# zhiyuns/AFCM

Measured on AMD Instinct MI355X. Metric: generator fwd+bwd images/sec @256^2, higher is better.
Workload: dtype bf16; 1 GPU; AFCM --model stylegan3 generator training step (fwd + L1 loss + bwd + grad all-reduce + Adam), IXI T1->T2 shape: 256x256, 4->1 channels, full-width 58.5M-param generator, random init; global_batch=16, per_gpu_batch=16, resolution=256, parallelism=dp1, world_size=1, gradient_buckets=0, comm_dtype=fp32, homogeneous_dot=True

## Files before the change

afcm_amd/_lib.py:

```python
import ctypes as C
import os

import numpy as np
import torch

_HERE = os.path.dirname(os.path.abspath(__file__))
LIB_PATH = os.environ.get('AFCM_HIP_LIB') or os.path.join(_HERE, 'libafcm_hip.so')

F32, F16, BF16 = 0, 1, 2
E_NOKERNEL, E_INVALID = -1, -2
SIGNS_NONE, SIGNS_WRITE, SIGNS_READ = 0, 1, 2
SRC_U8, SRC_I16, SRC_F32, SRC_F64 = 0, 1, 2, 3
SCHEDULE_SLOTS = 8
EMA_LERP, EMA_COPY = 0, 1
GROUP_2B, GROUP_4B = 2, 4

_DTYPES = {torch.float32: F32, torch.float16: F16, torch.bfloat16: BF16}
OUT_DTYPES = tuple(_DTYPES)
SOURCE_DTYPES = {torch.uint8: SRC_U8, torch.int16: SRC_I16, torch.float32: SRC_F32, torch.float64: SRC_F64}
NUMPY_SOURCE_DTYPES = {np.dtype(np.uint8): SRC_U8, np.dtype(np.int16): SRC_I16, np.dtype(np.float32): SRC_F32, np.dtype(np.float64): SRC_F64}


class FilteredLReluArgs(C.Structure):
    _fields_ = [
        ('x', C.c_void_p), ('y', C.c_void_p), ('b', C.c_void_p), ('signs', C.c_void_p),
        ('fu', C.c_void_p), ('fd', C.c_void_p),
        ('dtype', C.c_int32),
        ('n', C.c_int32), ('c', C.c_int32), ('xh', C.c_int32), ('xw', C.c_int32), ('yh', C.c_int32), ('yw', C.c_int32),
        ('fuw', C.c_int32), ('fuh', C.c_int32), ('fdw', C.c_int32), ('fdh', C.c_int32),
        ('up', C.c_int32), ('down', C.c_int32),
        ('px0', C.c_int32), ('px1', C.c_int32), ('py0', C.c_int32), ('py1', C.c_int32),
        ('sx', C.c_int32), ('sy', C.c_int32), ('sh', C.c_int32), ('swb', C.c_int32),
        ('gain', C.c_float), ('slope', C.c_float), ('clamp', C.c_float),
        ('flip_filter', C.c_int32), ('sign_mode', C.c_int32),
        ('workspace', C.c_void_p), ('sign_layout', C.c_int32), ('plane_sum_slots', C.c_int32),
        ('plane_sum', C.c_void_p), ('oscale', C.c_void_p), ('skip', C.c_void_p), ('oscale2', C.c_void_p),
        ('x_pitch', C.c_int32), ('y_pitch', C.c_int32), ('skip_pitch', C.c_int32), ('row_pitch_ok', C.c_int32),
        ('clamp_flags', C.c_void_p),
    ]


AFFINE_MAX = 16


class AffineBank(C.Structure):
    _fields_ = [
        ('layers', C.c_int32), ('n', C.c_int32), ('kw', C.c_int32), ('kg', C.c_int32),
        ('w_stride_n', C.c_int64), ('w_stride_l', C.c_int64),
        ('w', C.c_void_p), ('g', C.c_void_p),
        ('weight', C.c_void_p * AFFINE_MAX), ('bias', C.c_void_p * AFFINE_MAX),
        ('cout', C.c_int32 * AFFINE_MAX), ('w_index', C.c_int32 * AFFINE_MAX),
        ('alpha', C.c_float * AFFINE_MAX), ('beta', C.c_float * AFFINE_MAX),
    ]


MODULATION_MAX = 16


class ModulationLayer(C.Structure):
    _fields_ = [('cout', C.c_int32), ('cin', C.c_int32), ('kk', C.c_int32), ('demodulate', C.c_int32)] + [
        (k, C.c_void_p) for k in ('w', 't', 'magnitude', 'w_hat', 'wsq', 'scale', 's_eff', 'd', 'r', 'g_hat', 'g_s', 'g_d', 'dw', 'dt', 'workspace')]


PACK_MAX = 32


class PackEntry(C.Structure):
    _fields_ = [('dst_fwd', C.c_void_p), ('dst_dgrad', C.c_void_p), ('w', C.c_void_p),
                ('cout', C.c_int32), ('cin', C.c_int32), ('rows_pad_fwd', C.c_int32), ('rows_pad_dgrad', C.c_int32)]


_lib = None
ABI_VERSION = 13

_i32, _i64, _f32, _f64, _vp = C.c_int32, C.c_int64, C.c_float, C.c_double, C.c_void_p
SIGNATURES = {
    'afcm_abi_version': (C.c_int, []),
    'afcm_last_error': (C.c_char_p, []),
    'afcm_noop': (C.c_int, [_vp]),
    'afcm_filtered_lrelu_shapes': (C.c_int, [C.POINTER(FilteredLReluArgs)]),
    'afcm_filtered_lrelu': (C.c_int, [C.POINTER(FilteredLReluArgs), _vp]),
    'afcm_filtered_lrelu_workspace_bytes': (C.c_int64, []),
    'afcm_filtered_lrelu_prepare': (C.c_int, [C.POINTER(FilteredLReluArgs), _vp]),
    'afcm_filtered_lrelu_act': (C.c_int, [_vp, _vp, _i32, _i32, _i32, _i32, _i32, _i32, _i32, _i32, _i32, _f32, _f32, _f32, _i32, _vp]),
    'afcm_upfirdn2d': (C.c_int, [_vp, _vp, _vp, _i32, _i32, _i32, _i32, _i32, _i32, _i32, _i32, _i32, _i32, _i32, _i32, _i32,
                                 _i32, _i32, _i32, _f32, _vp]),
    'afcm_bias_act': (C.c_int, [_vp, _vp, _vp, _vp, _vp, _vp, _i32, _i64, _i64, _i32, _i32, _i32, _f32, _f32, _f32, _vp]),
    'afcm_conv2d_block_k': (C.c_int, [_i32]),
    'afcm_conv2d_block_k_ks': (C.c_int, [_i32, _i32]),
    'afcm_conv2d_pack_weights_bk': (C.c_int, [_vp, _vp, _i32, _i32, _i32, _i32, _i32, _i32, _i32, _vp]),
    'afcm_conv2d_pack_weights': (C.c_int, [_vp, _vp, _i32, _i32, _i32, _i32, _i32, _i32, _vp]),
    'afcm_conv2d_pack_weights2': (C.c_int, [_vp, _vp, _vp, _i32, _i32, _i32, _i32, _i32, _i32, _vp]),
    'afcm_conv2d': (C.c_int, [_vp, _vp, _vp, _vp, _vp, _i32, _i32, _i32, _i32, _i32, _i32, _i32, _i32, _i32, _vp]),
    'afcm_conv2d_ld': (C.c_int, [_vp, _vp, _vp, _vp, _vp, _i32, _i32, _i32, _i32, _i32, _i32, _i32, _i32, _i32, _i32, _i32, _vp]),
    'afcm_conv2d_plan': (C.c_int, [_i32] * 11 + [C.POINTER(_i32)]),
    'afcm_conv2d_wgrad_plan': (C.c_int, [_i32] * 11 + [C.POINTER(_i32)]),
    'afcm_conv2d_wgrad_splits': (C.c_int, [_i32, _i32, _i32, _i32]),
    'afcm_conv2d_wgrad': (C.c_int, [_vp, _vp, _vp, _vp, _i32, _i32, _i32, _i32, _i32, _i32, _i32, _i32, _vp]),
    'afcm_conv2d_wgrad_ld': (C.c_int, [_vp, _vp, _vp, _vp, _i32, _i32, _i32, _i32, _i32, _i32, _i32, _i32, _i32, _i32, _vp]),
    'afcm_conv2d_wgrad_dots_ld': (C.c_int, [_vp, _vp, _vp, _vp, _vp, _vp, _i32, _i32, _i32, _i32, _i32, _i32, _i32, _i32, _i32, _i32, _vp]),
    'afcm_scale_planes': (C.c_int, [_vp, _vp, _vp, _i32, _i32, _i64, _i32, _vp]),
    'afcm_plane_dot': (C.c_int, [_vp, _vp, _vp, _i32, _i64, _i32, _vp]),
    'afcm_plane_dot_ld': (C.c_int, [_vp, _vp, _vp, _i32, _i64, _i32, _i32, _i32, _i32, _vp]),
    'afcm_split16': (C.c_int, [_vp, _vp, _vp, _vp, _i32, _i64, _i32, _i32, _i64, _vp]),
    'afcm_conv2d_split': (C.c_int, [_vp, _vp, _vp, _vp, _vp, _i32, _i32, _i32, _i32, _i32, _i32, _i32, _i32, _i32, C.c_uint32, _i64, _vp, _vp, _vp]),
    'afcm_amax_bits': (C.c_int, [_vp, _vp, _i64, _i32, _vp, _vp]),
    'afcm_unscale': (C.c_int, [_vp, _i64, _vp, _vp, _vp]),
    'afcm_plane_dot_parts': (C.c_int, [_vp, _vp, _i64, _i32, _vp, _i32, _i64, _i32, _vp, _vp]),
    'afcm_conv2d_pack_split': (C.c_int, [_vp, _vp, _vp, _i32, _i32, _i32, _i32, _i32, _i32, C.c_uint32, _vp]),
    'afcm_plane_dot_gated_ld': (C.c_int, [_vp, _vp, _vp, _i32, _i64, _i32, _i32, _i32, _i32, _vp, _i32, _vp, _vp, _vp, _vp, _vp]),
    'afcm_weight_norm_fwd': (C.c_int, [_vp, _vp, _vp, _vp, _i32, _i32, _i32, _vp]),
    'afcm_weight_norm_bwd': (C.c_int, [_vp, _vp, _vp, _vp, _vp, _i32, _i32, _i32, _vp]),
    'afcm_style_coefs_fwd': (C.c_int, [_vp, _vp, _vp, _vp, _vp, _vp, _i32, _i32, _i32, _i32, _vp]),
    'afcm_style_coefs_bwd': (C.c_int, [_vp, _vp, _vp, _vp, _vp, _vp, _vp, _vp, _vp, _vp, _i32, _i32, _i32, _i32, _vp]),
    'afcm_layer_bwd_coefs': (C.c_int, [_vp, _vp, _vp, _vp, _i32, _vp, _vp, _vp, _vp, _vp, _i32, _i32, _vp]),
    'afcm_affine_bank_workspace_bytes': (C.c_int64, [C.POINTER(AffineBank)]),
    'afcm_affine_bank_fwd': (C.c_int, [C.POINTER(AffineBank), C.POINTER(C.c_void_p), _vp]),
    'afcm_modulation_bank_workspace_floats': (C.c_int64, [_i32, _i32, _i32, _i32]),
    'afcm_modulation_bank_fwd': (C.c_int, [C.POINTER(ModulationLayer), _i32, _i32, _vp]),
    'afcm_modulation_bank_bwd': (C.c_int, [C.POINTER(ModulationLayer), _i32, _i32, _vp]),
    'afcm_conv2d_stride2': (C.c_int, [_vp, _vp, _vp, _i32, _i32, _i32, _i32, _i32, _i32, _i32, _i32, _vp]),
    'afcm_conv2d_pack_bank': (C.c_int, [C.POINTER(PackEntry), _i32, _i32, _i32, _vp]),
    'afcm_affine_bank_bwd': (C.c_int, [C.POINTER(AffineBank), C.POINTER(C.c_void_p), C.POINTER(C.c_void_p), C.POINTER(C.c_void_p), _vp, _vp, _vp, _vp]),
    'afcm_pool_blocks_fwd': (C.c_int, [_vp, _vp, _i32, _i64, _i32, _i32, _vp]),
    'afcm_pool_blocks_bwd': (C.c_int, [_vp, _vp, _i32, _i64, _i32, _i32, _vp]),
    'afcm_l1_partials': (C.c_int, [_vp, _vp, _vp, _i64, _i32, _f32, _vp]),
    'afcm_l1_grad': (C.c_int, [_vp, _vp, _vp, _vp, _i64, _f32, _vp]),
    'afcm_axpy_planes': (C.c_int, [_vp, _vp, _vp, _vp, _i32, _i64, _i32, _vp]),
    'afcm_fc_act_fwd': (C.c_int, [_vp, _vp, _vp, _vp, _i32, _i32, _i32, _f32, _f32, _i32, _vp]),
    'afcm_fc_act_bwd': (C.c_int, [_vp, _vp, _vp, _vp, _vp, _vp, _vp, _i32, _i32, _i32, _f32, _f32, _i32, _vp]),
    'afcm_mapping_input_fwd': (C.c_int, [_vp, _vp, _vp, _vp, _vp, _i32, _i32, _i32, _i32, _f32, _f32, _vp]),
    'afcm_mapping_input_bwd_workspace_bytes': (C.c_int64, [_i32, _i32]),
    'afcm_mapping_input_bwd': (C.c_int, [_vp, _vp, _vp, _vp, _vp, _vp, _i32, _i32, _i32, _i32, _f32, _f32, _vp, _vp]),
    'afcm_adam_chunk_elems': (C.c_int32, []),
    'afcm_adam_multi': (C.c_int, [_vp, _i32, _i64, _f32, _f32, _f32, _f32, _f32, _f32, _f32, _f32, _i32, _f32, _f32, _i32, _vp]),
    'afcm_adam_multi_capturable': (C.c_int, [_vp, _i32, _i64, _vp, _f32, _f32, _f32, _f32, _f32, _i32, _f32, _f32, _i32, _vp]),
    'afcm_adam_multi_capturable_d': (C.c_int, [_vp, _i32, _i64, _vp, C.c_double, C.c_double, C.c_double, _f32, _f32, _i32, _f32, _f32, _i32, _vp]),
    'afcm_adam_multi_capturable_lr': (C.c_int, [_vp, _i32, _i64, _vp, _vp, C.c_double, C.c_double, _f32, _f32, _i32, _f32, _f32, _i32, _vp]),
    'afcm_plane_metrics_workspace_bytes': (C.c_int64, [_i64, _i32, _i32]),
    'afcm_plane_metrics': (C.c_int, [_vp, _vp, _vp, _i32, _i32, _i64, _i32, _i32, _i64, _i64, _i64, _i64, _i64, _i64, _i32, _f64, _f64, _vp, _vp]),
    'afcm_volume_ssim_workspace_bytes': (C.c_int64, [_i64, _i32, _i32, _i32]),
    'afcm_volume_ssim': (C.c_int, [_vp, _vp, _vp, _i32, _i32, _i64, _i32, _i32, _i32] + [_i64] * 8 + [_i32, _f64, _f64, _vp, _vp]),
    'afcm_slice_assemble': (C.c_int, [_vp, _vp, _vp, _i32, _i32, _i32, _i32, _i32, _i64, _i32, _i32, _i32, _i32, _i32, _i32, _f64, _f64, _vp]),
    'afcm_halo_accumulate': (C.c_int, [_vp, _vp, _vp, _i32, _i64, _i64, _i64, _i64, _i64, _i32, _vp, _i32, _i32, _i32] + [_i32] * 17 + [_vp]),
    'afcm_batch_assemble': (C.c_int, [_vp, _vp, _vp, _vp, _i64, _i32, _vp, _i32, _vp, _i32, _vp] + [_i32] * 6 + [_f64, _f64, _vp]),
    'afcm_batch_assemble_aug': (C.c_int, [_vp, _vp, _vp, _vp, _i64, _i32, _vp, _i32, _vp, _i32, _vp, _vp] + [_i32] * 6 + [_f64, _f64, _vp]),
    'afcm_cursor_advance': (C.c_int, [_vp, _i64, _vp]),
    'afcm_schedule_advance': (C.c_int, [_vp, _i64, _f64, _f64, _f64, _f64, _vp]),
    'afcm_gauss_blur_rmax': (C.c_int32, []),
    'afcm_gauss_blur': (C.c_int, [_vp, _vp, _vp, _i64, _i32, _i32, _f64, _vp, _vp]),
    'afcm_ema_multi': (C.c_int, [_vp, _i32, _i64, _f64, _vp, _vp]),
    'afcm_rescale_plan': (C.c_int, [_i64, _i32, C.POINTER(_i32)]),
    'afcm_rescale_workspace_bytes': (C.c_int64, [_i64, _i32]),
    'afcm_rescale_intensity': (C.c_int, [_vp, _vp, _vp, _vp, _i32, _i32, _i32, _i32, _i64, _f64, _f64, _vp]),
    'afcm_percentile_plan': (C.c_int, [_i64, _i32, C.POINTER(_i32)]),
    'afcm_percentile_workspace_bytes': (C.c_int64, [_i64, _i32]),
    'afcm_percentile_bounds': (C.c_int, [_vp, _vp, _vp, _i32, _i32, _i32, _i32, _i64, _f64, _f64, _i32, _vp]),
    'afcm_clip_normalize': (C.c_int, [_vp, _vp, _vp, _i32, _i32, _i32, _i32, _i64, _vp]),
    'afcm_group_chunk_bytes': (C.c_int32, []),
    'afcm_group_expand': (C.c_int, [_vp, _vp, _i32, _i32, _vp, _vp]),
}


def load():
    global _lib
    if _lib is None:
        if not os.path.exists(LIB_PATH):
            raise RuntimeError(
                f'{LIB_PATH} is missing: the HIP kernels are not built.  Run `python -c "import __graft_entry__ as g; g.build()"` '
                f'or `make -C afcm_amd/csrc`.  afcm_amd has no CPU fallback.')
        lib = C.CDLL(LIB_PATH)
        for name, (res, args) in SIGNATURES.items():
            fn = getattr(lib, name)
            fn.restype = res
            fn.argtypes = args
        if lib.afcm_abi_version() != ABI_VERSION:
            raise RuntimeError(f'libafcm_hip.so ABI version {lib.afcm_abi_version()} does not match this package ({ABI_VERSION}); rebuild it')
        _lib = lib
    return _lib


def dtype_code(t):
    try:
        return _DTYPES[t.dtype]
    except KeyError:
        raise RuntimeError(f'afcm_amd kernels support float32/float16/bfloat16, got {t.dtype}') from None


def source_code(dtype, what):
    code = (SOURCE_DTYPES if isinstance(dtype, torch.dtype) else NUMPY_SOURCE_DTYPES).get(dtype)
    if code is None:
        raise RuntimeError(f'{what}: source volumes are uint8 / int16 / float32 / float64, got {dtype}')
    return code


def require_out_dtype(dtype, what):
    if dtype not in OUT_DTYPES:
        raise RuntimeError(f'{what}: output dtype float32 / float16 / bfloat16, got {dtype}')


def require_slice_num(slice_num, what):
    if slice_num not in (1, 4):
        raise RuntimeError(f'{what}: slice number {slice_num} not supported (1 or 4)')


def require_gpu(*tensors):
    for t in tensors:
        if t is not None and t.device.type != 'cuda':
            raise RuntimeError(
                f'afcm_amd ops need ROCm device tensors (got a tensor on {t.device}); there is no CPU path in this package '
                f'-- the aten reference lives in oracle/ and is test-only')


def stream_ptr(t):
    return torch.cuda.current_stream(t.device).cuda_stream


def ptr(t):
    return None if t is None else t.data_ptr()


def check(rc, what):
    if rc == 0 or rc == E_NOKERNEL:
        return rc
    if rc == E_INVALID:
        raise RuntimeError(f'{what}: {load().afcm_last_error().decode()}')
    raise RuntimeError(f'{what}: HIP error {rc - 1000} at kernel launch')


def launched(rc, what):
    if check(rc, what) == E_NOKERNEL:
        raise RuntimeError(f'{what}: no kernel for this shape (the Python gate and the C entry point disagree)')
    return rc
```

afcm_amd/csrc/common.h:

```cpp
#pragma once
#include <hip/hip_runtime.h>
#include <stdint.h>
#include <stdio.h>
#include <stdarg.h>

#include "../../include/afcm_hip.h"

namespace afcm {

typedef _Float16 f16_t;
typedef __bf16   bf16_t;

template <typename T> __device__ __forceinline__ float to_f32(T v) { return (float)v; }
template <typename T> __device__ __forceinline__ T from_f32(float v) { return (T)v; }

template <int DT> struct dtype_of;
template <> struct dtype_of<AFCM_F32>  { typedef float  type; };
template <> struct dtype_of<AFCM_F16>  { typedef f16_t  type; };
template <> struct dtype_of<AFCM_BF16> { typedef bf16_t type; };

static inline int dtype_size(int dt) { return dt == AFCM_F32 ? 4 : 2; }

void set_error(const char* fmt, ...);

#define AFCM_REQUIRE(cond, ...)                         \
    do {                                                \
        if (!(cond)) {                                  \
            ::afcm::set_error(__VA_ARGS__);             \
            return AFCM_E_INVALID;                      \
        }                                               \
    } while (0)

static inline int hip_status(hipError_t e) { return e == hipSuccess ? AFCM_OK : 1000 + (int)e; }

constexpr int kAdamChunk = 16384;

constexpr int cdiv(int a, int b) { return (a + b - 1) / b; }
constexpr int round_up(int a, int b) { return cdiv(a, b) * b; }

__device__ __forceinline__ int xcd_order(int bid, int total) {
    const int x = bid & 7, k = bid >> 3, q = total >> 3, r = total & 7;
    return x * q + (x < r ? x : r) + k;
}
constexpr int cmax(int a, int b) { return a > b ? a : b; }
constexpr int odd4(int a) { return ((a / 4) % 2 == 1) ? a : a + 4; }

__host__ __device__ __forceinline__ int floor_div(int a, int b) {
    int q = a / b;
    return (a % b != 0 && (a < 0)) ? q - 1 : q;
}
__host__ __device__ __forceinline__ int pos_mod(int a, int b) {
    int r = a % b;
    return r < 0 ? r + b : r;
}

}
```

afcm_amd/csrc/conv2d_planes.hip:

```cpp
#include "conv2d_common.h"

namespace afcm {

template <typename T> struct Vec4 { T v[4]; } __attribute__((aligned(sizeof(T) * 4)));

__device__ __forceinline__ float formed_f32(float v) { asm("" : "+v"(v)); return v; }

template <typename TI, typename TO>
__global__ __launch_bounds__(256) void scale_planes_kernel(TO* __restrict__ y, const TI* __restrict__ x, const float* __restrict__ scale,
                                                           long long planes, int hw) {
    const int per = (hw + 3) >> 2;
    const long long total = planes * per;
    const bool vec = (hw & 3) == 0 && ((uintptr_t)x & (sizeof(TI) * 4 - 1)) == 0 && ((uintptr_t)y & (sizeof(TO) * 4 - 1)) == 0;
    for (long long idx = (long long)blockIdx.x * blockDim.x + threadIdx.x; idx < total; idx += (long long)gridDim.x * blockDim.x) {
        const long long plane = idx / per;
        const int i0 = (int)(idx - plane * per) << 2;
        const float sc = scale ? scale[plane] : 1.f;
        const TI* xp = x + plane * hw + i0;
        TO* yp = y + plane * hw + i0;
        if (vec) {
            const Vec4<TI> in = *(const Vec4<TI>*)xp;
            Vec4<TO> out;
#pragma unroll
            for (int e = 0; e < 4; e++) out.v[e] = from_f32<TO>(formed_f32(to_f32(in.v[e]) * sc));
// ... 9 lines not shown
template <typename T>
__global__ __launch_bounds__(256) void axpy_planes_kernel(T* __restrict__ y, const T* __restrict__ a, const T* __restrict__ b, const float* __restrict__ scale,
                                                          long long planes, int hw) {
    union V16 { uint4 u; T v[8]; };
    const int per = hw >> 3;
    for (long long plane = blockIdx.y; plane < planes; plane += gridDim.y) {
        const float sc = scale ? scale[plane] : 1.f;
        const uint4* ap = (const uint4*)a + plane * per;
        const uint4* bp = (const uint4*)b + plane * per;
        uint4* yp = (uint4*)y + plane * per;
        for (int i = blockIdx.x * blockDim.x + threadIdx.x; i < per; i += gridDim.x * blockDim.x) {
            V16 av, bv, out;
            av.u = ap[i];
            bv.u = bp[i];
#pragma unroll
            for (int e = 0; e < 8; e++) out.v[e] = from_f32<T>(to_f32(av.v[e]) + sc * to_f32(bv.v[e]));
            yp[i] = out.u;
        }
    }
}

__global__ __launch_bounds__(256) void amax_bits_kernel(unsigned* __restrict__ out, const float* __restrict__ x, long long planes, int hw,
                                                        const float* __restrict__ scale) {
    __shared__ unsigned red[4];
    unsigned m = 0;
    const long long numel = planes * hw;
    const bool vec = (((uintptr_t)x & 15) == 0) && (hw & 3) == 0;
    const long long n4 = vec ? (numel >> 2) : 0;
    const int per = hw >> 2;
    const long long stride = (long long)gridDim.x * blockDim.x;
    long long i = (long long)blockIdx.x * blockDim.x + threadIdx.x;
    auto fold = [&](const uint4 v, long long g) {
        const unsigned ax = v.x & 0x7fffffffu, ay = v.y & 0x7fffffffu, az = v.z & 0x7fffffffu, aw = v.w & 0x7fffffffu;
        unsigned a = max(max(ax < 0x7f800000u ? ax : 0u, ay < 0x7f800000u ? ay : 0u), max(az < 0x7f800000u ? az : 0u, aw < 0x7f800000u ? aw : 0u));
        if (scale) {
            a = __float_as_uint(__uint_as_float(a) * __builtin_fabsf(scale[g / per]));
            if (a >= 0x7f800000u) a = 0u;
        }
        m = max(m, a);
    };
    for (; i + 3 * stride < n4; i += 4 * stride) {
        const uint4 v0 = ((const uint4*)x)[i], v1 = ((const uint4*)x)[i + stride], v2 = ((const uint4*)x)[i + 2 * stride], v3 = ((const uint4*)x)[i + 3 * stride];
        fold(v0, i); fold(v1, i + stride); fold(v2, i + 2 * stride); fold(v3, i + 3 * stride);
    }
    for (; i < n4; i += stride) fold(((const uint4*)x)[i], i);
    for (long long j = 4 * n4 + (long long)blockIdx.x * blockDim.x + threadIdx.x; j < numel; j += stride) {
        const float v = x[j] * (scale ? scale[j / hw] : 1.f);
        const unsigned a = __float_as_uint(v) & 0x7fffffffu;
        m = max(m, a < 0x7f800000u ? a : 0u);
    }
#pragma unroll
    for (int o = 32; o > 0; o >>= 1) m = max(m, (unsigned)__shfl_xor((int)m, o));
    if ((threadIdx.x & 63) == 0) red[threadIdx.x >> 6] = m;
    __syncthreads();
    if (threadIdx.x == 0) {
        m = max(max(red[0], red[1]), max(red[2], red[3]));
        if (m > __atomic_load_n(out, __ATOMIC_RELAXED)) atomicMax(out, m);
    }
}

template <typename TP>
__global__ __launch_bounds__(256) void plane_dot_parts_kernel(float* __restrict__ out, const TP* __restrict__ parts, long long part_stride, int nparts,
                                                              const float* __restrict__ b, long long planes, int hw, const unsigned* __restrict__ bound) {
    __shared__ float red[4];
    const long long plane = blockIdx.x;
    if (plane >= planes) return;
    const TP* ap = parts + plane * hw;
    const float* bp = b + plane * hw;
    float acc = 0.f;
    if ((hw & 3) == 0 && (part_stride & 3) == 0) {
        union V8 { uint2 u; TP v[4]; };
        for (int i = threadIdx.x * 4; i < hw; i += blockDim.x * 4) {
            const float4 b0 = *(const float4*)(bp + i);
            const float bv[4] = {b0.x, b0.y, b0.z, b0.w};
            for (int k = 0; k < nparts; k++) {
                V8 a; a.u = *(const uint2*)(ap + k * part_stride + i);
#pragma unroll
                for (int e = 0; e < 4; e++) acc += (float)a.v[e] * bv[e];
            }
        }
    } else {
        for (int i = threadIdx.x; i < hw; i += blockDim.x) {
            float a = 0.f;
            for (int k = 0; k < nparts; k++) a += (float)ap[k * part_stride + i];
            acc += a * bp[i];
        }
    }
#pragma unroll
    for (int o = 32; o > 0; o >>= 1) acc += __shfl_xor(acc, o);
    if ((threadIdx.x & 63) == 0) red[threadIdx.x >> 6] = acc;
    __syncthreads();
    if (threadIdx.x == 0) {
        float inv = 1.f;
        if (bound) pow2_factor(bound[0], &inv);
        out[plane] = (red[0] + red[1] + red[2] + red[3]) * inv;
    }
}

__global__ __launch_bounds__(256) void unscale_kernel(float* __restrict__ t, long long numel, const unsigned* __restrict__ bound_a, const unsigned* __restrict__ bound_b) {
    float ia = 1.f, ib = 1.f;
    if (bound_a) pow2_factor(bound_a[0], &ia);
    if (bound_b) pow2_factor(bound_b[0], &ib);
    const float inv = ia * ib;
    for (long long i = (long long)blockIdx.x * blockDim.x + threadIdx.x; i < numel; i += (long long)gridDim.x * blockDim.x) t[i] *= inv;
}

template <typename TP, int PARTS>
__global__ __launch_bounds__(256) void split16_kernel(TP* __restrict__ parts, const float* __restrict__ x, const float* __restrict__ scale,
                                                      const unsigned* __restrict__ bound, long long planes, int hw, long long part_stride) {
    const int per = (hw + 3) >> 2;
    const long long total = planes * per;
    const bool vec = (hw & 3) == 0;
    const float gs = bound ? pow2_factor(bound[0]) : 1.f;
    for (long long idx = (long long)blockIdx.x * blockDim.x + threadIdx.x; idx < total; idx += (long long)gridDim.x * blockDim.x) {
        const long long plane = idx / per;
        const int i0 = (int)(idx - plane * per) << 2;
        const float sc = (scale ? scale[plane] : 1.f) * gs;
        const float* xp = x + plane * hw + i0;
        TP* yp = parts + plane * hw + i0;
        float v[4];
        if (vec) {
            const Vec4<float> in = *(const Vec4<float>*)xp;
#pragma unroll
            for (int e = 0; e < 4; e++) v[e] = in.v[e] * sc;
        } else {
#pragma unroll
            for (int e = 0; e < 4; e++) v[e] = (i0 + e < hw) ? xp[e] * sc : 0.f;
        }
        Vec4<TP> out[PARTS];
#pragma unroll
        for (int e = 0; e < 4; e++) {
            float r = v[e];
#pragma unroll
            for (int k = 0; k < PARTS; k++) {
                const TP q = (TP)r;
                out[k].v[e] = q;
                const float qf = (float)q;
                r = (__builtin_fabsf(qf) <= 3.4028234664e38f) ? r - qf : 0.f;
            }
        }
#pragma unroll
        for (int k = 0; k < PARTS; k++) {
            if (vec) {
                *(Vec4<TP>*)(yp + k * part_stride) = out[k];
            } else {
#pragma unroll
                for (int e = 0; e < 4; e++)
                    if (i0 + e < hw) yp[k * part_stride + e] = out[k].v[e];
            }
        }
    }
}

template <typename T>
__global__ __launch_bounds__(256) void plane_dot_kernel(float* __restrict__ out, const T* __restrict__ a, const T* __restrict__ b,
                                                        long long planes, int hw) {
    constexpr int E = 16 / (int)sizeof(T);
    union V16 { uint4 u; T v[E]; };
    __shared__ float part[4];
    const long long plane = blockIdx.x;
    if (plane >= planes) return;
    const long long off = plane * hw;
    const T* ap = a + off;
    const T* bp = b ? b + off : nullptr;
    int head = (int)((E - (off % E)) % E);
    if (head > hw) head = hw;
    const int nv = (hw - head) / E;
    float s0 = 0.f, s1 = 0.f;
    {
        const int tail0 = head + nv * E;
        int i = -1;
        if ((int)threadIdx.x < head) i = threadIdx.x;
        else if ((int)threadIdx.x - head < hw - tail0) i = tail0 + (int)threadIdx.x - head;
        if (i >= 0) s0 = to_f32(ap[i]) * (bp ? to_f32(bp[i]) : 1.f);
    }
    const uint4* av = (const uint4*)(ap + head);
    const uint4* bv = bp ? (const uint4*)(bp + head) : nullptr;
    int i = threadIdx.x;
    if (bv) {
        for (; i + 768 < nv; i += 1024) {
            V16 a0, a1, a2, a3, b0, b1, b2, b3;
            a0.u = av[i]; a1.u = av[i + 256]; a2.u = av[i + 512]; a3.u = av[i + 768];
            b0.u = bv[i]; b1.u = bv[i + 256]; b2.u = bv[i + 512]; b3.u = bv[i + 768];
#pragma unroll
            for (int e = 0; e < E; e++) {
                s0 = fmaf(to_f32(a0.v[e]), to_f32(b0.v[e]), s0); s1 = fmaf(to_f32(a1.v[e]), to_f32(b1.v[e]), s1);
                s0 = fmaf(to_f32(a2.v[e]), to_f32(b2.v[e]), s0); s1 = fmaf(to_f32(a3.v[e]), to_f32(b3.v[e]), s1);
            }
        }
    }
    for (; i + 256 < nv; i += 512) {
        V16 a0, a1, b0, b1;
        a0.u = av[i]; a1.u = av[i + 256];
        if (bv) {
            b0.u = bv[i]; b1.u = bv[i + 256];
#pragma unroll
            for (int e = 0; e < E; e++) { s0 = fmaf(to_f32(a0.v[e]), to_f32(b0.v[e]), s0); s1 = fmaf(to_f32(a1.v[e]), to_f32(b1.v[e]), s1); }
        } else {
#pragma unroll
            for (int e = 0; e < E; e++) { s0 += to_f32(a0.v[e]); s1 += to_f32(a1.v[e]); }
        }
    }
    if (i < nv) {
        V16 a0, b0;
        a0.u = av[i];
        if (bv) {
            b0.u = bv[i];
#pragma unroll
            for (int e = 0; e < E; e++) s0 = fmaf(to_f32(a0.v[e]), to_f32(b0.v[e]), s0);
        } else {
#pragma unroll
            for (int e = 0; e < E; e++) s0 += to_f32(a0.v[e]);
        }
    }
    float s = s0 + s1;
#pragma unroll
    for (int off2 = 32; off2 > 0; off2 >>= 1) s += __shfl_down(s, off2, 64);
    if ((threadIdx.x & 63) == 0) part[threadIdx.x >> 6] = s;
    __syncthreads();
    if (threadIdx.x == 0) out[plane] = part[0] + part[1] + part[2] + part[3];
}

template <typename T>
__global__ __launch_bounds__(256) void plane_dot_wave_kernel(float* __restrict__ out, const T* __restrict__ a, const T* __restrict__ b,
                                                             long long planes, int hw) {
    constexpr int E = 16 / (int)sizeof(T);
    union V16 { uint4 u; T v[E]; };
    const int lane = threadIdx.x & 63;
    const long long plane = (long long)blockIdx.x * 4 + (threadIdx.x >> 6);
    if (plane >= planes) return;
    const long long off = plane * hw;
    const T* ap = a + off;
    const T* bp = b ? b + off : nullptr;
    int head = (int)((E - (off % E)) % E);
    if (head > hw) head = hw;
    const int nv = (hw - head) / E;
    float s0 = 0.f, s1 = 0.f;
    {
        const int tail0 = head + nv * E;
        int i = -1;
        if (lane < head) i = lane;
        else if (lane - head < hw - tail0) i = tail0 + lane - head;
        if (i >= 0) s0 = to_f32(ap[i]) * (bp ? to_f32(bp[i]) : 1.f);
    }
    const uint4* av = (const uint4*)(ap + head);
    const uint4* bv = bp ? (const uint4*)(bp + head) : nullptr;
    int i = lane;
    for (; i + 64 < nv; i += 128) {
        V16 a0, a1, b0, b1;
        a0.u = av[i]; a1.u = av[i + 64];
        if (bv) {
            b0.u = bv[i]; b1.u = bv[i + 64];
#pragma unroll
            for (int e = 0; e < E; e++) { s0 = fmaf(to_f32(a0.v[e]), to_f32(b0.v[e]), s0); s1 = fmaf(to_f32(a1.v[e]), to_f32(b1.v[e]), s1); }
        } else {
#pragma unroll
            for (int e = 0; e < E; e++) { s0 += to_f32(a0.v[e]); s1 += to_f32(a1.v[e]); }
        }
    }
    if (i < nv) {
        V16 a0, b0;
        a0.u = av[i];
        if (bv) {
            b0.u = bv[i];
#pragma unroll
            for (int e = 0; e < E; e++) s0 = fmaf(to_f32(a0.v[e]), to_f32(b0.v[e]), s0);
        } else {
#pragma unroll
            for (int e = 0; e < E; e++) s0 += to_f32(a0.v[e]);
        }
    }
    float s = s0 + s1;
#pragma unroll
    for (int off2 = 32; off2 > 0; off2 >>= 1) s += __shfl_down(s, off2, 64);
    if (lane == 0) out[plane] = s;
}

struct PlaneGate {
    const int* flags;
    int slots;
    const float *osc, *gz, *nsc, *gsk;
};
template <typename T, bool PER_WAVE>
__global__ __launch_bounds__(256) void plane_dot_rows_kernel(float* __restrict__ out, const T* __restrict__ a, const T* __restrict__ b,
                                                             long long planes, int h, int w, int lda, int ldb, PlaneGate gate) {
    constexpr int E = 16 / (int)sizeof(T);
    union V16 { uint4 u; T v[E]; };
    __shared__ float part[4];
    const int nthr = PER_WAVE ? 64 : 256;
    const int t = PER_WAVE ? (int)(threadIdx.x & 63) : (int)threadIdx.x;
    const long long plane = PER_WAVE ? (long long)blockIdx.x * 4 + (threadIdx.x >> 6) : (long long)blockIdx.x;
    if (plane >= planes) return;
    if (gate.flags != nullptr) {
        int any = 0;
        for (int i = 0; i < gate.slots; i++) any |= gate.flags[plane * gate.slots + i];
        if (!any) {
            const float zz = gate.gz[plane], kk = gate.gsk ? (gate.nsc ? gate.nsc[plane] : 1.f) * gate.gsk[plane] : 0.f;
            const float diff = zz - kk;
            if (!(gate.gsk != nullptr && fabsf(diff) * 8.f < fabsf(zz) + fabsf(kk))) {
                if (t == 0) out[plane] = gate.osc[plane] * diff;
                return;
            }
        }
    }
    const int nvec = (w + E - 1) / E, total = h * nvec;
    const unsigned magic = nvec > 1 ? (unsigned)((0x100000000ull + (unsigned)nvec - 1) / (unsigned)nvec) : 0u;
    const T* ap = a + plane * h * lda;
    const T* bp = b ? b + plane * h * ldb : nullptr;
    float s0 = 0.f, s1 = 0.f;
    for (int i0 = t; i0 < total; i0 += 4 * nthr) {
        V16 av[4], bv[4];
        int skip[4];
#pragma unroll
        for (int u = 0; u < 4; u++) {
            const int i = i0 + u * nthr;
            const int ic = i < total ? i : total - 1;
            int row = nvec > 1 ? (int)__umulhi((unsigned)ic, magic) : ic;
            row -= row * nvec > ic;
            const int col = (ic - row * nvec) * E;
            const int colc = col + E <= w ? col : w - E;
            skip[u] = i < total ? col - colc : E;
            av[u].u = *(const uint4*)(ap + (size_t)row * lda + colc);
            if (bp) bv[u].u = *(const uint4*)(bp + (size_t)row * ldb + colc);
        }
#pragma unroll
        for (int u = 0; u < 4; u++) {
#pragma unroll
            for (int e = 0; e < E; e++) {
                const float x = e >= skip[u] ? to_f32(av[u].v[e]) : 0.f;
                const float y = bp ? to_f32(bv[u].v[e]) : 1.f;
                if (u & 1) s1 = fmaf(x, e >= skip[u] ? y : 0.f, s1); else s0 = fmaf(x, e >= skip[u] ? y : 0.f, s0);
            }
        }
    }
    float s = s0 + s1;
#pragma unroll
    for (int off2 = 32; off2 > 0; off2 >>= 1) s += __shfl_down(s, off2, 64);
    if (PER_WAVE) {
        if ((threadIdx.x & 63) == 0) out[plane] = s;
    } else {
        if ((threadIdx.x & 63) == 0) part[threadIdx.x >> 6] = s;
        __syncthreads();
        if (threadIdx.x == 0) out[plane] = part[0] + part[1] + part[2] + part[3];
    }
}

}

using namespace afcm;

extern "C" int afcm_split16(void* parts, const float* x, const float* scale, const uint32_t* bound, int32_t dtype, int64_t planes, int32_t hw,
                            int32_t nparts, int64_t part_stride, void* stream) {
    AFCM_REQUIRE(parts != nullptr && x != nullptr && planes > 0 && hw > 0, "split16: empty input");
    AFCM_REQUIRE(dtype == AFCM_BF16 || dtype == AFCM_F16, "split16: parts are bfloat16 or float16");
    AFCM_REQUIRE(nparts == 2 || nparts == 3, "split16: 2 or 3 parts (got %d)", nparts);
    AFCM_REQUIRE(part_stride >= planes * (long long)hw && part_stride % 4 == 0, "split16: part stride %lld must cover the tensor and be a multiple of 4", (long long)part_stride);
    AFCM_REQUIRE(((uintptr_t)x & 15) == 0 && ((uintptr_t)parts & 7) == 0, "split16: x must be 16-byte, parts 8-byte aligned");
    long long blocks = (planes * ((hw + 3) >> 2) + 255) / 256;
    if (blocks > 4096) blocks = 4096;
    dim3 grid((unsigned)blocks), block(256);
    hipStream_t st = (hipStream_t)stream;
#define AFCM_SPLIT(T, K) hipLaunchKernelGGL((split16_kernel<T, K>), grid, block, 0, st, (T*)parts, x, scale, (const unsigned*)bound, (long long)planes, hw, (long long)part_stride)
    if (dtype == AFCM_BF16) { if (nparts == 2) AFCM_SPLIT(bf16_t, 2); else AFCM_SPLIT(bf16_t, 3); }
    else { if (nparts == 2) AFCM_SPLIT(f16_t, 2); else AFCM_SPLIT(f16_t, 3); }
#undef AFCM_SPLIT
    return hip_status(hipGetLastError());
}

extern "C" int afcm_amax_bits(uint32_t* out, const float* x, int64_t planes, int32_t hw, const float* scale, void* stream) {
    AFCM_REQUIRE(out != nullptr && x != nullptr && planes > 0 && hw > 0, "amax_bits: empty input");
    AFCM_REQUIRE(((uintptr_t)out & 3) == 0 && ((uintptr_t)x & 3) == 0, "amax_bits: misaligned pointer");
    long long blocks = (planes * hw / 16 + 255) / 256;
    blocks = blocks < 1 ? 1 : (blocks > 2048 ? 2048 : blocks);
    hipLaunchKernelGGL(amax_bits_kernel, dim3((unsigned)blocks), dim3(256), 0, (hipStream_t)stream, (unsigned*)out, x, (long long)planes, hw, scale);
    return hip_status(hipGetLastError());
}

extern "C" int afcm_plane_dot_parts(float* out, const void* parts, int64_t part_stride, int32_t nparts, const float* b, int32_t dtype, int64_t planes,
                                    int32_t hw, const uint32_t* bound, void* stream) {
    AFCM_REQUIRE(out != nullptr && parts != nullptr && b != nullptr && planes > 0 && hw > 0, "plane_dot_parts: empty input");
    AFCM_REQUIRE(dtype == AFCM_BF16 || dtype == AFCM_F16, "plane_dot_parts: parts are bfloat16 or float16");
    AFCM_REQUIRE(nparts >= 1 && nparts <= 3 && part_stride >= planes * (long long)hw, "plane_dot_parts: 1..3 parts, a stride covering the tensor");
    AFCM_REQUIRE(planes < (1ll << 31), "plane_dot_parts: too many planes");
    AFCM_REQUIRE(((uintptr_t)parts & 7) == 0 && ((uintptr_t)b & 15) == 0, "plane_dot_parts: parts must be 8-byte, b 16-byte aligned");
    hipStream_t st = (hipStream_t)stream;
    if (dtype == AFCM_BF16) hipLaunchKernelGGL((plane_dot_parts_kernel<bf16_t>), dim3((unsigned)planes), dim3(256), 0, st, out, (const bf16_t*)parts, (long long)part_stride, nparts, b, (long long)planes, hw, (const unsigned*)bound);
    else hipLaunchKernelGGL((plane_dot_parts_kernel<f16_t>), dim3((unsigned)planes), dim3(256), 0, st, out, (const f16_t*)parts, (long long)part_stride, nparts, b, (long long)planes, hw, (const unsigned*)bound);
    return hip_status(hipGetLastError());
}

extern "C" int afcm_unscale(float* t, int64_t numel, const uint32_t* bound_a, const uint32_t* bound_b, void* stream) {
    AFCM_REQUIRE(t != nullptr && numel > 0, "unscale: empty input");
    long long blocks = (numel + 255) / 256;
    if (blocks > 2048) blocks = 2048;
    hipLaunchKernelGGL(unscale_kernel, dim3((unsigned)blocks), dim3(256), 0, (hipStream_t)stream, t, (long long)numel, (const unsigned*)bound_a, (const unsigned*)bound_b);
    return hip_status(hipGetLastError());
}

extern "C" int afcm_scale_planes(void* y, const void* x, const float* scale, int32_t dtype_in, int32_t dtype_out, int64_t planes,
                                 int32_t hw, void* stream) {
    AFCM_REQUIRE(y != nullptr && x != nullptr && planes > 0 && hw > 0, "scale_planes: empty input");
    long long blocks = (planes * ((hw + 3) >> 2) + 255) / 256;
    if (blocks > 2048) blocks = 2048;
    dim3 grid((unsigned)blocks), block(256);
    hipStream_t st = (hipStream_t)stream;
#define AFCM_SP(TI, TO) hipLaunchKernelGGL((scale_planes_kernel<TI, TO>), grid, block, 0, st, (TO*)y, (const TI*)x, scale, (long long)planes, hw)
    if (dtype_in == AFCM_F32 && dtype_out == AFCM_F32) AFCM_SP(float, float);
    else if (dtype_in == AFCM_F32 && dtype_out == AFCM_BF16) AFCM_SP(float, bf16_t);
    else if (dtype_in == AFCM_F32 && dtype_out == AFCM_F16) AFCM_SP(float, f16_t);
    else if (dtype_in == AFCM_BF16 && dtype_out == AFCM_BF16) AFCM_SP(bf16_t, bf16_t);
    else if (dtype_in == AFCM_F16 && dtype_out == AFCM_F16) AFCM_SP(f16_t, f16_t);
    else if (dtype_in == AFCM_BF16 && dtype_out == AFCM_F32) AFCM_SP(bf16_t, float);
    else if (dtype_in == AFCM_F16 && dtype_out == AFCM_F32) AFCM_SP(f16_t, float);
    else { set_error("scale_planes: unsupported dtype pair %d -> %d", dtype_in, dtype_out); return AFCM_E_INVALID; }
#undef AFCM_SP
    return hip_status(hipGetLastError());
}

extern "C" int afcm_axpy_planes(void* y, const void* a, const void* b, const float* scale, int32_t dtype, int64_t planes, int32_t hw, void* stream) {
    AFCM_REQUIRE(y != nullptr && a != nullptr && b != nullptr && planes > 0 && hw > 0, "axpy_planes: empty input");
    AFCM_REQUIRE(dtype == AFCM_F16 || dtype == AFCM_BF16, "axpy_planes: 16-bit tensors only");
    if ((hw & 7) != 0 || ((((uintptr_t)y | (uintptr_t)a | (uintptr_t)b)) & 15) != 0) return AFCM_E_NOKERNEL;
    const int per = hw >> 3;
    const dim3 grid((unsigned)((per + 1023) / 1024), (unsigned)(planes < 65535 ? planes : 65535));
    hipStream_t st = (hipStream_t)stream;
    if (dtype == AFCM_BF16) hipLaunchKernelGGL((axpy_planes_kernel<bf16_t>), grid, dim3(256), 0, st, (bf16_t*)y, (const bf16_t*)a, (const bf16_t*)b, scale, (long long)planes, hw);
    else hipLaunchKernelGGL((axpy_planes_kernel<f16_t>), grid, dim3(256), 0, st, (f16_t*)y, (const f16_t*)a, (const f16_t*)b, scale, (long long)planes, hw);
    return hip_status(hipGetLastError());
}

extern "C" int afcm_plane_dot(float* out, const void* a, const void* b, int32_t dtype, int64_t planes, int32_t hw, void* stream) {
    AFCM_REQUIRE(out != nullptr && a != nullptr && planes > 0 && hw > 0, "plane_dot: empty input");
    AFCM_REQUIRE(planes < (1ll << 31), "plane_dot: too many planes");
    AFCM_REQUIRE((((uintptr_t)a | (uintptr_t)b) & 15) == 0, "plane_dot: operands must be 16-byte aligned");
    hipStream_t st = (hipStream_t)stream;
    const int esize = dtype == AFCM_F32 ? 4 : 2;
    const bool per_wave = (long long)hw * esize <= 16384;
    dim3 grid((unsigned)(per_wave ? (planes + 3) / 4 : planes)), block(256);
#define AFCM_PD(T) do { \
        if (per_wave) hipLaunchKernelGGL((plane_dot_wave_kernel<T>), grid, block, 0, st, out, (const T*)a, (const T*)b, (long long)planes, hw); \
        else hipLaunchKernelGGL((plane_dot_kernel<T>), grid, block, 0, st, out, (const T*)a, (const T*)b, (long long)planes, hw); } while (0)
    switch (dtype) {
        case AFCM_F32: AFCM_PD(float); break;
        case AFCM_F16: AFCM_PD(f16_t); break;
        case AFCM_BF16: AFCM_PD(bf16_t); break;
        default: set_error("plane_dot: bad dtype"); return AFCM_E_INVALID;
    }
#undef AFCM_PD
    return hip_status(hipGetLastError());
}

static int plane_dot_rows(float* out, const void* a, const void* b, int32_t dtype, int64_t planes, int32_t h, int32_t w,
                          int32_t a_pitch, int32_t b_pitch, const PlaneGate& gate, void* stream) {
    AFCM_REQUIRE(out != nullptr && a != nullptr && planes > 0 && h > 0 && w > 0, "plane_dot: empty input");
    AFCM_REQUIRE(planes < (1ll << 31), "plane_dot: too many planes");
    const int esize = dtype == AFCM_F32 ? 4 : 2;
    const int lda = a_pitch ? a_pitch : w, ldb = b_pitch ? b_pitch : w;
    AFCM_REQUIRE(lda >= w && ldb >= w, "plane_dot: row pitches %d / %d are below the width %d", lda, ldb, w);
    AFCM_REQUIRE(w >= 16 / esize, "plane_dot: rows of %d elements are shorter than one 16-byte vector", w);
    AFCM_REQUIRE((((uintptr_t)a | (uintptr_t)b) & 3) == 0 && (esize == 4 || ((w | lda | ldb) & 1) == 0), "plane_dot: rows must start on 4-byte boundaries");
    AFCM_REQUIRE((long long)h * (lda > ldb ? lda : ldb) < (1ll << 31) / 16, "plane_dot: plane is out of range");
    hipStream_t st = (hipStream_t)stream;
    const bool per_wave = (long long)h * w * esize <= 16384;
    dim3 grid((unsigned)(per_wave ? (planes + 3) / 4 : planes)), block(256);
#define AFCM_PDR(T) do { \
        if (per_wave) hipLaunchKernelGGL((plane_dot_rows_kernel<T, true>), grid, block, 0, st, out, (const T*)a, (const T*)b, (long long)planes, h, w, lda, ldb, gate); \
        else hipLaunchKernelGGL((plane_dot_rows_kernel<T, false>), grid, block, 0, st, out, (const T*)a, (const T*)b, (long long)planes, h, w, lda, ldb, gate); } while (0)
    switch (dtype) {
        case AFCM_F32: AFCM_PDR(float); break;
        case AFCM_F16: AFCM_PDR(f16_t); break;
        case AFCM_BF16: AFCM_PDR(bf16_t); break;
        default: set_error("plane_dot: bad dtype"); return AFCM_E_INVALID;
    }
#undef AFCM_PDR
    return hip_status(hipGetLastError());
}

extern "C" int afcm_plane_dot_ld(float* out, const void* a, const void* b, int32_t dtype, int64_t planes, int32_t h, int32_t w,
                                 int32_t a_pitch, int32_t b_pitch, void* stream) {
    return plane_dot_rows(out, a, b, dtype, planes, h, w, a_pitch, b_pitch, PlaneGate{nullptr, 0, nullptr, nullptr, nullptr, nullptr}, stream);
}

extern "C" int afcm_plane_dot_gated_ld(float* out, const void* a, const void* b, int32_t dtype, int64_t planes, int32_t h, int32_t w,
                                       int32_t a_pitch, int32_t b_pitch, const int32_t* flags, int32_t slots, const float* out_scale,
                                       const float* gz, const float* next_scale, const float* gskip, void* stream) {
    AFCM_REQUIRE(flags != nullptr && slots > 0 && out_scale != nullptr && gz != nullptr && b != nullptr, "plane_dot_gated: null pointer");
    return plane_dot_rows(out, a, b, dtype, planes, h, w, a_pitch, b_pitch, PlaneGate{flags, slots, out_scale, gz, next_scale, gskip}, stream);
}
```

afcm_amd/csrc/conv2d_wgrad.hip:

```cpp
#include <type_traits>

#include "conv2d_common.h"

namespace afcm {

constexpr int kWgKQ = 64;

struct WgradParams {
    const void* dy;
    const void* x;
    float* part;
    int N, O, I, H, W, P, Q, pad;
    int lddy, ldx;
    int splits, steps_per_split;
    int splits_img;
    int qchunks;
    int rowgroups;
};

template <int KS, int XOFF>
__global__ __launch_bounds__(512, 1) void conv2d_wgrad_kernel(WgradParams p) {
    constexpr int R = 1, KK = KS * KS;
    constexpr int PDY = kWgKQ + 8;
    constexpr int PX = kWgKQ + 24;
// ... 685 lines not shown
                    const frag_t bv = *(const frag_t*)(buf + x0_off[ib2] + xr * (64 * ROWB));
#pragma unroll
                    for (int ob2 = 0; ob2 < 2; ob2++) mma(a[ob2][xr], bv, 0, 2 * ob2 + ib2);
                });
            } else {
                frag_t a[2][R];
#pragma unroll
                for (int ob2 = 0; ob2 < 2; ob2++)
#pragma unroll
                    for (int rr = 0; rr < R; rr++) a[ob2][rr] = *(const frag_t*)(buf + a_off[ob2] + rr * (64 * ROWB));
                uint4 lo_n = *(const uint4*)(buf + x0_off[0]);
                uint4 hi_n = *(const uint4*)(buf + x1_off[0][0]);
                static_for<0, 2 * XR>([&](auto itc) __attribute__((always_inline)) {
                    constexpr int it = decltype(itc)::value, xr = it >> 1, ib2 = it & 1, NIT = 2 * XR;
                    const uint4 lo = lo_n, hi = hi_n;
                    if constexpr (it + 1 < NIT) {
                        constexpr int xr1 = (it + 1) >> 1, ib1 = (it + 1) & 1;
                        lo_n = *(const uint4*)(buf + x0_off[ib1] + xr1 * (64 * ROWB));
                        hi_n = *(const uint4*)(buf + x1_off[ib1][xr1]);
                    }
                    __builtin_amdgcn_sched_barrier(0);
                    if constexpr (LATE) {
                        static_assert(!LATE || NPIECE == NIT - 1, "one piece per iteration after the first");
                        if constexpr (it > 0) issue_piece(std::integral_constant<int, it - 1>{});
                    } else
                        issue_range(std::integral_constant<int, (it * NPIECE) / NIT>{}, std::integral_constant<int, ((it + 1) * NPIECE) / NIT>{});
                    asm volatile("" : : "v"(lo.x), "v"(lo.y), "v"(lo.z));
                    const unsigned d[5] = {lo.w, hi.x, hi.y, hi.z, hi.w};
#pragma unroll
                    for (int sft = 0; sft < KS; sft++) {
                        union { unsigned u[4]; frag_t f; } bw;
#pragma unroll
                        for (int w = 0; w < 4; w++)
                            bw.u[w] = (sft == 0) ? d[w] : (sft == 1) ? __builtin_amdgcn_alignbyte(d[w + 1], d[w], 2) : d[w + 1];
#pragma unroll
                        for (int rr = 0; rr < R; rr++) {
                            const int r = xr - rr;
                            if (r >= 0 && r < KS) {
#pragma unroll
                                for (int ob2 = 0; ob2 < 2; ob2++) mma(a[ob2][rr], bw.f, r * KS + sft, 2 * ob2 + ib2);
                            }
                        }
                    }
                    if constexpr (LATE && it == 0) begin_loads(step + NBUF - 1 < s1);
                    __builtin_amdgcn_sched_barrier(0);
                });
            }
        } else if constexpr (!TAIL) {
            static_for<0, 2>([&](auto kqc) __attribute__((always_inline)) {
                constexpr int kq = decltype(kqc)::value;
                if ((kq * 2 + th) * 16 >= vq) {
                    issue_range(std::integral_constant<int, (kq * XR * NPIECE) / (2 * XR)>{}, std::integral_constant<int, ((kq + 1) * XR * NPIECE) / (2 * XR)>{});
                    return;
                }
                frag_t a[R];
#pragma unroll
                for (int rr = 0; rr < R; rr++) a[rr] = *(const frag_t*)(buf + a_off[kq] + rr * (64 * ROWB));
                static_for<0, XR>([&](auto xrc) __attribute__((always_inline)) {
                    constexpr int xr = decltype(xrc)::value;
                    constexpr int it = kq * XR + xr, NIT = 2 * XR;
                    issue_range(std::integral_constant<int, (it * NPIECE) / NIT>{}, std::integral_constant<int, ((it + 1) * NPIECE) / NIT>{});
                    const frag_t b = *(const frag_t*)(buf + x0_off[kq] + xr * (64 * ROWB));
                    constexpr int rr = xr;
                    if constexpr (std::is_same<T, bf16_t>::value) acc[0] = __builtin_amdgcn_mfma_f32_32x32x16_bf16(a[rr], b, acc[0], 0, 0, 0);
                    else acc[0] = __builtin_amdgcn_mfma_f32_32x32x16_f16(a[rr], b, acc[0], 0, 0, 0);
                });
            });
        } else {
            frag_t a[2][R];
#pragma unroll
            for (int rr = 0; rr < R; rr++) a[0][rr] = *(const frag_t*)(buf + a_off[0] + rr * (64 * ROWB));
            uint4 lo_n = *(const uint4*)(buf + x0_off[0]);
            uint4 hi_n = *(const uint4*)(buf + x1_off[0][0]);
            static_for<0, 2>([&](auto kqc) __attribute__((always_inline)) {
                constexpr int kq = decltype(kqc)::value;
                if ((kq * 2 + th) * 16 >= vq) {
                    issue_range(std::integral_constant<int, (kq * XR * NPIECE) / (2 * XR)>{}, std::integral_constant<int, ((kq + 1) * XR * NPIECE) / (2 * XR)>{});
                    if constexpr (kq == 0) {
#pragma unroll
                        for (int rr = 0; rr < R; rr++) a[1][rr] = *(const frag_t*)(buf + a_off[1] + rr * (64 * ROWB));
                        lo_n = *(const uint4*)(buf + x0_off[1]);
                        hi_n = *(const uint4*)(buf + x1_off[1][0]);
                    }
                    return;
                }
                static_for<0, XR>([&](auto xrc) __attribute__((always_inline)) {
                    constexpr int xr = decltype(xrc)::value;
                    const uint4 lo = lo_n, hi = hi_n;
                    if constexpr (xr + 1 < XR) {
                        lo_n = *(const uint4*)(buf + x0_off[kq] + (xr + 1) * (64 * ROWB));
                        hi_n = *(const uint4*)(buf + x1_off[kq][xr + 1 < XR ? xr + 1 : xr]);
                    } else if constexpr (kq == 0) {
                        lo_n = *(const uint4*)(buf + x0_off[1]);
                        hi_n = *(const uint4*)(buf + x1_off[1][0]);
                    }
                    if constexpr (kq == 0 && xr == 1) {
#pragma unroll
                        for (int rr = 0; rr < R; rr++) a[1][rr] = *(const frag_t*)(buf + a_off[1] + rr * (64 * ROWB));
                    }
                    __builtin_amdgcn_sched_barrier(0);
                    row_mfmas(kqc, xrc, lo, hi, a[kq]);
                    __builtin_amdgcn_sched_barrier(0);
                });
            });
        }
        if (NBUF == 3) asm volatile("s_waitcnt vmcnt(%0)" : : "n"(NPIECE));
        else { asm volatile("s_waitcnt vmcnt(0)"); f_q0 = c_q0; f_live = c_live; f_bufa = c_bufa; }
        fix_edge();
        __syncthreads();
        if (++cbuf == NBUF) cbuf = 0;
    }
    asm volatile("s_waitcnt vmcnt(0)");
    __syncthreads();
    {
        float* red = (float*)lds;
        constexpr int TPR_CAP = (NBUF * BUF) / (4 * 16 * 64 * (int)sizeof(float));
        constexpr int TPR = TPR_CAP < KK ? TPR_CAP : KK;
        static_assert(TPR >= 1, "LDS too small for the half-sum");
        const int wv4 = wo + 2 * wi;
#pragma unroll
        for (int t0 = 0; t0 < KK; t0 += TPR) {
            if (t0 > 0) __syncthreads();
            if (th == 1) {
#pragma unroll
                for (int t = t0; t < t0 + TPR && t < KK; t++)
#pragma unroll
                    for (int reg = 0; reg < 16; reg++) red[((wv4 * TPR + (t - t0)) * 16 + reg) * 64 + lane] = acc[t][reg];
            }
            __syncthreads();
            if (th == 0) {
#pragma unroll
                for (int t = t0; t < t0 + TPR && t < KK; t++)
#pragma unroll
                    for (int reg = 0; reg < 16; reg++) acc[t][reg] += red[((wv4 * TPR + (t - t0)) * 16 + reg) * 64 + lane];
            }
        }
    }
    if (th == 0) {
        float* out = p.part + (size_t)split * p.O * p.I * KK;
#pragma unroll
        for (int reg = 0; reg < 16; reg++) {
            const int o = o0 + wo * 32 + (X16 ? 16 * (reg >> 3) + 4 * g4 + (reg & 3) : (reg & 3) + 8 * (reg >> 2) + 4 * h);
            const int i = i0 + wi * 32 + (X16 ? 16 * ((reg >> 2) & 1) + c16 : r32);
            if (o < p.O && i < p.I) {
                float* dst = out + ((size_t)o * p.I + i) * KK;
#pragma unroll
                for (int t = 0; t < KK; t++) dst[t] = acc[t][reg];
            }
        }
    }
}

struct WgradSlabs { int splits; };
__global__ __launch_bounds__(256) void wgrad_reduce_kernel(float* __restrict__ dw, const float* __restrict__ part, long long numel, WgradSlabs w) {
    for (long long idx = (long long)blockIdx.x * blockDim.x + threadIdx.x; idx < numel; idx += (long long)gridDim.x * blockDim.x) {
        float s = 0.f;
        for (int k = 0; k < w.splits; k++) s += part[(size_t)k * numel + idx];
        dw[idx] = s;
    }
}

template <int COLS>
__global__ __launch_bounds__(256) void wgrad_reduce4_kernel(float* __restrict__ dw, const float* __restrict__ part, long long numel4, WgradSlabs w) {
    constexpr int GROUPS = 256 / COLS;
    typedef __attribute__((ext_vector_type(4))) float f32x4v;
    __shared__ f32x4v red[GROUPS][COLS];
    const int col = threadIdx.x % COLS, grp = threadIdx.x / COLS;
    const long long c4 = (long long)blockIdx.x * COLS + col;
    f32x4v s0 = {0.f, 0.f, 0.f, 0.f}, s1 = s0;
    if (c4 < numel4) {
        const f32x4v* src = (const f32x4v*)part + c4;
        const int splits = w.splits;
        int k = grp;
        for (; k + 3 * GROUPS < splits; k += 4 * GROUPS) {
            const f32x4v v0 = src[(size_t)k * numel4], v1 = src[(size_t)(k + GROUPS) * numel4];
            const f32x4v v2 = src[(size_t)(k + 2 * GROUPS) * numel4], v3 = src[(size_t)(k + 3 * GROUPS) * numel4];
            s0 += v0; s1 += v1; s0 += v2; s1 += v3;
        }
        for (; k < splits; k += GROUPS) s0 += src[(size_t)k * numel4];
    }
    s0 += s1;
    if (GROUPS > 1) {
        red[grp][col] = s0;
        __syncthreads();
        if (grp == 0 && c4 < numel4) {
#pragma unroll
            for (int g = 1; g < GROUPS; g++) s0 += red[g][col];
            ((f32x4v*)dw)[c4] = s0;
        }
    } else if (c4 < numel4) {
        ((f32x4v*)dw)[c4] = s0;
    }
}


template <typename T, int KK>
__global__ __launch_bounds__(1024) void wgrad_reduce_dots_kernel(float* __restrict__ dw, float* __restrict__ dots, const float* __restrict__ part,
                                                                 const float* __restrict__ w, int N, int O, int I, int splits_img) {
    constexpr int NW = 16;
    __shared__ float red[NW - 1][64][KK];
    const int i = blockIdx.x, lane = threadIdx.x & 63, q = threadIdx.x >> 6;
    const size_t slab = (size_t)O * I * KK;
    float dotp[4];
#pragma unroll
    for (int k = 0; k < 4; k++) dotp[k] = 0.f;
    for (int ob = 0; ob < O; ob += 64) {
        const int o = ob + lane;
        const bool live = o < O;
        const size_t e0 = ((size_t)(live ? o : O - 1) * I + i) * KK;
        float wq[KK], tot[KK];
#pragma unroll
        for (int t = 0; t < KK; t++) { wq[t] = live ? to_f32(from_f32<T>(w[e0 + t])) : 0.f; tot[t] = 0.f; }
#pragma unroll
        for (int k = 0; k < 4; k++) {
            const int n = q + NW * k;
            if (n >= N) break;
            float acc[KK];
#pragma unroll
            for (int t = 0; t < KK; t++) acc[t] = 0.f;
            for (int sp = 0; sp < splits_img; sp++) {
                const float* src = part + (size_t)(n * splits_img + sp) * slab + e0;
#pragma unroll
                for (int t = 0; t < KK; t++) acc[t] += src[t];
            }
            float d = 0.f;
#pragma unroll
            for (int t = 0; t < KK; t++) { tot[t] += acc[t]; d = fmaf(wq[t], acc[t], d); }
            dotp[k] += d;
        }
        if (ob > 0) __syncthreads();
        if (q > 0) {
#pragma unroll
            for (int t = 0; t < KK; t++) red[q - 1][lane][t] = tot[t];
        }
        __syncthreads();
        if (q == 0 && live) {
#pragma unroll
            for (int t = 0; t < KK; t++) {
                float s = tot[t];
#pragma unroll
                for (int k = 0; k < NW - 1; k++) s += red[k][lane][t];
                dw[e0 + t] = s;
            }
        }
    }
#pragma unroll
    for (int k = 0; k < 4; k++) {
        const int n = q + NW * k;
        if (n >= N) break;
        float d = dotp[k];
#pragma unroll
        for (int off = 32; off > 0; off >>= 1) d += __shfl_xor(d, off);
        if (lane == 0) dots[(size_t)n * I + i] = d;
    }
}
}

using namespace afcm;


static int wgrad_rows_per_step(int dtype) { return dtype == AFCM_F32 ? 1 : 2; }

static int wgrad_splits(int n, int cout, int cin, int p_rows) {
    const int tiles = cdiv(cout, 64) * cdiv(cin, 64);
    const long long ksteps = (long long)n * p_rows;
    int s = 256 / tiles;
    if (s > ksteps) s = (int)ksteps;
    return s < 1 ? 1 : s;
}

extern "C" int afcm_conv2d_wgrad_splits(int32_t n, int32_t cout, int32_t cin, int32_t p_rows) {
    return wgrad_splits(n, cout, cin, p_rows);
}

extern "C" int afcm_conv2d_wgrad(float* dw, float* workspace, const void* dy, const void* x, int32_t dtype, int32_t n, int32_t cin,
                                 int32_t cout, int32_t h, int32_t w, int32_t ks, int32_t pad, void* stream) {
    return afcm_conv2d_wgrad_ld(dw, workspace, dy, x, dtype, n, cin, cout, h, w, ks, pad, 0, 0, stream);
}

enum { kWgF32 = 0, kWgDword = 1, kWgGranule = 2 };
enum { kWgReduceScalar = 0, kWgReduce4x256 = 1, kWgReduce4x64 = 2, kWgReduce4x16 = 3, kWgReduceDots = 4 };
struct WgradPlan {
    int kernel;
    int pad_odd;
    bool x16;
    bool small;
    int qchunks, rowgroups;
    int splits, steps_per_split, splits_img;
    int reduce;
};

static int wgrad_plan(WgradPlan* pl, int dtype, int n, int cin, int cout, int h, int ldx, int ks, int pad, int P, int Q, int lddy, bool dots) {
    const int R = wgrad_rows_per_step(dtype);
    pl->qchunks = cdiv(Q, kWgKQ);
    pl->rowgroups = cdiv(P, R);
    const long long ksteps = (long long)n * pl->rowgroups * pl->qchunks;
    const bool granule = (ks == 3 && pad == 2) || (ks == 1 && pad == 0);
    pl->kernel = dtype == AFCM_F32 ? kWgF32 : granule ? kWgGranule : kWgDword;
    pl->pad_odd = (ks == 3) ? (pad & 1) : 0;
    pl->splits = wgrad_splits(n, cout, cin, P);
    if (pl->splits > ksteps) pl->splits = (int)ksteps;
    pl->steps_per_split = (int)((ksteps + pl->splits - 1) / pl->splits);
    pl->splits_img = 0;
    if (dots) {
        if (pl->kernel != kWgGranule || n > 64 || pl->splits % n != 0 || pl->splits / n < 1) return AFCM_E_NOKERNEL;
        pl->splits_img = pl->splits / n;
        const long long per_img = (long long)pl->rowgroups * pl->qchunks;
        pl->steps_per_split = (int)((per_img + pl->splits_img - 1) / pl->splits_img);
    }
    const int q_last = Q % 64;
    pl->x16 = !(q_last > 32 && q_last <= 48);
    pl->small = (long long)n * cout * P * lddy * 2 < (1ll << 31) - 65536 &&
                (long long)n * cin * h * ldx * 2 < (1ll << 31) - 65536;
    const long long numel = (long long)cout * cin * ks * ks;
    if (pl->splits_img > 0) pl->reduce = kWgReduceDots;
    else if ((numel & 3) != 0) pl->reduce = kWgReduceScalar;
    else pl->reduce = pl->splits >= 64 ? kWgReduce4x16 : pl->splits >= 8 ? kWgReduce4x64 : kWgReduce4x256;
    return AFCM_OK;
}

static int wgrad_impl(float* dw, float* workspace, const void* dy, const void* x, int32_t dtype, int32_t n, int32_t cin,
                      int32_t cout, int32_t h, int32_t w, int32_t ks, int32_t pad, int32_t dy_pitch, int32_t x_pitch, float* dots, const float* wref, void* stream) {
    AFCM_REQUIRE(dw != nullptr && workspace != nullptr && dy != nullptr && x != nullptr, "conv2d_wgrad: null pointer");
    AFCM_REQUIRE(dtype == AFCM_F32 || dtype == AFCM_F16 || dtype == AFCM_BF16, "x must be float32, float16 or bfloat16");
    AFCM_REQUIRE(ks == 1 || ks == 3, "only 1x1 and 3x3 kernels are supported");
    AFCM_REQUIRE(pad >= 0 && pad <= ks - 1, "padding must be in [0, k-1]");
    WgradParams p;
    p.dy = dy; p.x = x; p.part = workspace;
    p.N = n; p.O = cout; p.I = cin; p.H = h; p.W = w; p.pad = pad;
    p.P = h + 2 * pad - ks + 1; p.Q = w + 2 * pad - ks + 1;
    AFCM_REQUIRE(p.P >= 1 && p.Q >= 1, "output must be at least 1x1");
    AFCM_REQUIRE(dtype == AFCM_F32 || (w % 2 == 0 && p.Q % 2 == 0), "16-bit conv2d_wgrad needs even widths (got %d, %d)", w, p.Q);
    p.lddy = dy_pitch ? dy_pitch : p.Q; p.ldx = x_pitch ? x_pitch : w;
    const bool pitched = p.lddy != p.Q || p.ldx != w;
    AFCM_REQUIRE(!pitched || (p.lddy >= p.Q && p.ldx >= w && ((p.lddy | p.ldx) & 1) == 0), "conv2d_wgrad: row pitches %d / %d must be even and cover the widths %d / %d", p.lddy, p.ldx, p.Q, w);
    WgradPlan pl;
    if (wgrad_plan(&pl, dtype, n, cin, cout, h, p.ldx, ks, pad, p.P, p.Q, p.lddy, dots != nullptr) != AFCM_OK) return AFCM_E_NOKERNEL;
    AFCM_REQUIRE(dots == nullptr || wref != nullptr, "conv2d_wgrad_dots: the weight tensor the dot products are taken with is missing");
    p.qchunks = pl.qchunks; p.rowgroups = pl.rowgroups;
    p.splits = pl.splits; p.steps_per_split = pl.steps_per_split; p.splits_img = pl.splits_img;
    const bool granule = pl.kernel == kWgGranule;
    const bool wg_x16 = pl.x16, small = pl.small;
    const long long blocks = (long long)cdiv(cout, 64) * cdiv(cin, 64) * p.splits;
    dim3 grid((unsigned)blocks), block(512);
    hipStream_t st = (hipStream_t)stream;
#define AFCM_WG16(T) do { constexpr int NB = 3; \
                           if (pl.pad_odd == 0) hipLaunchKernelGGL((conv2d_wgrad16_kernel<T, 3, 0, NB>), grid, block, 0, st, p); \
                           else hipLaunchKernelGGL((conv2d_wgrad16_kernel<T, 3, 1, NB>), grid, block, 0, st, p); } while (0)
#define AFCM_WG16G_(T, X) do { constexpr int NB = kWgradRing; \
                            if (small && ks == 3) hipLaunchKernelGGL((conv2d_wgrad16g_kernel<T, 3, NB, true, X>), grid, block, 0, st, p); \
                            else if (small) hipLaunchKernelGGL((conv2d_wgrad16g_kernel<T, 1, NB, true, X>), grid, block, 0, st, p); \
                            else if (ks == 3) hipLaunchKernelGGL((conv2d_wgrad16g_kernel<T, 3, NB, false, X>), grid, block, 0, st, p); \
                            else hipLaunchKernelGGL((conv2d_wgrad16g_kernel<T, 1, NB, false, X>), grid, block, 0, st, p); } while (0)
#define AFCM_WG16G(T) do { if (wg_x16) AFCM_WG16G_(T, true); else AFCM_WG16G_(T, false); } while (0)
    AFCM_REQUIRE(!pitched || (dtype != AFCM_F32 && granule), "conv2d_wgrad: row pitches need the 16-bit granule kernel (3x3 pad 2 or 1x1 pad 0)");
    switch (dtype) {
        case AFCM_F32:
            if (ks == 3 && pl.pad_odd == 0) hipLaunchKernelGGL((conv2d_wgrad_kernel<3, 0>), grid, block, 0, st, p);
            else if (ks == 3) hipLaunchKernelGGL((conv2d_wgrad_kernel<3, 1>), grid, block, 0, st, p);
            else hipLaunchKernelGGL((conv2d_wgrad_kernel<1, 0>), grid, block, 0, st, p);
            break;
        case AFCM_F16: if (granule) AFCM_WG16G(f16_t); else AFCM_WG16(f16_t); break;
        default: if (granule) AFCM_WG16G(bf16_t); else AFCM_WG16(bf16_t); break;
    }
#undef AFCM_WG16G
#undef AFCM_WG16G_
#undef AFCM_WG16
    int rc = hip_status(hipGetLastError());
    if (rc != AFCM_OK) return rc;
    const long long numel = (long long)cout * cin * ks * ks;
    if (p.splits_img > 0) {
        const dim3 rgrid((unsigned)cin), rblock(1024);
#define AFCM_RD(T) do { if (ks == 3) hipLaunchKernelGGL((wgrad_reduce_dots_kernel<T, 9>), rgrid, rblock, 0, st, dw, dots, (const float*)workspace, wref, n, cout, cin, p.splits_img); \
                        else hipLaunchKernelGGL((wgrad_reduce_dots_kernel<T, 1>), rgrid, rblock, 0, st, dw, dots, (const float*)workspace, wref, n, cout, cin, p.splits_img); } while (0)
        if (dtype == AFCM_F16) AFCM_RD(f16_t); else AFCM_RD(bf16_t);
#undef AFCM_RD
        return hip_status(hipGetLastError());
    }
    const WgradSlabs slabs{p.splits};
    long long rb = (numel + 255) / 256;
    if (rb > 2048) rb = 2048;
    if (pl.reduce != kWgReduceScalar && (((uintptr_t)dw | (uintptr_t)workspace) & 15) == 0) {
        const long long n4 = numel / 4;
        if (pl.reduce == kWgReduce4x16) hipLaunchKernelGGL(wgrad_reduce4_kernel<16>, dim3((unsigned)cdiv(n4, 16)), dim3(256), 0, st, dw, (const float*)workspace, n4, slabs);
        else if (pl.reduce == kWgReduce4x64) hipLaunchKernelGGL(wgrad_reduce4_kernel<64>, dim3((unsigned)cdiv(n4, 64)), dim3(256), 0, st, dw, (const float*)workspace, n4, slabs);
        else hipLaunchKernelGGL(wgrad_reduce4_kernel<256>, dim3((unsigned)cdiv(n4, 256)), dim3(256), 0, st, dw, (const float*)workspace, n4, slabs);
    } else {
        hipLaunchKernelGGL(wgrad_reduce_kernel, dim3((unsigned)rb), dim3(256), 0, st, dw, (const float*)workspace, numel, slabs);
    }
    return hip_status(hipGetLastError());
}

extern "C" int afcm_conv2d_wgrad_ld(float* dw, float* workspace, const void* dy, const void* x, int32_t dtype, int32_t n, int32_t cin,
                                    int32_t cout, int32_t h, int32_t w, int32_t ks, int32_t pad, int32_t dy_pitch, int32_t x_pitch, void* stream) {
    return wgrad_impl(dw, workspace, dy, x, dtype, n, cin, cout, h, w, ks, pad, dy_pitch, x_pitch, nullptr, nullptr, stream);
}

extern "C" int afcm_conv2d_wgrad_dots_ld(float* dw, float* dots, float* workspace, const void* dy, const void* x, const float* wref, int32_t dtype,
                                         int32_t n, int32_t cin, int32_t cout, int32_t h, int32_t w, int32_t ks, int32_t pad, int32_t dy_pitch,
                                         int32_t x_pitch, void* stream) {
    AFCM_REQUIRE(dots != nullptr, "conv2d_wgrad_dots: dots must be non-null");
    return wgrad_impl(dw, workspace, dy, x, dtype, n, cin, cout, h, w, ks, pad, dy_pitch, x_pitch, dots, wref, stream);
}

extern "C" int afcm_conv2d_wgrad_plan(int32_t dtype, int32_t n, int32_t cin, int32_t cout, int32_t h, int32_t w, int32_t ks, int32_t pad,
                                      int32_t dy_pitch, int32_t x_pitch, int32_t dots, int32_t out[8]) {
    AFCM_REQUIRE(out != nullptr, "conv2d_wgrad_plan: null pointer");
    AFCM_REQUIRE(dtype == AFCM_F32 || dtype == AFCM_F16 || dtype == AFCM_BF16, "x must be float32, float16 or bfloat16");
    AFCM_REQUIRE(n > 0 && cin > 0 && cout > 0 && h > 0 && w > 0, "x is empty");
    AFCM_REQUIRE(ks == 1 || ks == 3, "only 1x1 and 3x3 kernels are supported");
    AFCM_REQUIRE(pad >= 0 && pad <= ks - 1, "padding must be in [0, k-1]");
    const int P = h + 2 * pad - ks + 1, Q = w + 2 * pad - ks + 1;
    AFCM_REQUIRE(P >= 1 && Q >= 1, "output must be at least 1x1");
    WgradPlan pl;
    const int rc = wgrad_plan(&pl, dtype, n, cin, cout, h, x_pitch ? x_pitch : w, ks, pad, P, Q, dy_pitch ? dy_pitch : Q, dots != 0);
    if (rc != AFCM_OK) return rc;
    out[0] = pl.kernel; out[1] = pl.pad_odd; out[2] = pl.x16 ? 1 : 0; out[3] = pl.small ? 1 : 0; out[4] = pl.splits; out[5] = pl.steps_per_split;
    out[6] = pl.reduce; out[7] = pl.splits_img;
    return AFCM_OK;
}
```

afcm_amd/csrc/modulation.hip:

```cpp
#include "common.h"

namespace afcm {

__device__ __forceinline__ float block_sum(float v, float* red) {
#pragma unroll
    for (int off = 32; off > 0; off >>= 1) v += __shfl_xor(v, off, 64);
    __syncthreads();
    if ((threadIdx.x & 63) == 0) red[threadIdx.x >> 6] = v;
    __syncthreads();
    return red[0] + red[1] + red[2] + red[3];
}

template <int PT>
__device__ __forceinline__ void weight_norm_fwd_body(float* red, float* row, int o, float* __restrict__ w_hat, float* __restrict__ wsq,
                                                     float* __restrict__ scale, const float* __restrict__ w, int I, int KK) {
    const int n = I * KK;
    const float* wo = w + (size_t)o * n;
    float ss = 0.f;
    if constexpr (PT > 0) {
        float v[PT];
#pragma unroll
        for (int k = 0; k < PT; k++) { const int j = threadIdx.x + 256 * k; v[k] = j < n ? wo[j] : 0.f; }
#pragma unroll
        for (int k = 0; k < PT; k++) ss += v[k] * v[k];
// ... 71 lines not shown
        dot = block_sum(dot, red);
        const float m = dot / (float)n, sc = scale[o];
        for (int j = threadIdx.x; j < n; j += 256) {
            const float wh = w_hat[base + j];
            float g = g_hat ? g_hat[base + j] : 0.f;
            if (g_wsq) g += 2.f * wh * g_wsq[(size_t)o * I + j / KK];
            dw[base + j] = sc * (g - wh * m);
        }
    }
}

template <int PT>
__global__ __launch_bounds__(256) void weight_norm_bwd_kernel(float* __restrict__ dw, const float* __restrict__ g_hat, const float* __restrict__ g_wsq,
                                                              const float* __restrict__ w_hat, const float* __restrict__ scale, int I, int KK) {
    __shared__ float red[4];
    weight_norm_bwd_body<PT>(red, blockIdx.x, dw, g_hat, g_wsq, w_hat, scale, I, KK);
}

__device__ __forceinline__ void style_coefs_fwd_body(float* red, float* s2, int n, int oc, float* __restrict__ s_eff, float* __restrict__ d,
                                                     float* __restrict__ r_out, const float* __restrict__ t, const float* __restrict__ wsq,
                                                     const float* __restrict__ magnitude, int N, int I, int O, int demod) {
    float r = 1.f;
    if (demod) {
        float ss = 0.f;
        float s4[4] = {0.f, 0.f, 0.f, 0.f};
        int j = threadIdx.x;
        for (; j + 768 < N * I; j += 1024) {
            const float a0 = t[j], a1 = t[j + 256], a2 = t[j + 512], a3 = t[j + 768];
            s4[0] += a0 * a0; s4[1] += a1 * a1; s4[2] += a2 * a2; s4[3] += a3 * a3;
        }
        for (; j < N * I; j += 256) s4[0] += t[j] * t[j];
        ss = block_sum((s4[0] + s4[1]) + (s4[2] + s4[3]), red);
        r = rsqrtf(ss / (float)(N * I));
    }
    if (n == 0 && oc == 0 && threadIdx.x == 0) r_out[0] = r;
    const float g = magnitude ? rsqrtf(magnitude[0]) : 1.f;
    for (int i = threadIdx.x; i < I; i += 256) {
        const float sh = t[(size_t)n * I + i] * r;
        if (oc == 0) s_eff[(size_t)n * I + i] = sh * g;
        s2[i] = sh * sh;
    }
    if (!demod) return;
    __syncthreads();
    const int wave = threadIdx.x >> 6, lane = threadIdx.x & 63;
    const int ob = oc * 32 + wave * 8;
    float q[8];
#pragma unroll
    for (int j = 0; j < 8; j++) q[j] = 0.f;
    for (int i = lane; i < I; i += 64) {
        const float sv = s2[i];
#pragma unroll
        for (int j = 0; j < 8; j++) {
            const int o = ob + j < O ? ob + j : O - 1;
            q[j] = fmaf(sv, wsq[(size_t)o * I + i], q[j]);
        }
    }
#pragma unroll
    for (int j = 0; j < 8; j++) {
#pragma unroll
        for (int off = 32; off > 0; off >>= 1) q[j] += __shfl_xor(q[j], off, 64);
        if (lane == 0 && ob + j < O) d[(size_t)n * O + ob + j] = rsqrtf(q[j] + 1e-8f);
    }
}

__global__ __launch_bounds__(256) void style_coefs_fwd_kernel(float* __restrict__ s_eff, float* __restrict__ d, float* __restrict__ r_out,
                                                              const float* __restrict__ t, const float* __restrict__ wsq,
                                                              const float* __restrict__ magnitude, int N, int I, int O, int demod) {
    __shared__ float red[4];
    extern __shared__ float s2[];
    style_coefs_fwd_body(red, s2, blockIdx.x, blockIdx.y, s_eff, d, r_out, t, wsq, magnitude, N, I, O, demod);
}

__device__ __forceinline__ void style_coefs_bwd1_body(float (*us)[64], float* q_s, int n, int ib, int IB, float* __restrict__ G,
                                                      float* __restrict__ Q, float* __restrict__ partial, const float* __restrict__ g_s,
                                                      const float* __restrict__ g_d, const float* __restrict__ t, const float* __restrict__ d,
                                                      const float* __restrict__ wsq, const float* __restrict__ magnitude,
                                                      const float* __restrict__ r_in, int I, int O, int demod) {
    const int tx = threadIdx.x & 63, ty = threadIdx.x >> 6;
    const int i = ib * 64 + tx;
    const float r = r_in[0], g = magnitude ? rsqrtf(magnitude[0]) : 1.f;
    if (demod) {
        for (int o = threadIdx.x; o < O; o += 256) {
            const float dd = d[(size_t)n * O + o];
            const float q = g_d ? -0.5f * g_d[(size_t)n * O + o] * dd * dd * dd : 0.f;
            q_s[o] = q;
            if (ib == 0) Q[(size_t)n * O + o] = q;
        }
        __syncthreads();
        float u = 0.f;
        if (i < I) {
#pragma unroll 8
            for (int o = ty; o < O; o += 4) u = fmaf(q_s[o], wsq[(size_t)o * I + i], u);
        }
        us[ty][tx] = u;
        __syncthreads();
    }
    if (ty != 0) return;
    float dot = 0.f;
    if (i < I) {
        const float sh = t[(size_t)n * I + i] * r;
        float gg = g_s ? g * g_s[(size_t)n * I + i] : 0.f;
        if (demod) gg += 2.f * sh * (us[0][tx] + us[1][tx] + us[2][tx] + us[3][tx]);
        G[(size_t)n * I + i] = gg;
        dot = gg * sh;
    }
#pragma unroll
    for (int off = 32; off > 0; off >>= 1) dot += __shfl_xor(dot, off, 64);
    if (tx == 0) partial[(size_t)n * IB + ib] = dot;
}

__global__ __launch_bounds__(256) void style_coefs_bwd1_kernel(float* __restrict__ G, float* __restrict__ Q, float* __restrict__ partial,
                                                               const float* __restrict__ g_s, const float* __restrict__ g_d,
                                                               const float* __restrict__ t, const float* __restrict__ d, const float* __restrict__ wsq,
                                                               const float* __restrict__ magnitude, const float* __restrict__ r_in, int I, int O, int demod) {
    __shared__ float us[4][64];
    extern __shared__ float q_s[];
    style_coefs_bwd1_body(us, q_s, blockIdx.x, blockIdx.y, gridDim.y, G, Q, partial, g_s, g_d, t, d, wsq, magnitude, r_in, I, O, demod);
}

__device__ __forceinline__ void style_coefs_bwd2_body(int bx, float* __restrict__ dt, float* __restrict__ g_wsq, const float* __restrict__ G,
                                                      const float* __restrict__ Q, const float* __restrict__ partial, const float* __restrict__ t,
                                                      const float* __restrict__ r_in, int N, int I, int O, int demod, int NP) {
    const float r = r_in[0];
    if (bx < N) {
        const int n = bx;
        float m = 0.f;
        if (demod) {
            for (int k = 0; k < NP; k++) m += partial[k];
            m /= (float)(N * I);
        }
        for (int i = threadIdx.x; i < I; i += 256) {
            const float gg = G[(size_t)n * I + i];
            dt[(size_t)n * I + i] = demod ? r * (gg - t[(size_t)n * I + i] * r * m) : gg;
        }
    } else if (demod && g_wsq != nullptr) {
        const int o = bx - N;
        for (int i = threadIdx.x; i < I; i += 256) {
            float acc = 0.f;
            for (int n = 0; n < N; n++) {
                const float sh = t[(size_t)n * I + i] * r;
                acc += Q[(size_t)n * O + o] * sh * sh;
            }
            g_wsq[(size_t)o * I + i] = acc;
        }
    }
}

__global__ __launch_bounds__(256) void style_coefs_bwd2_kernel(float* __restrict__ dt, float* __restrict__ g_wsq, const float* __restrict__ G,
                                                               const float* __restrict__ Q, const float* __restrict__ partial,
                                                               const float* __restrict__ t, const float* __restrict__ r_in, int N, int I, int O, int demod, int NP) {
    style_coefs_bwd2_body((int)blockIdx.x, dt, g_wsq, G, Q, partial, t, r_in, N, I, O, demod, NP);
}

__global__ __launch_bounds__(64) void layer_bwd_coefs_kernel(float* __restrict__ db, float* __restrict__ d_next, float* __restrict__ d_out,
                                                             const float* __restrict__ psum, int slots, const float* __restrict__ out_scale,
                                                             const float* __restrict__ next_scale, const float* __restrict__ bias,
                                                             const float* __restrict__ gz, const float* __restrict__ dysy, int N, int O) {
    const int o = blockIdx.x;
    const float b = bias ? bias[o] : 0.f;
    float acc = 0.f;
    for (int n = threadIdx.x; n < N; n += 64) {
        const size_t idx = (size_t)n * O + o;
        float ps = 0.f;
        for (int k = 0; k < slots; k++) ps += psum[idx * slots + k];
        const float d = out_scale ? out_scale[idx] : 1.f;
        acc += ps / d;
        if (d_next) {
            const float ns = next_scale[idx];
            d_next[idx] = ns != 0.f ? gz[idx] / ns : 0.f;
        }
        if (d_out) d_out[idx] = (dysy[idx] - b * ps) / (d * d);
    }
#pragma unroll
    for (int off = 32; off > 0; off >>= 1) acc += __shfl_xor(acc, off, 64);
    if (db && threadIdx.x == 0) db[o] = acc;
}

struct ModBank {
    int count, n;
    int blk[AFCM_MODULATION_MAX + 1];
    afcm_modulation_layer L[AFCM_MODULATION_MAX];
};

__device__ __forceinline__ int bank_layer(const ModBank& b, int bid) {
    int l = 0;
    while (l + 1 < b.count && bid >= b.blk[l + 1]) l++;
    return l;
}

__global__ __launch_bounds__(256) void modulation_bank_norm_fwd_kernel(const ModBank b) {
    __shared__ float red[4];
    __shared__ float row[256 * 18];
    const int l = bank_layer(b, blockIdx.x), o = blockIdx.x - b.blk[l];
    const afcm_modulation_layer& L = b.L[l];
    const int n = L.cin * L.kk;
    if (n <= 256 * 4) weight_norm_fwd_body<4>(red, row, o, L.w_hat, L.wsq, L.scale, L.w, L.cin, L.kk);
    else if (n <= 256 * 18) weight_norm_fwd_body<18>(red, row, o, L.w_hat, L.wsq, L.scale, L.w, L.cin, L.kk);
    else weight_norm_fwd_body<0>(red, row, o, L.w_hat, L.wsq, L.scale, L.w, L.cin, L.kk);
}

__global__ __launch_bounds__(256) void modulation_bank_coefs_fwd_kernel(const ModBank b) {
    __shared__ float red[4];
    extern __shared__ float dyn[];
    const int l = bank_layer(b, blockIdx.x), loc = blockIdx.x - b.blk[l];
    const afcm_modulation_layer& L = b.L[l];
    const int ocs = L.demodulate ? (L.cout + 31) / 32 : 1;
    style_coefs_fwd_body(red, dyn, loc / ocs, loc % ocs, L.s_eff, L.d, L.r, L.t, L.wsq, L.magnitude, b.n, L.cin, L.cout, L.demodulate);
}

__device__ __forceinline__ void bank_workspace(const afcm_modulation_layer& L, int n, float*& G, float*& Q, float*& partial, float*& g_wsq) {
    G = L.workspace;
    Q = G + (size_t)n * L.cin;
    partial = Q + (size_t)n * (L.demodulate ? L.cout : 0);
    g_wsq = partial + (size_t)n * ((L.cin + 63) / 64);
}

__global__ __launch_bounds__(256) void modulation_bank_coefs_bwd1_kernel(const ModBank b) {
    __shared__ float us[4][64];
    extern __shared__ float dyn[];
    const int l = bank_layer(b, blockIdx.x), loc = blockIdx.x - b.blk[l];
    const afcm_modulation_layer& L = b.L[l];
    const int IB = (L.cin + 63) / 64;
    float *G, *Q, *partial, *g_wsq;
    bank_workspace(L, b.n, G, Q, partial, g_wsq);
    style_coefs_bwd1_body(us, dyn, loc / IB, loc % IB, IB, G, Q, partial, L.g_s, L.g_d, L.t, L.d, L.wsq, L.magnitude, L.r, L.cin, L.cout, L.demodulate);
}

__global__ __launch_bounds__(256) void modulation_bank_coefs_bwd2_kernel(const ModBank b) {
    const int l = bank_layer(b, blockIdx.x), loc = blockIdx.x - b.blk[l];
    const afcm_modulation_layer& L = b.L[l];
    float *G, *Q, *partial, *g_wsq;
    bank_workspace(L, b.n, G, Q, partial, g_wsq);
    style_coefs_bwd2_body(loc, L.dt, g_wsq, G, Q, partial, L.t, L.r, b.n, L.cin, L.cout, L.demodulate, b.n * ((L.cin + 63) / 64));
}

__global__ __launch_bounds__(256) void modulation_bank_norm_bwd_kernel(const ModBank b) {
    __shared__ float red[4];
    const int l = bank_layer(b, blockIdx.x), o = blockIdx.x - b.blk[l];
    const afcm_modulation_layer& L = b.L[l];
    float *G, *Q, *partial, *g_wsq;
    bank_workspace(L, b.n, G, Q, partial, g_wsq);
    const int n = L.cin * L.kk;
    if (n <= 256 * 4) weight_norm_bwd_body<4>(red, o, L.dw, L.g_hat, g_wsq, L.w_hat, L.scale, L.cin, L.kk);
    else if (n <= 256 * 18) weight_norm_bwd_body<18>(red, o, L.dw, L.g_hat, g_wsq, L.w_hat, L.scale, L.cin, L.kk);
    else weight_norm_bwd_body<0>(red, o, L.dw, L.g_hat, g_wsq, L.w_hat, L.scale, L.cin, L.kk);
}

}

using namespace afcm;

extern "C" int afcm_layer_bwd_coefs(float* db, float* d_next, float* d_out, const float* psum, int32_t slots, const float* out_scale,
                                    const float* next_scale, const float* bias, const float* gz, const float* dysy, int32_t n, int32_t cout,
                                    void* stream) {
    AFCM_REQUIRE(psum && slots > 0 && n > 0 && cout > 0, "layer_bwd_coefs: bad arguments");
    AFCM_REQUIRE(!d_next || (next_scale && gz), "layer_bwd_coefs: d_next needs next_scale and <g, z>");
    AFCM_REQUIRE(!d_out || (out_scale && dysy), "layer_bwd_coefs: d_out needs out_scale and <dys, y>");
    hipLaunchKernelGGL(layer_bwd_coefs_kernel, dim3(cout), dim3(64), 0, (hipStream_t)stream, db, d_next, d_out, psum, slots, out_scale, next_scale,
                       bias, gz, dysy, n, cout);
    return hip_status(hipGetLastError());
}

extern "C" int afcm_weight_norm_fwd(float* w_hat, float* wsq, float* scale, const float* w, int32_t cout, int32_t cin, int32_t kk, void* stream) {
    AFCM_REQUIRE(w_hat && wsq && scale && w && cout > 0 && cin > 0 && kk > 0, "weight_norm_fwd: bad arguments");
    const int n = cin * kk;
    if (n <= 256 * 4) hipLaunchKernelGGL(weight_norm_fwd_kernel<4>, dim3(cout), dim3(256), 0, (hipStream_t)stream, w_hat, wsq, scale, w, cin, kk);
    else if (n <= 256 * 18) hipLaunchKernelGGL(weight_norm_fwd_kernel<18>, dim3(cout), dim3(256), 0, (hipStream_t)stream, w_hat, wsq, scale, w, cin, kk);
    else hipLaunchKernelGGL(weight_norm_fwd_kernel<0>, dim3(cout), dim3(256), 0, (hipStream_t)stream, w_hat, wsq, scale, w, cin, kk);
    return hip_status(hipGetLastError());
}

extern "C" int afcm_weight_norm_bwd(float* dw, const float* g_hat, const float* g_wsq, const float* w_hat, const float* scale, int32_t cout,
                                    int32_t cin, int32_t kk, void* stream) {
    AFCM_REQUIRE(dw && w_hat && scale && cout > 0 && cin > 0 && kk > 0, "weight_norm_bwd: bad arguments");
    const int n = cin * kk;
    if (n <= 256 * 4) hipLaunchKernelGGL(weight_norm_bwd_kernel<4>, dim3(cout), dim3(256), 0, (hipStream_t)stream, dw, g_hat, g_wsq, w_hat, scale, cin, kk);
    else if (n <= 256 * 18) hipLaunchKernelGGL(weight_norm_bwd_kernel<18>, dim3(cout), dim3(256), 0, (hipStream_t)stream, dw, g_hat, g_wsq, w_hat, scale, cin, kk);
    else hipLaunchKernelGGL(weight_norm_bwd_kernel<0>, dim3(cout), dim3(256), 0, (hipStream_t)stream, dw, g_hat, g_wsq, w_hat, scale, cin, kk);
    return hip_status(hipGetLastError());
}

extern "C" int afcm_style_coefs_fwd(float* s_eff, float* d, float* r, const float* t, const float* wsq, const float* magnitude, int32_t n, int32_t cin,
                                    int32_t cout, int32_t demodulate, void* stream) {
    AFCM_REQUIRE(s_eff && r && t && n > 0 && cin > 0 && (!demodulate || (d && wsq && cout > 0)), "style_coefs_fwd: bad arguments");
    AFCM_REQUIRE(cin <= 16384, "style_coefs_fwd: %d input channels exceed the LDS row", cin);
    hipLaunchKernelGGL(style_coefs_fwd_kernel, dim3(n, demodulate ? (cout + 31) / 32 : 1), dim3(256), cin * sizeof(float), (hipStream_t)stream, s_eff,
                       d, r, t, wsq, magnitude, n, cin, cout, demodulate);
    return hip_status(hipGetLastError());
}

extern "C" int afcm_style_coefs_bwd(float* dt, float* g_wsq, float* workspace, const float* g_s, const float* g_d, const float* t, const float* d,
                                    const float* wsq, const float* magnitude, const float* r, int32_t n, int32_t cin, int32_t cout, int32_t demodulate,
                                    void* stream) {
    AFCM_REQUIRE(dt && workspace && t && r && n > 0 && cin > 0 && (!demodulate || (d && wsq && cout > 0)), "style_coefs_bwd: bad arguments");
    AFCM_REQUIRE(cout <= 16384, "style_coefs_bwd: %d output channels exceed the LDS row", cout);
    float* G = workspace;
    float* Q = G + (size_t)n * cin;
    float* partial = Q + (size_t)n * (demodulate ? cout : 0);
    hipStream_t st = (hipStream_t)stream;
    const int ib = (cin + 63) / 64;
    hipLaunchKernelGGL(style_coefs_bwd1_kernel, dim3(n, ib), dim3(256), (demodulate ? cout : 1) * sizeof(float), st, G, Q, partial, g_s, g_d, t, d, wsq,
                       magnitude, r, cin, cout, demodulate);
    hipLaunchKernelGGL(style_coefs_bwd2_kernel, dim3(n + ((demodulate && g_wsq) ? cout : 0)), dim3(256), 0, st, dt, g_wsq, G, Q, partial, t, r, n, cin,
                       cout, demodulate, n * ib);
    return hip_status(hipGetLastError());
}

static int bank_check(const afcm_modulation_layer* layers, int32_t count, int32_t n, bool bwd) {
    AFCM_REQUIRE(layers && count > 0 && count <= AFCM_MODULATION_MAX && n > 0, "modulation_bank: bad arguments (1..%d layers)", AFCM_MODULATION_MAX);
    for (int l = 0; l < count; l++) {
        const afcm_modulation_layer& L = layers[l];
        AFCM_REQUIRE(L.cin > 0 && L.cin <= 16384 && L.t && L.r, "modulation_bank: layer %d: styles / r missing or cin outside 1..16384", l);
        if (L.demodulate)
            AFCM_REQUIRE(L.cout > 0 && L.cout <= 16384 && L.kk > 0 && L.w_hat && L.wsq && L.scale && L.d,
                         "modulation_bank: layer %d demodulates: w_hat / wsq / scale / d needed, cout in 1..16384", l);
        if (bwd) AFCM_REQUIRE(L.dt && L.workspace, "modulation_bank: layer %d: dt / workspace missing", l);
        else AFCM_REQUIRE(L.s_eff && (!L.demodulate || L.w), "modulation_bank: layer %d: s_eff / w missing", l);
    }
    return AFCM_OK;
}

extern "C" int64_t afcm_modulation_bank_workspace_floats(int32_t n, int32_t cin, int32_t cout, int32_t demodulate) {
    if (n <= 0 || cin <= 0 || (demodulate && cout <= 0)) return -1;
    return (int64_t)n * cin + (int64_t)n * ((cin + 63) / 64) + (demodulate ? (int64_t)n * cout + (int64_t)cout * cin : 0);
}

extern "C" int afcm_modulation_bank_fwd(const afcm_modulation_layer* layers, int32_t count, int32_t n, void* stream) {
    if (int rc = bank_check(layers, count, n, false)) return rc;
    hipStream_t st = (hipStream_t)stream;
    ModBank b;
    b.count = count;
    b.n = n;
    int max_cin = 1;
    for (int l = 0; l < count; l++) { b.L[l] = layers[l]; max_cin = layers[l].cin > max_cin ? layers[l].cin : max_cin; }
    int tot = 0;
    for (int l = 0; l < count; l++) { b.blk[l] = tot; tot += layers[l].demodulate ? layers[l].cout : 0; }
    b.blk[count] = tot;
    if (tot > 0) hipLaunchKernelGGL(modulation_bank_norm_fwd_kernel, dim3(tot), dim3(256), 0, st, b);
    tot = 0;
    for (int l = 0; l < count; l++) { b.blk[l] = tot; tot += n * (layers[l].demodulate ? (layers[l].cout + 31) / 32 : 1); }
    b.blk[count] = tot;
    hipLaunchKernelGGL(modulation_bank_coefs_fwd_kernel, dim3(tot), dim3(256), max_cin * sizeof(float), st, b);
    return hip_status(hipGetLastError());
}

extern "C" int afcm_modulation_bank_bwd(const afcm_modulation_layer* layers, int32_t count, int32_t n, void* stream) {
    if (int rc = bank_check(layers, count, n, true)) return rc;
    hipStream_t st = (hipStream_t)stream;
    ModBank b;
    b.count = count;
    b.n = n;
    int max_cout = 1;
    for (int l = 0; l < count; l++) { b.L[l] = layers[l]; if (layers[l].demodulate && layers[l].cout > max_cout) max_cout = layers[l].cout; }
    int tot = 0;
    for (int l = 0; l < count; l++) { b.blk[l] = tot; tot += n * ((layers[l].cin + 63) / 64); }
    b.blk[count] = tot;
    hipLaunchKernelGGL(modulation_bank_coefs_bwd1_kernel, dim3(tot), dim3(256), max_cout * sizeof(float), st, b);
    tot = 0;
    for (int l = 0; l < count; l++) { b.blk[l] = tot; tot += n + ((layers[l].demodulate && layers[l].dw) ? layers[l].cout : 0); }
    b.blk[count] = tot;
    hipLaunchKernelGGL(modulation_bank_coefs_bwd2_kernel, dim3(tot), dim3(256), 0, st, b);
    tot = 0;
    for (int l = 0; l < count; l++) { b.blk[l] = tot; tot += (layers[l].demodulate && layers[l].dw) ? layers[l].cout : 0; }
    b.blk[count] = tot;
    if (tot > 0) hipLaunchKernelGGL(modulation_bank_norm_bwd_kernel, dim3(tot), dim3(256), 0, st, b);
    return hip_status(hipGetLastError());
}
```

afcm_amd/torch_utils/ops/conv2d.py:

```python
import torch

from ... import _lib
from ... import profiling
from . import _rows


def _pad64(n):
    return (n + 63) // 64 * 64


def pack_weights(w, dtype, mode):
    lib = _lib.load()
    o, i, kh, kw = w.shape
    assert kh == kw and kh in (1, 3), 'only 1x1 and 3x3 kernels are supported'
    w = w.detach().to(torch.float32).contiguous()
    code = _lib._DTYPES[dtype]
    bk = lib.afcm_conv2d_block_k_ks(code, kh)
    rows, cols = (o, i) if mode == 0 else (i, o)
    rows_pad = _pad64(rows)
    nkc = (cols + bk - 1) // bk
    dst = torch.empty([nkc, kh * kw, rows_pad, bk], dtype=dtype, device=w.device)
    _lib.launched(lib.afcm_conv2d_pack_weights(dst.data_ptr(), w.data_ptr(), code, o, i, kh, mode, rows_pad, _lib.stream_ptr(w)),
                  'conv2d_pack_weights')
    return dst, rows_pad


def pack_weights_both(w, dtype):
    lib = _lib.load()
    o, i, kh, kw = w.shape
    assert kh == kw and kh in (1, 3), 'only 1x1 and 3x3 kernels are supported'
    w = w.detach().to(torch.float32).contiguous()
    code = _lib._DTYPES[dtype]
    bk = lib.afcm_conv2d_block_k_ks(code, kh)
    rp0, rp1 = _pad64(o), _pad64(i)
    d0 = torch.empty([(i + bk - 1) // bk, kh * kw, rp0, bk], dtype=dtype, device=w.device)
    d1 = torch.empty([(o + bk - 1) // bk, kh * kw, rp1, bk], dtype=dtype, device=w.device)
    _lib.launched(lib.afcm_conv2d_pack_weights2(d0.data_ptr(), d1.data_ptr(), w.data_ptr(), code, o, i, kh, rp0, rp1, _lib.stream_ptr(w)),
                  'conv2d_pack_weights2')
    return (d0, rp0), (d1, rp1)


PACK_MAX = _lib.PACK_MAX


def pack_weights_bank(ws, dtype, need_dgrad=True):
    lib = _lib.load()
    assert 0 < len(ws) <= _lib.PACK_MAX
    ks = int(ws[0].shape[2])
    assert ks in (1, 3) and all(tuple(w.shape[2:]) == (ks, ks) for w in ws), 'one kernel size (1x1 or 3x3) per bank'
    code = _lib._DTYPES[dtype]
    bk = lib.afcm_conv2d_block_k_ks(code, ks)
    table = (_lib.PackEntry * len(ws))()
    out, keep = [], []
    for e, w in zip(table, ws):
        o, i = int(w.shape[0]), int(w.shape[1])
        w32 = w.detach().to(torch.float32).contiguous()
        keep.append(w32)
        rp0, rp1 = _pad64(o), _pad64(i)
        d0 = torch.empty([(i + bk - 1) // bk, ks * ks, rp0, bk], dtype=dtype, device=w.device)
        d1 = torch.empty([(o + bk - 1) // bk, ks * ks, rp1, bk], dtype=dtype, device=w.device) if need_dgrad else None
        e.dst_fwd, e.dst_dgrad, e.w = d0.data_ptr(), (d1.data_ptr() if need_dgrad else 0), w32.data_ptr()
        e.cout, e.cin, e.rows_pad_fwd, e.rows_pad_dgrad = o, i, rp0, rp1
        out.append(((d0, rp0), ((d1, rp1) if need_dgrad else None)))
    _lib.launched(lib.afcm_conv2d_pack_bank(table, len(ws), code, ks, _lib.stream_ptr(ws[0])), 'conv2d_pack_bank')
    return out


def scale_planes(x, scale, out_dtype=None):
    lib = _lib.load()
    out_dtype = out_dtype or x.dtype
    full = _rows.whole_buffer(x) if out_dtype == x.dtype else None
    if full is not None:
        return scale_planes(full, scale, out_dtype)[..., :x.shape[3]]
    x = x.contiguous()
    y = torch.empty(x.shape, dtype=out_dtype, device=x.device)
    n, c, h, w = x.shape
    if scale is not None:
        scale = scale.to(torch.float32).contiguous()
        assert scale.numel() == n * c
    _lib.launched(lib.afcm_scale_planes(y.data_ptr(), x.data_ptr(), _lib.ptr(scale), _lib.dtype_code(x), _lib._DTYPES[out_dtype],
                                        n * c, h * w, _lib.stream_ptr(x)), 'scale_planes')
    return y


def plane_dot(a, b=None):
    lib = _lib.load()
    if b is not None:
        assert b.shape == a.shape and b.dtype == a.dtype
    lda = _rows.pitch_of(a)
    ldb = _rows.pitch_of(b) if b is not None else 0
    if (not (a.is_contiguous() and (b is None or b.is_contiguous())) and lda is not None and ldb is not None
            and a.shape[3] * a.element_size() >= 16 and (a.element_size() == 4 or a.shape[3] % 2 == 0)
            and a.data_ptr() % 4 == 0 and (b is None or b.data_ptr() % 4 == 0)):
        n, c, h, w = a.shape
        out = torch.empty([n, c], dtype=torch.float32, device=a.device)
        _lib.launched(lib.afcm_plane_dot_ld(out.data_ptr(), a.data_ptr(), _lib.ptr(b), _lib.dtype_code(a), n * c, h, w, lda, ldb, _lib.stream_ptr(a)),
                      'plane_dot')
        return out
    a = a.contiguous()
    if a.data_ptr() % 16:
        a = a.clone()
    n, c, h, w = a.shape
    if b is not None:
        b = b.contiguous()
        assert b.shape == a.shape and b.dtype == a.dtype
        if b.data_ptr() % 16:
            b = b.clone()
    out = torch.empty([n, c], dtype=torch.float32, device=a.device)
    _lib.launched(lib.afcm_plane_dot(out.data_ptr(), a.data_ptr(), _lib.ptr(b), _lib.dtype_code(a), n * c, h * w, _lib.stream_ptr(a)),
                  'plane_dot')
    return out


def plane_dot_gated(a, b, flags, out_scale, gz, next_scale=None, gskip=None):
    lib = _lib.load()
    assert b.shape == a.shape and b.dtype == a.dtype
    lda, ldb = _rows.pitch_of(a), _rows.pitch_of(b)
    n, c, h, w = a.shape
    ok = (lda is not None and ldb is not None and w * a.element_size() >= 16 and (a.element_size() == 4 or w % 2 == 0)
          and a.data_ptr() % 4 == 0 and b.data_ptr() % 4 == 0 and flags.dtype == torch.int32 and flags.is_contiguous()
          and tuple(flags.shape[:2]) == (n, c))
    if not ok:
        return plane_dot(a, b)
    f32 = torch.float32
    for t in (out_scale, gz, next_scale, gskip):
        assert t is None or (t.dtype == f32 and t.is_contiguous() and t.numel() == n * c)
    out = torch.empty([n, c], dtype=f32, device=a.device)
    _lib.launched(lib.afcm_plane_dot_gated_ld(out.data_ptr(), a.data_ptr(), b.data_ptr(), _lib.dtype_code(a), n * c, h, w, lda, ldb,
                                              flags.data_ptr(), int(flags.shape[2]), out_scale.data_ptr(), gz.data_ptr(), _lib.ptr(next_scale),
                                              _lib.ptr(gskip), _lib.stream_ptr(a)), 'plane_dot_gated')
    return out


FP32_SPLIT = (torch.float16, 3, 3, 3)
_SPLIT_TERMS = {
    3: ((1, 0), (0, 1), (0, 0)),
    6: ((2, 0), (0, 2), (1, 1), (1, 0), (0, 1), (0, 0)),
}


def _parts_fit(shape):
    n, c, h, w = [int(v) for v in shape]
    numel = n * c * h * w
    return (numel + 3) // 4 * 4 * 2 * 2 + c * h * w * 2 < (1 << 31)


def _split_plan(x, ks, cout=None, padding=None):
    if FP32_SPLIT is None or x.dtype != torch.float32 or ks != 3 or x.device.type != 'cuda' or x.ndim != 4 or x.shape[3] % 2:
        return None
    if not _parts_fit(x.shape):
        return None
    if cout is not None and padding is not None:
        p, q = x.shape[2] + 2 * padding - 2, x.shape[3] + 2 * padding - 2
        if q % 2 or not _parts_fit((x.shape[0], cout, p, q)):
            return None
    return FP32_SPLIT


_BOUND_POOL = {}


def _bound_word(device):
    slot = _BOUND_POOL.get(device)
    if slot is None or slot[1] >= slot[0].numel():
        slot = _BOUND_POOL[device] = [torch.zeros([1024], dtype=torch.int32, device=device), 0]
    word = slot[0][slot[1]:slot[1] + 1]
    slot[1] += 1
    return word


def amax_bits(x, scale=None, out=None):
    lib = _lib.load()
    assert x.dtype == torch.float32 and x.is_contiguous()
    word = _bound_word(x.device) if out is None else out
    if x.ndim == 4:
        planes, hw = x.shape[0] * x.shape[1], x.shape[2] * x.shape[3]
    else:
        planes, hw = 1, x.numel()
    if scale is not None:
        scale = scale.detach().to(torch.float32).contiguous()
        assert scale.numel() == planes
    _lib.launched(lib.afcm_amax_bits(word.data_ptr(), x.data_ptr(), planes, hw, _lib.ptr(scale), _lib.stream_ptr(x)), 'amax_bits')
    return word


def pow2_factor(word):
    b = word.view(torch.float32).double().cpu()
    if not bool(torch.isfinite(b).all()):
        return 1.0
    return float(2.0 ** (15 - torch.frexp(b.clamp_min(1e-30))[1].item()))


def split16(x, scale=None, nparts=2, dtype=torch.float16, bound=None):
    lib = _lib.load()
    x = x.contiguous()
    assert x.dtype == torch.float32 and x.ndim == 4 and nparts in (2, 3) and dtype in (torch.float16, torch.bfloat16)
    n, c, h, w = x.shape
    total = x.numel()
    stride = (total + 3) // 4 * 4
    buf = torch.empty([nparts, stride], dtype=dtype, device=x.device)
    if scale is not None:
        scale = scale.to(torch.float32).contiguous()
        assert scale.numel() == n * c
    if bound is not None:
        assert bound.dtype == torch.int32 and bound.numel() == 1 and bound.device == x.device
    _lib.launched(lib.afcm_split16(buf.data_ptr(), x.data_ptr(), _lib.ptr(scale), _lib.ptr(bound), _lib._DTYPES[dtype], n * c, h * w, nparts, stride,
                                   _lib.stream_ptr(x)), 'split16')
    return buf[:, :total].view(nparts, n, c, h, w)


def plane_dot_parts(parts, b, bound=None):
    lib = _lib.load()
    nparts, n, c, h, w = parts.shape
    b = b.contiguous()
    assert b.dtype == torch.float32 and tuple(b.shape) == (n, c, h, w) and parts.stride(1) == c * h * w
    out = torch.empty([n, c], dtype=torch.float32, device=b.device)
    _lib.launched(lib.afcm_plane_dot_parts(out.data_ptr(), parts.data_ptr(), parts.stride(0), nparts, b.data_ptr(), _lib._DTYPES[parts.dtype], n * c, h * w,
                                           _lib.ptr(bound), _lib.stream_ptr(b)), 'plane_dot_parts')
    return out


def _split_operand(x, scale, terms, dtype, bound=None):
    x = x.contiguous()
    if dtype == torch.float16 and bound is None:
        bound = amax_bits(x, scale)
    return split16(x, scale, _nparts(terms), dtype, bound if dtype == torch.float16 else None), (bound if dtype == torch.float16 else None)


def _nparts(*term_counts):
    return 1 + max(max(a, b) for t in term_counts for a, b in _SPLIT_TERMS[t])


def pack_weights_split(w, terms, dtype, transposed=False):
    lib = _lib.load()
    w = w.detach().to(torch.float32).contiguous()
    o, i = int(w.shape[0]), int(w.shape[1])
    assert tuple(w.shape[2:]) == (3, 3)
    rows, cols = (i, o) if transposed else (o, i)
    rows_pad = _pad64(rows)
    bound = amax_bits(w) if dtype == torch.float16 else None
    table = _SPLIT_TERMS[terms]
    bk = lib.afcm_conv2d_block_k_ks(_lib._DTYPES[dtype], 3)
    dst = torch.empty([terms * ((cols + bk - 1) // bk), 9, rows_pad, bk], dtype=dtype, device=w.device)
    code = sum(b << (4 * t) for t, (_, b) in enumerate(table))
    _lib.launched(lib.afcm_conv2d_pack_split(dst.data_ptr(), w.data_ptr(), _lib.ptr(bound), _lib._DTYPES[dtype], o, i, 1 if transposed else 0, rows_pad,
                                             terms, code, _lib.stream_ptr(w)), 'conv2d_pack_split')
    return dst, rows_pad, bound


def _conv_split(parts, wp, rows_pad, terms, oscale, cout, pad, obias=None, bounds=(None, None)):
    lib = _lib.load()
    nparts, n, cin, h, w = parts.shape
    table = _SPLIT_TERMS[terms]
    assert nparts > max(a for a, _ in table) and parts.dtype == wp.dtype and parts.stride(1) == cin * h * w
    bk = lib.afcm_conv2d_block_k_ks(_lib._DTYPES[parts.dtype], 3)
    assert tuple(wp.shape) == (terms * ((cin + bk - 1) // bk), 9, rows_pad, bk), 'the weight image does not belong to this split'
    p, q = h + 2 * pad - 2, w + 2 * pad - 2
    y = torch.empty([n, cout, p, q], dtype=torch.float32, device=parts.device)
    if oscale is not None:
        oscale = oscale.to(torch.float32).contiguous()
        assert oscale.numel() == n * cout
    if obias is not None:
        obias = obias.to(torch.float32).contiguous()
        assert obias.numel() == cout
    code = sum(a << (4 * t) for t, (a, _) in enumerate(table))
    span = profiling.span('conv2d', 2.0 * n * cout * cin * 9 * p * q)
    _lib.launched(lib.afcm_conv2d_split(y.data_ptr(), parts.data_ptr(), wp.data_ptr(), _lib.ptr(oscale), _lib.ptr(obias), _lib._DTYPES[parts.dtype], n, cin,
                                        cout, h, w, pad, rows_pad, terms, code, parts.stride(0), _lib.ptr(bounds[0]), _lib.ptr(bounds[1]),
                                        _lib.stream_ptr(parts)), 'conv2d_split')
    if span is not None:
        span.end()
    return y


def _wgrad_split(dy_parts, x_parts, cout, cin, pad, terms, bounds=(None, None)):
    dw = None
    framed = {}
    for a, b in _SPLIT_TERMS[terms]:
        if b not in framed:
            framed[b] = _frame_dy(dy_parts[b], 3, pad)
        dyb, padb = framed[b]
        d = _wgrad_raw(dyb, x_parts[a], cout, cin, 3, padb, work_share=1.0 / terms)
        dw = d if dw is None else dw.add_(d)
    if bounds[0] is not None or bounds[1] is not None:
        _lib.launched(_lib.load().afcm_unscale(dw.data_ptr(), dw.numel(), _lib.ptr(bounds[0]), _lib.ptr(bounds[1]), _lib.stream_ptr(dw)), 'unscale')
    return dw


def _pitch_conv(dtype, ks):
    return dtype in (torch.bfloat16, torch.float16) and ks == 3


def _pitch_wgrad(dtype, ks, pad):
    return dtype in (torch.bfloat16, torch.float16) and ((ks == 3 and pad == 2) or (ks == 1 and pad == 0))


def _conv_raw(x, wp, rows_pad, oscale, cout, ks, pad, obias=None, pitched_out=False):
    lib = _lib.load()
    n, cin, h, w = x.shape
    p, q = h + 2 * pad - ks + 1, w + 2 * pad - ks + 1
    if _pitch_conv(x.dtype, ks):
        x, xld = _rows.rows(x)
        y = _rows.empty([n, cout, p, q], x.dtype, x.device, pitched=pitched_out)
    else:
        x, xld = _rows.dense(x), w
        y = torch.empty([n, cout, p, q], dtype=x.dtype, device=x.device)
    yld = q if y.is_contiguous() else y.stride(2)
    if oscale is not None:
        oscale = oscale.to(torch.float32).contiguous()
    span = profiling.span('conv2d', 2.0 * n * cout * cin * ks * ks * p * q)
    if obias is not None:
        obias = obias.to(torch.float32).contiguous()
        assert obias.numel() == cout
    _lib.launched(lib.afcm_conv2d_ld(y.data_ptr(), x.data_ptr(), wp.data_ptr(), _lib.ptr(oscale), _lib.ptr(obias), _lib.dtype_code(x), n, cin, cout, h, w,
                                     ks, pad, rows_pad, 0 if xld == w else xld, 0 if yld == q else yld, _lib.stream_ptr(x)), 'conv2d')
    if span is not None:
        span.end()
    return y


_FRAME_WGRAD_MAX = 12 << 20


def _frame_dy(dy, ks, pad):
    if ks == 3 and pad == 1 and dy.dtype in (torch.bfloat16, torch.float16) and dy.numel() <= _FRAME_WGRAD_MAX:
        return torch.nn.functional.pad(dy, [1, 1, 1, 1]), 2
    return dy, pad


def _wgrad_raw(dy, x, cout, cin, ks, pad, work_share=1.0, dots_with=None):
    lib = _lib.load()
    n, _, h, w = x.shape
    work = work_share * 2.0 * n * cout * cin * ks * ks * (h + 2 * pad - ks + 1) * (w + 2 * pad - ks + 1)
    dy, pad = _frame_dy(dy, ks, pad)
    p = h + 2 * pad - ks + 1
    if _pitch_wgrad(x.dtype, ks, pad):
        (dy, lddy), (x, ldx) = _rows.rows(dy), _rows.rows(x)
    else:
        (dy, lddy), (x, ldx) = (_rows.dense(dy), dy.shape[3]), (_rows.dense(x), w)
    splits = lib.afcm_conv2d_wgrad_splits(n, cout, cin, p)
    dw = torch.empty([cout, cin, ks, ks], dtype=torch.float32, device=x.device)
    ws = torch.empty([splits, cout, cin, ks, ks], dtype=torch.float32, device=x.device)
    span = profiling.span('conv2d_wgrad', work)
    dots = None
    if dots_with is not None and x.dtype in (torch.bfloat16, torch.float16):
        wref = dots_with.detach().to(torch.float32).contiguous()
        dots = torch.empty([n, cin], dtype=torch.float32, device=x.device)
        rc = _lib.check(lib.afcm_conv2d_wgrad_dots_ld(dw.data_ptr(), dots.data_ptr(), ws.data_ptr(), dy.data_ptr(), x.data_ptr(), wref.data_ptr(),
                                                      _lib.dtype_code(x), n, cin, cout, h, w, ks, pad, 0 if lddy == dy.shape[3] else lddy,
                                                      0 if ldx == w else ldx, _lib.stream_ptr(x)), 'conv2d_wgrad_dots')
        if rc != 0:
            dots = None
    if dots is None:
        _lib.launched(lib.afcm_conv2d_wgrad_ld(dw.data_ptr(), ws.data_ptr(), dy.data_ptr(), x.data_ptr(), _lib.dtype_code(x), n, cin, cout,
                                               h, w, ks, pad, 0 if lddy == dy.shape[3] else lddy, 0 if ldx == w else ldx, _lib.stream_ptr(x)), 'conv2d_wgrad')
    if span is not None:
        span.end()
    return dw if dots_with is None else (dw, dots)


class _ScaledConv2d(torch.autograd.Function):

    @staticmethod
    def forward(ctx, x, w, in_scale, out_scale, padding, prescaled=False, link=None):
        ctx.link = link if (link is not None and prescaled) else None
        _lib.require_gpu(x, w, in_scale, out_scale)
        if x.ndim != 4 or w.ndim != 4 or x.shape[1] != w.shape[1]:
            raise RuntimeError(f'conv2d: incompatible shapes x{tuple(x.shape)} w{tuple(w.shape)}')
        if x.numel() == 0:
            raise RuntimeError('x is empty')
        _lib.dtype_code(x)
        cout, cin, ks, _ = w.shape
        x = x.contiguous()
        ctx.wpt = None
        plan = _split_plan(x, ks, cout, padding)
        if plan is not None:
            dt, tf = plan[0], plan[1]
            eff_in = in_scale if (in_scale is not None and not prescaled) else None
            parts, gsx = _split_operand(x, eff_in, tf, dt)
            wp, rows_pad, gsw = pack_weights_split(w, tf, dt)
            y = _conv_split(parts, wp, rows_pad, tf, out_scale, cout, padding, bounds=(gsx, gsw))
            keep_parts = (in_scale is not None or out_scale is not None) and _nparts(plan[3]) <= parts.shape[0]
            ctx.save_for_backward(parts if keep_parts else x, w, in_scale, out_scale, y if (out_scale is not None and ctx.needs_input_grad[3]) else None)
            ctx.padding = padding
            ctx.prescaled = bool(prescaled)
            ctx.split = plan
            ctx.kept_parts = keep_parts
            ctx.x_bound = gsx
            return y
        ctx.split = None
        xs = scale_planes(x, in_scale) if (in_scale is not None and not prescaled) else x
        if ctx.needs_input_grad[0] or ctx.needs_input_grad[2]:
            (wp, rows_pad), ctx.wpt = pack_weights_both(w, x.dtype)
        else:
            wp, rows_pad = pack_weights(w, x.dtype, 0)
        y = _conv_raw(xs, wp, rows_pad, out_scale, cout, ks, padding)
        ctx.save_for_backward(xs, w, in_scale, out_scale, y if (out_scale is not None and ctx.needs_input_grad[3]) else None)
        ctx.padding = padding
        ctx.prescaled = bool(prescaled)
        return y

    @staticmethod
    def backward(ctx, dy):
        xs, w, in_scale, out_scale, y = ctx.saved_tensors
        pad = ctx.padding
        if torch.is_grad_enabled() and (dy.requires_grad or xs.requires_grad or w.requires_grad):
            if in_scale is not None or out_scale is not None:
                raise RuntimeError('conv2d: second-order gradients are only built for the unscaled convolution')
            ks = int(w.shape[2])
            dx = dw = None
            if ctx.needs_input_grad[0]:
                dx = _ScaledConv2d.apply(dy, w.transpose(0, 1).flip([2, 3]), None, None, ks - 1 - pad, False)
            if ctx.needs_input_grad[1]:
                dw = _ConvWgrad.apply(dy, xs, ks, pad).to(w.dtype)
            return dx, dw, None, None, None, None, None
        dy = dy.detach()
        if ctx.prescaled:
            in_scale = None
        cout, cin, ks, _ = w.shape
        dy = dy.contiguous()
        dx = dw = d_in = d_out = None
        if ctx.split is not None:
            dt, td, tw = ctx.split[0], ctx.split[2], ctx.split[3]
            need_dx = ctx.needs_input_grad[0] or ctx.needs_input_grad[2]
            terms = [td] * bool(need_dx) + [tw] * bool(ctx.needs_input_grad[1])
            if terms:
                dparts, gsd = _split_operand(dy, out_scale, max(terms), dt)
            if need_dx:
                wpt, rows_pad, gsw = pack_weights_split(w, td, dt, transposed=True)
                dx = _conv_split(dparts, wpt, rows_pad, td, in_scale, cin, ks - 1 - pad, bounds=(gsd, gsw))
                if ctx.needs_input_grad[2] and in_scale is not None:
                    s1 = in_scale.to(torch.float32)
                    if ctx.kept_parts:
                        s2 = s1.square()
                        d_in = torch.where(s2 > 0, plane_dot_parts(xs, dx, ctx.x_bound) / s2.clamp_min(1e-30), torch.zeros_like(s2)).to(in_scale.dtype)
                    else:
                        d_in = torch.where(s1 != 0, plane_dot(xs, dx) / torch.where(s1 != 0, s1, torch.ones_like(s1)), torch.zeros_like(s1)).to(in_scale.dtype)
            if ctx.needs_input_grad[1]:
                if ctx.kept_parts:
                    xparts, gsx = xs, ctx.x_bound
                else:
                    xparts, gsx = _split_operand(xs, in_scale, tw, dt, bound=ctx.x_bound)
                dw = _wgrad_split(dparts, xparts, cout, cin, pad, tw, bounds=(gsd, gsx)).to(w.dtype)
            if ctx.needs_input_grad[3]:
                d_out = (plane_dot(dy, y) / out_scale.to(torch.float32)).to(out_scale.dtype)
            return dx, dw, d_in, d_out, None, None, None
        dys = scale_planes(dy, out_scale) if out_scale is not None else dy
        if ctx.needs_input_grad[0] or ctx.needs_input_grad[2]:
            wpt, rows_pad = ctx.wpt if (ctx.wpt is not None and ctx.wpt[0].dtype == dy.dtype) else pack_weights(w, dy.dtype, 1)
            dx = _conv_raw(dys, wpt, rows_pad, in_scale, cin, ks, ks - 1 - pad)
            if ctx.needs_input_grad[2] and in_scale is not None:
                s2 = in_scale.to(torch.float32).square()
                d_in = torch.where(s2 > 0, plane_dot(xs, dx) / s2.clamp_min(1e-30), torch.zeros_like(s2)).to(in_scale.dtype)
        if ctx.needs_input_grad[1]:
            if ctx.link is not None and ctx.link.want:
                dw, ctx.link.gz = _wgrad_raw(dys, xs, cout, cin, ks, pad, dots_with=w)
                dw = dw.to(w.dtype)
            else:
                dw = _wgrad_raw(dys, xs, cout, cin, ks, pad).to(w.dtype)
        if ctx.needs_input_grad[3]:
            d_out = (plane_dot(dy, y) / out_scale.to(torch.float32)).to(out_scale.dtype)
        return dx, dw, d_in, d_out, None, None, None


class _ConvWgrad(torch.autograd.Function):

    @staticmethod
    def forward(ctx, dy, x, ks, pad):
        dy, x = dy.contiguous(), x.contiguous()
        cout, cin = int(dy.shape[1]), int(x.shape[1])
        ctx.save_for_backward(dy, x)
        ctx.cfg = (ks, pad)
        plan = _split_plan(dy, ks) if _split_plan(x, ks) is not None else None
        if plan is not None:
            (dparts, gsd), (xparts, gsx) = _split_operand(dy, None, plan[3], plan[0]), _split_operand(x, None, plan[3], plan[0])
            return _wgrad_split(dparts, xparts, cout, cin, pad, plan[3], bounds=(gsd, gsx))
        return _wgrad_raw(dy, x, cout, cin, ks, pad)

    @staticmethod
    def backward(ctx, g):
        dy, x = ctx.saved_tensors
        ks, pad = ctx.cfg
        g_dy = g_x = None
        if ctx.needs_input_grad[0]:
            g_dy = _ScaledConv2d.apply(x, g, None, None, pad, False)
        if ctx.needs_input_grad[1]:
            g_x = _ScaledConv2d.apply(dy, g.transpose(0, 1).flip([2, 3]), None, None, ks - 1 - pad, False)
        return g_dy, g_x, None, None


_ONE_TAP = {}


def _one_tap(device):
    f = _ONE_TAP.get(device)
    if f is None:
        f = _ONE_TAP[device] = torch.ones([1, 1], dtype=torch.float32, device=device)
    return f


class _StridedConv2d(torch.autograd.Function):

    @staticmethod
    def forward(ctx, x, w, padding):
        _lib.require_gpu(x, w)
        lib = _lib.load()
# ... 160 lines not shown
```

afcm_amd/torch_utils/ops/fused_layer.py:

```python
import torch

from ... import _lib
from . import _rows
from . import conv2d as _conv
from . import filtered_lrelu as _flr


class _ConvFilteredLRelu(torch.autograd.Function):
    @staticmethod
    def forward(ctx, x, w, in_scale, out_scale, bias, fu, fd, skip, next_scale, conv_pad, cfg, prescaled, packed=None, fork=None, link_in=None, link_out=None):
        _lib.require_gpu(x, w, in_scale, out_scale, bias, fu, fd, skip, next_scale)
        cout, cin, ks, _ = w.shape
        xs = _conv.scale_planes(x, in_scale) if (in_scale is not None and not prescaled) else x
        ctx.wpt = None
        need_wpt = ctx.needs_input_grad[0] or (ctx.needs_input_grad[2] and not prescaled)
        if packed is not None and packed[0][0].dtype == x.dtype and (packed[1] is not None or not need_wpt):
            (wp, rows_pad), ctx.wpt = packed
            bk = wp.shape[3]
            assert tuple(wp.shape) == ((cin + bk - 1) // bk, ks * ks, rows_pad, bk) and rows_pad == (cout + 63) // 64 * 64, \
                f'packed weight image {tuple(wp.shape)} does not belong to a {tuple(w.shape)} weight'
        elif need_wpt:
            (wp, rows_pad), ctx.wpt = _conv.pack_weights_both(w, x.dtype)
        else:
            wp, rows_pad = _conv.pack_weights(w, x.dtype, 0)
        y = _conv._conv_raw(xs, wp, rows_pad, out_scale, cout, ks, conv_pad, obias=bias, pitched_out=True)
        need_grad = any(ctx.needs_input_grad[:5]) or ctx.needs_input_grad[7] or ctx.needs_input_grad[8]
        keep_y = out_scale is not None and ctx.needs_input_grad[3]
        flags = [] if (keep_y and need_grad and HOMOGENEOUS_DOT) else None
        z, signs, layout, _ = _flr._run(y, fu, fd, None, None, cfg, need_grad, oscale=next_scale, skip=skip, pitched_out=True, clamp_flags_out=flags)
        flags = flags[0] if flags else None
        keep_z = (next_scale is not None and ctx.needs_input_grad[8]) or flags is not None
        ctx.save_for_backward(xs, w, in_scale, out_scale, bias, fu, fd, signs, next_scale, y if keep_y else None, z if keep_z else None,
                              flags, skip if (flags is not None and skip is not None) else None)
        ctx.skip_by_fork = False
        if fork is not None and skip is not None and next_scale is not None and ctx.needs_input_grad[7]:
            fork.scale = next_scale.detach()
            ctx.skip_by_fork = True
        ctx.link_out = link_out if (link_out is not None and next_scale is not None) else None
        if ctx.link_out is not None:
            ctx.link_out.want, ctx.link_out.gz = True, None
        ctx.link_in = link_in if (link_in is not None and prescaled) else None
        ctx.meta = (conv_pad, cfg, bool(prescaled), layout, tuple(y.shape), tuple(z.shape), skip is not None)
        return z

    @staticmethod
    @torch.autograd.function.once_differentiable
    def backward(ctx, g):
        xs, w, in_scale, out_scale, bias, fu, fd, signs, next_scale, y, z, flags, skip = ctx.saved_tensors
        conv_pad, cfg, prescaled, layout, y_shape, z_shape, has_skip = ctx.meta
        cout, cin, ks, _ = w.shape
        f32 = torch.float32
        assert g.dtype in (torch.bfloat16, torch.float16)
        bcfg = _flr._backward_cfg(cfg, fu, fd, y_shape, z_shape, layout)
        dys, _, _, psum = _flr._run(g, fd, fu, None, signs, bcfg, False, want_plane_sum=True, oscale=out_scale, oscale2=next_scale, pitched_out=True)
        dx = dw = d_in = d_out = db = d_skip = d_next = None
        n, o = int(g.shape[0]), int(g.shape[1])
        want_db, want_next, want_out = ctx.needs_input_grad[4], ctx.needs_input_grad[8], ctx.needs_input_grad[3]
        if want_db or want_next or want_out:
            lib = _lib.load()
            gz = None
            if want_next or (want_out and flags is not None):
                if ctx.link_out is not None and ctx.link_out.gz is not None and tuple(ctx.link_out.gz.shape) == (n, o):
                    gz, ctx.link_out.gz = ctx.link_out.gz, None
                else:
                    gz = _conv.plane_dot(g, z)
            osc = None if out_scale is None else out_scale.to(f32).contiguous()
            nsc = None if next_scale is None else next_scale.to(f32).contiguous()
            if want_out and flags is not None:
                gsk = _conv.plane_dot(g, skip) if skip is not None else None
                dysy = _conv.plane_dot_gated(dys, y, flags, osc, gz, nsc, gsk)
            else:
                dysy = _conv.plane_dot(dys, y) if want_out else None
            db32 = torch.empty([o], dtype=f32, device=g.device) if want_db else None
            dn32 = torch.empty([n, o], dtype=f32, device=g.device) if want_next else None
            do32 = torch.empty([n, o], dtype=f32, device=g.device) if want_out else None
            b32 = None if bias is None else bias.to(f32).contiguous()
            _lib.launched(lib.afcm_layer_bwd_coefs(_lib.ptr(db32), _lib.ptr(dn32), _lib.ptr(do32), psum.data_ptr(), int(psum.shape[2]), _lib.ptr(osc),
                                                   _lib.ptr(nsc), _lib.ptr(b32), _lib.ptr(gz if want_next else None), _lib.ptr(dysy), n, o, _lib.stream_ptr(g)),
                          'layer_bwd_coefs')
            db = None if db32 is None else db32.to(bias.dtype)
            d_next = None if dn32 is None else dn32.to(next_scale.dtype)
            d_out = None if do32 is None else do32.to(out_scale.dtype)
        if has_skip and ctx.needs_input_grad[7]:
            d_skip = _conv.scale_planes(g, next_scale) if (next_scale is not None and not ctx.skip_by_fork) else g
        if ctx.needs_input_grad[0] or (ctx.needs_input_grad[2] and not prescaled):
            wpt, rows_pad = ctx.wpt if (ctx.wpt is not None and ctx.wpt[0].dtype == g.dtype) else _conv.pack_weights(w, g.dtype, 1)
            eff_in = None if prescaled else in_scale
            dx = _conv._conv_raw(dys, wpt, rows_pad, eff_in, cin, ks, ks - 1 - conv_pad, pitched_out=True)
            if ctx.needs_input_grad[2] and eff_in is not None:
                s2 = in_scale.to(f32).square()
                d_in = torch.where(s2 > 0, _conv.plane_dot(xs, dx) / s2.clamp_min(1e-30), torch.zeros_like(s2)).to(in_scale.dtype)
        if ctx.needs_input_grad[1]:
            if ctx.link_in is not None and ctx.link_in.want:
                dw, ctx.link_in.gz = _conv._wgrad_raw(dys, xs, cout, cin, ks, conv_pad, dots_with=w)
                dw = dw.to(w.dtype)
            else:
                dw = _conv._wgrad_raw(dys, xs, cout, cin, ks, conv_pad).to(w.dtype)
        return dx, dw, d_in, d_out, db, None, None, d_skip, d_next, None, None, None, None, None, None, None


HOMOGENEOUS_DOT = True



def _cfg(up, down, padding, gain, slope, clamp):
    px0, px1, py0, py1 = _flr._parse_padding(padding)
    return (int(up), int(down), px0, px1, py0, py1, float(gain), float(slope), float(clamp if clamp is not None else 'inf'), False, 0, 0, 0)


def available(x, w, fu, fd, up, down, padding, gain, slope, clamp, conv_pad):
    if w.shape[2] != 3 or x.dtype not in (torch.bfloat16, torch.float16) or x.device.type != 'cuda':
        return False
    yshape = [x.shape[0], w.shape[0], x.shape[2] + 2 * conv_pad - 2, x.shape[3] + 2 * conv_pad - 2]
    return _flr.matrix_core_available(yshape, x.dtype, x.device, fu, fd, _cfg(up, down, padding, gain, slope, clamp))


class LayerLink:
    __slots__ = ('want', 'gz')

    def __init__(self):
        self.want, self.gz = False, None


def conv_filtered_lrelu(x, w, in_scale, out_scale, bias, fu, fd, up, down, padding, gain, slope, clamp, conv_pad, skip=None,
                        next_scale=None, prescaled=False, packed=None, link_in=None, link_out=None):
    cfg = _cfg(up, down, padding, gain, slope, clamp)
    fork = getattr(skip, '_afcm_fork', None) if skip is not None else None
    return _ConvFilteredLRelu.apply(x, w, in_scale, out_scale, bias, fu, fd, skip, next_scale, int(conv_pad), cfg, bool(prescaled), packed, fork,
                                    link_in, link_out)


class _ForkState:
    __slots__ = ('scale', 'spent')

    def __init__(self):
        self.scale, self.spent = None, False


class _SkipFork(torch.autograd.Function):

    @staticmethod
    def forward(ctx, x, state):
        ctx.state = state
        return x.view_as(x), x.view_as(x)

    @staticmethod
    @torch.autograd.function.once_differentiable
    def backward(ctx, ga, gb):
        if ctx.state.spent:
            raise RuntimeError('skip_fork: the skip arm\'s style factor was consumed by an earlier backward over this graph; a second '
                               'backward (retain_graph=True) through the fused generator layers is not supported -- run the forward again')
        scale = ctx.state.scale
        ctx.state.scale, ctx.state.spent = None, scale is not None
        if gb is None:
            return ga, None
        if ga is None:
            return (gb if scale is None else _conv.scale_planes(gb, scale)), None
        out = None
        if ga.is_cuda and ga.dtype in (torch.bfloat16, torch.float16) and ga.dtype == gb.dtype and ga.shape == gb.shape:
            fa, fb = (_rows.whole_buffer(ga), _rows.whole_buffer(gb)) if not ga.is_contiguous() else (ga, gb if gb.is_contiguous() else None)
            if fa is not None and fb is not None and fa.shape == fb.shape:
                n, c, h, ld = fa.shape
                y = torch.empty_like(fa)
                sc = None if scale is None else scale.to(torch.float32).contiguous()
                rc = _lib.check(_lib.load().afcm_axpy_planes(y.data_ptr(), fa.data_ptr(), fb.data_ptr(), _lib.ptr(sc), _lib.dtype_code(fa), n * c, h * ld,
                                                            _lib.stream_ptr(fa)), 'axpy_planes')
                if rc == 0:
                    out = y[..., :ga.shape[3]]
        if out is None:
            out = ga + (gb if scale is None else _conv.scale_planes(gb, scale))
        return out, None


def skip_fork(x):
    if not (x.requires_grad and torch.is_grad_enabled()):
        return x, x
    state = _ForkState()
    a, b = _SkipFork.apply(x, state)
    b._afcm_fork = state
    return a, b
```

include/afcm_hip.h:

```cpp
#ifndef AFCM_HIP_H
#define AFCM_HIP_H

#include <stdint.h>

#ifdef __cplusplus
extern "C" {
#endif

#define AFCM_ABI_VERSION 13

enum { AFCM_F32 = 0, AFCM_F16 = 1, AFCM_BF16 = 2 };
enum { AFCM_OK = 0, AFCM_E_NOKERNEL = -1, AFCM_E_INVALID = -2 };
enum { AFCM_SIGNS_NONE = 0, AFCM_SIGNS_WRITE = 1, AFCM_SIGNS_READ = 2 };

int afcm_abi_version(void);
const char* afcm_last_error(void);
int afcm_noop(void* stream);

typedef struct afcm_filtered_lrelu_args {
    const void* x;
    void*       y;
    const void* b;
    uint8_t*    signs;
    const float* fu;
    const float* fd;
    int32_t dtype;
    int32_t n, c, xh, xw, yh, yw;
    int32_t fuw, fuh, fdw, fdh;
    int32_t up, down;
    int32_t px0, px1, py0, py1;
    int32_t sx, sy;
    int32_t sh, swb;
    float   gain, slope, clamp;
    int32_t flip_filter;
    int32_t sign_mode;
    void*   workspace;
    int32_t sign_layout;
    int32_t plane_sum_slots;
    float*  plane_sum;
    const float* oscale;
    const void*  skip;
    const float* oscale2;
    int32_t x_pitch, y_pitch, skip_pitch;
    int32_t row_pitch_ok;
    int32_t* clamp_flags;
} afcm_filtered_lrelu_args;

int afcm_filtered_lrelu_shapes(afcm_filtered_lrelu_args* a);
int afcm_filtered_lrelu(const afcm_filtered_lrelu_args* a, void* stream);

int64_t afcm_filtered_lrelu_workspace_bytes(void);
int afcm_filtered_lrelu_prepare(const afcm_filtered_lrelu_args* a, void* stream);

int afcm_filtered_lrelu_act(void* x, uint8_t* signs, int32_t dtype, int32_t n, int32_t c, int32_t h, int32_t w,
                            int32_t sh, int32_t swb, int32_t sx, int32_t sy, float gain, float slope, float clamp,
                            int32_t sign_mode, void* stream);

int afcm_upfirdn2d(void* y, const void* x, const float* f, int32_t dtype, int32_t n, int32_t c, int32_t xh, int32_t xw,
                   int32_t yh, int32_t yw, int32_t fh, int32_t fw, int32_t upx, int32_t upy, int32_t downx, int32_t downy,
                   int32_t padx0, int32_t pady0, int32_t flip, float gain, void* stream);

int afcm_bias_act(void* y, const void* x, const void* b, const void* xref, const void* yref, const void* dy,
                  int32_t dtype, int64_t numel, int64_t inner, int32_t nb, int32_t grad, int32_t act, float alpha,
                  float gain, float clamp, void* stream);



int afcm_conv2d_block_k(int32_t dtype);
int afcm_conv2d_block_k_ks(int32_t dtype, int32_t ks);

int afcm_conv2d_pack_weights(void* dst, const float* w, int32_t dtype, int32_t cout, int32_t cin, int32_t ks,
                             int32_t mode, int32_t rows_pad, void* stream);

int afcm_conv2d_pack_weights2(void* dst_fwd, void* dst_dgrad, const float* w, int32_t dtype, int32_t cout, int32_t cin, int32_t ks,
                              int32_t rows_pad_fwd, int32_t rows_pad_dgrad, void* stream);
int afcm_conv2d_pack_weights_bk(void* dst, const float* w, int32_t dtype, int32_t cout, int32_t cin, int32_t ks, int32_t mode,
                                int32_t rows_pad, int32_t block_k, void* stream);

int afcm_conv2d(void* y, const void* x, const void* wpacked, const float* oscale, const float* obias, int32_t dtype, int32_t n,
                int32_t cin, int32_t cout, int32_t h, int32_t w, int32_t ks, int32_t pad, int32_t rows_pad, void* stream);
int afcm_conv2d_ld(void* y, const void* x, const void* wpacked, const float* oscale, const float* obias, int32_t dtype, int32_t n,
                   int32_t cin, int32_t cout, int32_t h, int32_t w, int32_t ks, int32_t pad, int32_t rows_pad, int32_t x_pitch,
                   int32_t y_pitch, void* stream);

int afcm_conv2d_plan(int32_t dtype, int32_t n, int32_t cin, int32_t cout, int32_t h, int32_t w, int32_t ks, int32_t pad, int32_t x_pitch,
                     int32_t y_pitch, int32_t split, int32_t out[8]);

int afcm_conv2d_wgrad_splits(int32_t n, int32_t cout, int32_t cin, int32_t p_rows);
int afcm_conv2d_wgrad(float* dw, float* workspace, const void* dy, const void* x, int32_t dtype, int32_t n, int32_t cin,
                      int32_t cout, int32_t h, int32_t w, int32_t ks, int32_t pad, void* stream);
int afcm_conv2d_wgrad_ld(float* dw, float* workspace, const void* dy, const void* x, int32_t dtype, int32_t n, int32_t cin,
                         int32_t cout, int32_t h, int32_t w, int32_t ks, int32_t pad, int32_t dy_pitch, int32_t x_pitch, void* stream);
int afcm_conv2d_wgrad_dots_ld(float* dw, float* dots, float* workspace, const void* dy, const void* x, const float* wref, int32_t dtype, int32_t n,
                              int32_t cin, int32_t cout, int32_t h, int32_t w, int32_t ks, int32_t pad, int32_t dy_pitch, int32_t x_pitch,
                              void* stream);

int afcm_conv2d_wgrad_plan(int32_t dtype, int32_t n, int32_t cin, int32_t cout, int32_t h, int32_t w, int32_t ks, int32_t pad,
                           int32_t dy_pitch, int32_t x_pitch, int32_t dots, int32_t out[8]);

int afcm_scale_planes(void* y, const void* x, const float* scale, int32_t dtype_in, int32_t dtype_out, int64_t planes,
                      int32_t hw, void* stream);

int afcm_plane_dot(float* out, const void* a, const void* b, int32_t dtype, int64_t planes, int32_t hw, void* stream);
int afcm_plane_dot_ld(float* out, const void* a, const void* b, int32_t dtype, int64_t planes, int32_t h, int32_t w,
                      int32_t a_pitch, int32_t b_pitch, void* stream);
int afcm_plane_dot_gated_ld(float* out, const void* a, const void* b, int32_t dtype, int64_t planes, int32_t h, int32_t w,
                            int32_t a_pitch, int32_t b_pitch, const int32_t* flags, int32_t slots, const float* out_scale,
                            const float* gz, const float* next_scale, const float* gskip, void* stream);

int afcm_weight_norm_fwd(float* w_hat, float* wsq, float* scale, const float* w, int32_t cout, int32_t cin, int32_t kk, void* stream);
int afcm_weight_norm_bwd(float* dw, const float* g_hat, const float* g_wsq, const float* w_hat, const float* scale, int32_t cout,
                         int32_t cin, int32_t kk, void* stream);
int afcm_style_coefs_fwd(float* s_eff, float* d, float* r, const float* t, const float* wsq, const float* magnitude, int32_t n, int32_t cin,
                         int32_t cout, int32_t demodulate, void* stream);
int afcm_style_coefs_bwd(float* dt, float* g_wsq, float* workspace, const float* g_s, const float* g_d, const float* t, const float* d,
                         const float* wsq, const float* magnitude, const float* r, int32_t n, int32_t cin, int32_t cout, int32_t demodulate,
                         void* stream);

int afcm_layer_bwd_coefs(float* db, float* d_next, float* d_out, const float* psum, int32_t slots, const float* out_scale,
                         const float* next_scale, const float* bias, const float* gz, const float* dysy, int32_t n, int32_t cout,
                         void* stream);

typedef struct afcm_adam_entry {
    void*   p;
    void*   g;
    void*   m;
    void*   v;
    int64_t numel;
    int64_t chunk0;
} afcm_adam_entry;
int32_t afcm_adam_chunk_elems(void);
int afcm_adam_multi(const afcm_adam_entry* table, int32_t n, int64_t total_chunks, float step_size, float beta1, float beta2,
                    float one_minus_beta1, float one_minus_beta2, float bias_correction2_sqrt, float eps, float grad_scale, int32_t scrub, float posinf, float neginf,
                    int32_t write_grad, void* stream);
int afcm_adam_multi_capturable(const afcm_adam_entry* table_dev, int32_t n, int64_t total_chunks, float* step_dev, float lr, float beta1, float beta2,
                               float eps, float grad_scale, int32_t scrub, float posinf, float neginf, int32_t write_grad, void* stream);
int afcm_adam_multi_capturable_d(const afcm_adam_entry* table_dev, int32_t n, int64_t total_chunks, float* step_dev, double lr, double beta1, double beta2,
                                 float eps, float grad_scale, int32_t scrub, float posinf, float neginf, int32_t write_grad, void* stream);
int afcm_adam_multi_capturable_lr(const afcm_adam_entry* table_dev, int32_t n, int64_t total_chunks, float* step_dev, const double* lr_dev, double beta1,
                                  double beta2, float eps, float grad_scale, int32_t scrub, float posinf, float neginf, int32_t write_grad, void* stream);

#define AFCM_AFFINE_MAX 16
typedef struct afcm_affine_bank {
    int32_t layers, n, kw, kg;
    int64_t w_stride_n, w_stride_l;
    const float* w;
    const float* g;
    const float* weight[AFCM_AFFINE_MAX];
    const float* bias[AFCM_AFFINE_MAX];
    int32_t cout[AFCM_AFFINE_MAX];
    int32_t w_index[AFCM_AFFINE_MAX];
    float alpha[AFCM_AFFINE_MAX], beta[AFCM_AFFINE_MAX];
} afcm_affine_bank;
int64_t afcm_affine_bank_workspace_bytes(const afcm_affine_bank* a);
int afcm_affine_bank_fwd(const afcm_affine_bank* a, float* const* y, void* stream);
int afcm_affine_bank_bwd(const afcm_affine_bank* a, const float* const* dy, float* const* dweight, float* const* dbias, float* dws, float* dg,
                         void* workspace, void* stream);

#define AFCM_MODULATION_MAX 16
typedef struct afcm_modulation_layer {
    int32_t cout, cin, kk, demodulate;
    const float* w;
    const float* t;
    const float* magnitude;
    float* w_hat;
    float* wsq;
    float* scale;
    float* s_eff;
    float* d;
    float* r;
    const float* g_hat;
    const float* g_s;
    const float* g_d;
    float* dw;
    float* dt;
    float* workspace;
} afcm_modulation_layer;
int64_t afcm_modulation_bank_workspace_floats(int32_t n, int32_t cin, int32_t cout, int32_t demodulate);
int afcm_modulation_bank_fwd(const afcm_modulation_layer* layers, int32_t count, int32_t n, void* stream);
int afcm_modulation_bank_bwd(const afcm_modulation_layer* layers, int32_t count, int32_t n, void* stream);

#define AFCM_PACK_MAX 32
typedef struct afcm_pack_entry {
    void* dst_fwd;
    void* dst_dgrad;
    const float* w;
    int32_t cout, cin, rows_pad_fwd, rows_pad_dgrad;
} afcm_pack_entry;
int afcm_conv2d_pack_bank(const afcm_pack_entry* entries, int32_t count, int32_t dtype, int32_t ks, void* stream);

int afcm_amax_bits(uint32_t* out, const float* x, int64_t planes, int32_t hw, const float* scale, void* stream);
int afcm_split16(void* parts, const float* x, const float* scale, const uint32_t* bound, int32_t dtype, int64_t planes, int32_t hw,
                 int32_t nparts, int64_t part_stride, void* stream);
int afcm_unscale(float* t, int64_t numel, const uint32_t* bound_a, const uint32_t* bound_b, void* stream);
int afcm_plane_dot_parts(float* out, const void* parts, int64_t part_stride, int32_t nparts, const float* b, int32_t dtype, int64_t planes,
                         int32_t hw, const uint32_t* bound, void* stream);
int afcm_conv2d_pack_split(void* dst, const float* w, const uint32_t* bound, int32_t dtype, int32_t cout, int32_t cin, int32_t mode,
                           int32_t rows_pad, int32_t terms, uint32_t term_wparts, void* stream);
int afcm_conv2d_split(float* y, const void* x_parts, const void* wpacked, const float* oscale, const float* obias, int32_t dtype, int32_t n,
                      int32_t cin, int32_t cout, int32_t h, int32_t w, int32_t pad, int32_t rows_pad, int32_t terms, uint32_t term_parts,
                      int64_t part_stride, const uint32_t* bound_a, const uint32_t* bound_b, void* stream);

int afcm_conv2d_stride2(void* y, const void* x, const void* wpacked, int32_t dtype, int32_t n, int32_t cin, int32_t cout, int32_t h, int32_t w,
                        int32_t pad, int32_t rows_pad, void* stream);

int afcm_pool_blocks_fwd(float* y, const void* x, int32_t dtype, int64_t planes, int32_t h, int32_t w, void* stream);
int afcm_pool_blocks_bwd(void* dx, const float* gy, int32_t dtype, int64_t planes, int32_t h, int32_t w, void* stream);

int afcm_l1_partials(float* partials, const float* a, const float* b, int64_t numel, int32_t blocks, float weight, void* stream);
int afcm_l1_grad(float* ga, const float* a, const float* b, const float* gout, int64_t numel, float weight, void* stream);

int afcm_axpy_planes(void* y, const void* a, const void* b, const float* scale, int32_t dtype, int64_t planes, int32_t hw, void* stream);

int afcm_fc_act_fwd(float* y, const float* x, const float* w, const float* b, int32_t n, int32_t cin, int32_t cout, float alpha, float beta,
                    int32_t act, void* stream);
int afcm_fc_act_bwd(float* dx, float* dw, float* db, const float* gy, const float* y, const float* x, const float* w, int32_t n, int32_t cin,
                    int32_t cout, float alpha, float beta, int32_t act, void* stream);
int afcm_mapping_input_fwd(float* x0, const float* z, const float* c, const float* ew, const float* eb, int32_t n, int32_t zdim, int32_t cdim,
                           int32_t wdim, float alpha, float beta, void* stream);
int64_t afcm_mapping_input_bwd_workspace_bytes(int32_t n, int32_t wdim);
int afcm_mapping_input_bwd(float* dew, float* deb, const float* gx0, const float* c, const float* ew, const float* eb, int32_t n, int32_t zdim,
                           int32_t cdim, int32_t wdim, float alpha, float beta, void* workspace, void* stream);

int64_t afcm_plane_metrics_workspace_bytes(int64_t planes, int32_t h, int32_t w);
int afcm_plane_metrics(double* table, const void* ref, const void* test, int32_t dtype_ref, int32_t dtype_test, int64_t planes, int32_t h, int32_t w,
                       int64_t ref_stride_plane, int64_t ref_stride_row, int64_t ref_stride_col, int64_t test_stride_plane, int64_t test_stride_row,
                       int64_t test_stride_col, int32_t unit_map, double c1, double c2, void* workspace, void* stream);

enum { AFCM_SRC_U8 = 0, AFCM_SRC_I16 = 1, AFCM_SRC_F32 = 2, AFCM_SRC_F64 = 3 };

int afcm_slice_assemble(void* a, float* slice_idx, const void* src, int32_t src_dtype, int32_t out_dtype, int32_t depth, int32_t hs, int32_t ws,
                        int64_t src_stride_z, int32_t first, int32_t count, int32_t k, int32_t thickness, int32_t h, int32_t w, double min_value,
                        double max_value, void* stream);

int afcm_halo_accumulate(float* map, uint8_t* mask, const void* pred, int32_t dtype, int64_t stride_b, int64_t stride_c, int64_t stride_d,
                         int64_t stride_h, int64_t stride_w, int32_t channels, const int32_t* origins, int32_t table_len, int32_t first, int32_t count,
                         int32_t pd, int32_t ph, int32_t pw, int32_t halo_z, int32_t halo_y, int32_t halo_x, int32_t D, int32_t H, int32_t W,
                         int32_t map_channels, int32_t prediction_channel, int32_t z0, int32_t z1, int32_t y0, int32_t y1, int32_t x0, int32_t x1,
                         void* stream);

int64_t afcm_volume_ssim_workspace_bytes(int64_t volumes, int32_t d, int32_t h, int32_t w);
int afcm_volume_ssim(double* layers, const void* ref, const void* test, int32_t dtype_ref, int32_t dtype_test, int64_t volumes, int32_t d, int32_t h,
                     int32_t w, int64_t ref_stride_volume, int64_t ref_stride_z, int64_t ref_stride_y, int64_t ref_stride_x,
                     int64_t test_stride_volume, int64_t test_stride_z, int64_t test_stride_y, int64_t test_stride_x, int32_t unit_map, double c1,
                     double c2, void* workspace, void* stream);

int afcm_batch_assemble(void* a, void* b, float* slice_idx, const void* pool, int64_t pool_elems, int32_t src_dtype, const int64_t* vols,
                        int32_t n_vols, const int32_t* items, int32_t n_items, const int64_t* cursor, int32_t first, int32_t count, int32_t k, int32_t h,
                        int32_t w, int32_t out_dtype, double min_value, double max_value, void* stream);
int afcm_cursor_advance(int64_t* cursor, int64_t by, void* stream);

int afcm_batch_assemble_aug(void* a, void* b, float* slice_idx, const void* pool, int64_t pool_elems, int32_t src_dtype, const int64_t* vols,
                            int32_t n_vols, const int32_t* items, int32_t n_items, const double* augment, const int64_t* cursor, int32_t first,
                            int32_t count, int32_t k, int32_t h, int32_t w, int32_t out_dtype, double min_value, double max_value, void* stream);

#define AFCM_SCHEDULE_SLOTS 8
#define AFCM_EMA_LERP 0
#define AFCM_EMA_COPY 1
typedef struct afcm_ema_entry {
    void*       dst;
    const void* src;
    int64_t     numel;
    int64_t     chunk0;
    int32_t     kind;
    int32_t     reserved;
} afcm_ema_entry;
int afcm_schedule_advance(double* block, int64_t batch, double blur_init_sigma, double blur_fade_kimg, double ema_kimgs, double ema_ramp, void* stream);
int32_t afcm_gauss_blur_rmax(void);
int afcm_gauss_blur(float* y, const float* x, float* scratch, int64_t planes, int32_t h, int32_t w, double sigma, const double* block, void* stream);
int afcm_ema_multi(const afcm_ema_entry* table, int32_t n, int64_t total_chunks, double beta, const double* block, void* stream);

int afcm_rescale_plan(int64_t n, int32_t src_dtype, int32_t* plan);
int64_t afcm_rescale_workspace_bytes(int64_t n, int32_t src_dtype);
int afcm_rescale_intensity(uint8_t* out, double* stats, void* workspace, const void* volume, int32_t src_dtype, int32_t depth, int32_t h, int32_t w,
// ... 28 lines not shown
```

Measured before the change: 484.1 images/sec.

## Fuse layer backward coefficients into wgrad tail and dual plane dots

Adds a dual plane-dot kernel that computes <g,z> and <g,skip> in one pass over g. It also folds the per-layer backward coefficient computation (db, d_next, d_out) into the tail of the weight-gradient kernel, reading and writing native dtypes directly. This removes a separate coefficient launch, several fp32 staging casts and allocations, and one extra read of the gradient planes. In exchange the wgrad kernel grows more complex and gains extra parameters.

```diff
diff --git a/afcm_amd/_lib.py b/afcm_amd/_lib.py
--- a/afcm_amd/_lib.py
+++ b/afcm_amd/_lib.py
@@ -68,6 +68,11 @@
 class PackEntry(C.Structure):
     _fields_ = [('dst_fwd', C.c_void_p), ('dst_dgrad', C.c_void_p), ('w', C.c_void_p),
                 ('cout', C.c_int32), ('cin', C.c_int32), ('rows_pad_fwd', C.c_int32), ('rows_pad_dgrad', C.c_int32)]
+
+
+class LayerCoefs(C.Structure):
+    _fields_ = [(k, C.c_void_p) for k in ('db', 'd_next', 'd_out', 'psum', 'out_scale', 'next_scale', 'bias', 'gz', 'dysy')] + [
+        (k, C.c_int32) for k in ('slots', 'n', 'cout', 'out_scale_dtype', 'next_scale_dtype', 'bias_dtype', 'db_dtype', 'd_next_dtype', 'd_out_dtype')]
 
 
 _lib = None
@@ -99,9 +104,12 @@
     'afcm_conv2d_wgrad': (C.c_int, [_vp, _vp, _vp, _vp, _i32, _i32, _i32, _i32, _i32, _i32, _i32, _i32, _vp]),
     'afcm_conv2d_wgrad_ld': (C.c_int, [_vp, _vp, _vp, _vp, _i32, _i32, _i32, _i32, _i32, _i32, _i32, _i32, _i32, _i32, _vp]),
     'afcm_conv2d_wgrad_dots_ld': (C.c_int, [_vp, _vp, _vp, _vp, _vp, _vp, _i32, _i32, _i32, _i32, _i32, _i32, _i32, _i32, _i32, _i32, _vp]),
+    'afcm_conv2d_wgrad_tail_ld': (C.c_int, [_vp, _vp, _vp, _vp, _vp, _vp, _i32, _i32, _i32, _i32, _i32, _i32, _i32, _i32, _i32, _i32, C.POINTER(LayerCoefs), _vp]),
     'afcm_scale_planes': (C.c_int, [_vp, _vp, _vp, _i32, _i32, _i64, _i32, _vp]),
     'afcm_plane_dot': (C.c_int, [_vp, _vp, _vp, _i32, _i64, _i32, _vp]),
     'afcm_plane_dot_ld': (C.c_int, [_vp, _vp, _vp, _i32, _i64, _i32, _i32, _i32, _i32, _vp]),
+    'afcm_plane_dot2': (C.c_int, [_vp, _vp, _vp, _vp, _vp, _i32, _i64, _i32, _vp]),
+    'afcm_plane_dot2_ld': (C.c_int, [_vp, _vp, _vp, _vp, _vp, _i32, _i64, _i32, _i32, _i32, _i32, _i32, _vp]),
     'afcm_split16': (C.c_int, [_vp, _vp, _vp, _vp, _i32, _i64, _i32, _i32, _i64, _vp]),
     'afcm_conv2d_split': (C.c_int, [_vp, _vp, _vp, _vp, _vp, _i32, _i32, _i32, _i32, _i32, _i32, _i32, _i32, _i32, C.c_uint32, _i64, _vp, _vp, _vp]),
     'afcm_amax_bits': (C.c_int, [_vp, _vp, _i64, _i32, _vp, _vp]),
diff --git a/afcm_amd/csrc/common.h b/afcm_amd/csrc/common.h
--- a/afcm_amd/csrc/common.h
+++ b/afcm_amd/csrc/common.h
@@ -45,6 +45,44 @@
 constexpr int cmax(int a, int b) { return a > b ? a : b; }
 constexpr int odd4(int a) { return ((a / 4) % 2 == 1) ? a : a + 4; }
 
+__device__ __forceinline__ float coef_load(const void* p, int dt, size_t i) {
+    return dt == AFCM_F32 ? ((const float*)p)[i] : dt == AFCM_F16 ? to_f32(((const f16_t*)p)[i]) : to_f32(((const bf16_t*)p)[i]);
+}
+__device__ __forceinline__ void coef_store(void* p, int dt, size_t i, float v) {
+    asm volatile("" : "+v"(v));
+    if (dt == AFCM_F32) ((float*)p)[i] = v;
+    else if (dt == AFCM_F16) ((f16_t*)p)[i] = from_f32<f16_t>(v);
+    else ((bf16_t*)p)[i] = from_f32<bf16_t>(v);
+}
+__device__ __forceinline__ void layer_bwd_coefs_wave(const afcm_layer_coefs& c, int o, int lane) {
+    const float b = c.bias ? coef_load(c.bias, c.bias_dtype, o) : 0.f;
+    float acc = 0.f;
+    for (int n = lane; n < c.n; n += 64) {
+        const size_t idx = (size_t)n * c.cout + o;
+        float ps = 0.f;
+        for (int k = 0; k < c.slots; k++) ps += c.psum[idx * c.slots + k];
+        const float d = c.out_scale ? coef_load(c.out_scale, c.out_scale_dtype, idx) : 1.f;
+        acc += ps / d;
+        if (c.d_next) {
+            const float ns = coef_load(c.next_scale, c.next_scale_dtype, idx);
+            coef_store(c.d_next, c.d_next_dtype, idx, ns != 0.f ? c.gz[idx] / ns : 0.f);
+        }
+        if (c.d_out) coef_store(c.d_out, c.d_out_dtype, idx, (c.dysy[idx] - b * ps) / (d * d));
+    }
+#pragma unroll
+    for (int off = 32; off > 0; off >>= 1) acc += __shfl_xor(acc, off, 64);
+    if (c.db && lane == 0) coef_store(c.db, c.db_dtype, o, acc);
+}
+
+static inline int layer_coefs_check(const afcm_layer_coefs& c) {
+    AFCM_REQUIRE(c.psum && c.slots > 0 && c.n > 0 && c.cout > 0, "layer_bwd_coefs: bad arguments");
+    AFCM_REQUIRE(!c.d_next || (c.next_scale && c.gz), "layer_bwd_coefs: d_next needs next_scale and <g, z>");
+    AFCM_REQUIRE(!c.d_out || (c.out_scale && c.dysy), "layer_bwd_coefs: d_out needs out_scale and <dys, y>");
+    for (int dt : {c.out_scale_dtype, c.next_scale_dtype, c.bias_dtype, c.db_dtype, c.d_next_dtype, c.d_out_dtype})
+        AFCM_REQUIRE(dt == AFCM_F32 || dt == AFCM_F16 || dt == AFCM_BF16, "layer_bwd_coefs: bad dtype code %d", dt);
+    return AFCM_OK;
+}
+
 __host__ __device__ __forceinline__ int floor_div(int a, int b) {
     int q = a / b;
     return (a % b != 0 && (a < 0)) ? q - 1 : q;
diff --git a/afcm_amd/csrc/conv2d_planes.hip b/afcm_amd/csrc/conv2d_planes.hip
--- a/afcm_amd/csrc/conv2d_planes.hip
+++ b/afcm_amd/csrc/conv2d_planes.hip
@@ -185,30 +185,34 @@
     }
 }
 
-template <typename T>
+template <typename T, bool DUAL = false>
 __global__ __launch_bounds__(256) void plane_dot_kernel(float* __restrict__ out, const T* __restrict__ a, const T* __restrict__ b,
-                                                        long long planes, int hw) {
+                                                        long long planes, int hw, float* __restrict__ out2, const T* __restrict__ c) {
     constexpr int E = 16 / (int)sizeof(T);
     union V16 { uint4 u; T v[E]; };
     __shared__ float part[4];
+    __shared__ float part2[DUAL ? 4 : 1];
     const long long plane = blockIdx.x;
     if (plane >= planes) return;
     const long long off = plane * hw;
     const T* ap = a + off;
     const T* bp = b ? b + off : nullptr;
+    const T* cp = DUAL ? c + off : nullptr;
     int head = (int)((E - (off % E)) % E);
     if (head > hw) head = hw;
     const int nv = (hw - head) / E;
-    float s0 = 0.f, s1 = 0.f;
+    float s0 = 0.f, s1 = 0.f, t0 = 0.f, t1 = 0.f;
     {
         const int tail0 = head + nv * E;
         int i = -1;
         if ((int)threadIdx.x < head) i = threadIdx.x;
         else if ((int)threadIdx.x - head < hw - tail0) i = tail0 + (int)threadIdx.x - head;
         if (i >= 0) s0 = to_f32(ap[i]) * (bp ? to_f32(bp[i]) : 1.f);
+        if (DUAL && i >= 0) t0 = to_f32(ap[i]) * to_f32(cp[i]);
     }
     const uint4* av = (const uint4*)(ap + head);
     const uint4* bv = bp ? (const uint4*)(bp + head) : nullptr;
+    const uint4* cv = DUAL ? (const uint4*)(cp + head) : nullptr;
     int i = threadIdx.x;
     if (bv) {
         for (; i + 768 < nv; i += 1024) {
@@ -220,6 +224,15 @@
                 s0 = fmaf(to_f32(a0.v[e]), to_f32(b0.v[e]), s0); s1 = fmaf(to_f32(a1.v[e]), to_f32(b1.v[e]), s1);
                 s0 = fmaf(to_f32(a2.v[e]), to_f32(b2.v[e]), s0); s1 = fmaf(to_f32(a3.v[e]), to_f32(b3.v[e]), s1);
             }
+            if (DUAL) {
+                V16 c0, c1, c2, c3;
+                c0.u = cv[i]; c1.u = cv[i + 256]; c2.u = cv[i + 512]; c3.u = cv[i + 768];
+#pragma unroll
+                for (int e = 0; e < E; e++) {
+                    t0 = fmaf(to_f32(a0.v[e]), to_f32(c0.v[e]), t0); t1 = fmaf(to_f32(a1.v[e]), to_f32(c1.v[e]), t1);
+                    t0 = fmaf(to_f32(a2.v[e]), to_f32(c2.v[e]), t0); t1 = fmaf(to_f32(a3.v[e]), to_f32(c3.v[e]), t1);
+                }
+            }
         }
     }
     for (; i + 256 < nv; i += 512) {
@@ -233,6 +246,12 @@
 #pragma unroll
             for (int e = 0; e < E; e++) { s0 += to_f32(a0.v[e]); s1 += to_f32(a1.v[e]); }
         }
+        if (DUAL) {
+            V16 c0, c1;
+            c0.u = cv[i]; c1.u = cv[i + 256];
+#pragma unroll
+            for (int e = 0; e < E; e++) { t0 = fmaf(to_f32(a0.v[e]), to_f32(c0.v[e]), t0); t1 = fmaf(to_f32(a1.v[e]), to_f32(c1.v[e]), t1); }
+        }
     }
     if (i < nv) {
         V16 a0, b0;
@@ -245,18 +264,34 @@
 #pragma unroll
             for (int e = 0; e < E; e++) s0 += to_f32(a0.v[e]);
         }
-    }
-    float s = s0 + s1;
+        if (DUAL) {
+            V16 c0;
+            c0.u = cv[i];
+#pragma unroll
+            for (int e = 0; e < E; e++) t0 = fmaf(to_f32(a0.v[e]), to_f32(c0.v[e]), t0);
+        }
+    }
+    float s = s0 + s1, t = t0 + t1;
 #pragma unroll
     for (int off2 = 32; off2 > 0; off2 >>= 1) s += __shfl_down(s, off2, 64);
-    if ((threadIdx.x & 63) == 0) part[threadIdx.x >> 6] = s;
+    if (DUAL) {
+#pragma unroll
+        for (int off2 = 32; off2 > 0; off2 >>= 1) t += __shfl_down(t, off2, 64);
+    }
+    if ((threadIdx.x & 63) == 0) {
+        part[threadIdx.x >> 6] = s;
+        if (DUAL) part2[threadIdx.x >> 6] = t;
+    }
     __syncthreads();
-    if (threadIdx.x == 0) out[plane] = part[0] + part[1] + part[2] + part[3];
-}
-
-template <typename T>
+    if (threadIdx.x == 0) {
+        out[plane] = part[0] + part[1] + part[2] + part[3];
+        if (DUAL) out2[plane] = part2[0] + part2[1] + part2[2] + part2[3];
+    }
+}
+
+template <typename T, bool DUAL = false>
 __global__ __launch_bounds__(256) void plane_dot_wave_kernel(float* __restrict__ out, const T* __restrict__ a, const T* __restrict__ b,
-                                                             long long planes, int hw) {
+                                                             long long planes, int hw, float* __restrict__ out2, const T* __restrict__ c) {
     constexpr int E = 16 / (int)sizeof(T);
     union V16 { uint4 u; T v[E]; };
     const int lane = threadIdx.x & 63;
@@ -265,19 +300,22 @@
     const long long off = plane * hw;
     const T* ap = a + off;
     const T* bp = b ? b + off : nullptr;
+    const T* cp = DUAL ? c + off : nullptr;
     int head = (int)((E - (off % E)) % E);
     if (head > hw) head = hw;
     const int nv = (hw - head) / E;
-    float s0 = 0.f, s1 = 0.f;
+    float s0 = 0.f, s1 = 0.f, t0 = 0.f, t1 = 0.f;
     {
         const int tail0 = head + nv * E;
         int i = -1;
         if (lane < head) i = lane;
         else if (lane - head < hw - tail0) i = tail0 + lane - head;
         if (i >= 0) s0 = to_f32(ap[i]) * (bp ? to_f32(bp[i]) : 1.f);
+        if (DUAL && i >= 0) t0 = to_f32(ap[i]) * to_f32(cp[i]);
     }
     const uint4* av = (const uint4*)(ap + head);
     const uint4* bv = bp ? (const uint4*)(bp + head) : nullptr;
+    const uint4* cv = DUAL ? (const uint4*)(cp + head) : nullptr;
     int i = lane;
     for (; i + 64 < nv; i += 128) {
         V16 a0, a1, b0, b1;
@@ -290,6 +328,12 @@
 #pragma unroll
             for (int e = 0; e < E; e++) { s0 += to_f32(a0.v[e]); s1 += to_f32(a1.v[e]); }
         }
+        if (DUAL) {
+            V16 c0, c1;
+            c0.u = cv[i]; c1.u = cv[i + 64];
+#pragma unroll
+            for (int e = 0; e < E; e++) { t0 = fmaf(to_f32(a0.v[e]), to_f32(c0.v[e]), t0); t1 = fmaf(to_f32(a1.v[e]), to_f32(c1.v[e]), t1); }
+        }
     }
     if (i < nv) {
         V16 a0, b0;
@@ -302,11 +346,24 @@
 #pragma unroll
             for (int e = 0; e < E; e++) s0 += to_f32(a0.v[e]);
         }
-    }
-    float s = s0 + s1;
+        if (DUAL) {
+            V16 c0;
+            c0.u = cv[i];
+#pragma unroll
+            for (int e = 0; e < E; e++) t0 = fmaf(to_f32(a0.v[e]), to_f32(c0.v[e]), t0);
+        }
+    }
+    float s = s0 + s1, t = t0 + t1;
 #pragma unroll
     for (int off2 = 32; off2 > 0; off2 >>= 1) s += __shfl_down(s, off2, 64);
-    if (lane == 0) out[plane] = s;
+    if (DUAL) {
+#pragma unroll
+        for (int off2 = 32; off2 > 0; off2 >>= 1) t += __shfl_down(t, off2, 64);
+    }
+    if (lane == 0) {
+        out[plane] = s;
+        if (DUAL) out2[plane] = t;
+    }
 }
 
 struct PlaneGate {
@@ -314,12 +371,14 @@
     int slots;
     const float *osc, *gz, *nsc, *gsk;
 };
-template <typename T, bool PER_WAVE>
+template <typename T, bool PER_WAVE, bool DUAL = false>
 __global__ __launch_bounds__(256) void plane_dot_rows_kernel(float* __restrict__ out, const T* __restrict__ a, const T* __restrict__ b,
-                                                             long long planes, int h, int w, int lda, int ldb, PlaneGate gate) {
+                                                             long long planes, int h, int w, int lda, int ldb, PlaneGate gate,
+                                                             float* __restrict__ out2, const T* __restrict__ c, int ldc) {
     constexpr int E = 16 / (int)sizeof(T);
     union V16 { uint4 u; T v[E]; };
     __shared__ float part[4];
+    __shared__ float part2[DUAL ? 4 : 1];
     const int nthr = PER_WAVE ? 64 : 256;
     const int t = PER_WAVE ? (int)(threadIdx.x & 63) : (int)threadIdx.x;
     const long long plane = PER_WAVE ? (long long)blockIdx.x * 4 + (threadIdx.x >> 6) : (long long)blockIdx.x;
@@ -340,9 +399,10 @@
     const unsigned magic = nvec > 1 ? (unsigned)((0x100000000ull + (unsigned)nvec - 1) / (unsigned)nvec) : 0u;
     const T* ap = a + plane * h * lda;
     const T* bp = b ? b + plane * h * ldb : nullptr;
-    float s0 = 0.f, s1 = 0.f;
+    const T* cp = DUAL ? c + plane * h * ldc : nullptr;
+    float s0 = 0.f, s1 = 0.f, t0 = 0.f, t1 = 0.f;
     for (int i0 = t; i0 < total; i0 += 4 * nthr) {
-        V16 av[4], bv[4];
+        V16 av[4], bv[4], cv[DUAL ? 4 : 1];
         int skip[4];
 #pragma unroll
         for (int u = 0; u < 4; u++) {
@@ -355,6 +415,7 @@
             skip[u] = i < total ? col - colc : E;
             av[u].u = *(const uint4*)(ap + (size_t)row * lda + colc);
             if (bp) bv[u].u = *(const uint4*)(bp + (size_t)row * ldb + colc);
+            if (DUAL) cv[u].u = *(const uint4*)(cp + (size_t)row * ldc + colc);
         }
 #pragma unroll
         for (int u = 0; u < 4; u++) {
@@ -363,18 +424,35 @@
                 const float x = e >= skip[u] ? to_f32(av[u].v[e]) : 0.f;
                 const float y = bp ? to_f32(bv[u].v[e]) : 1.f;
                 if (u & 1) s1 = fmaf(x, e >= skip[u] ? y : 0.f, s1); else s0 = fmaf(x, e >= skip[u] ? y : 0.f, s0);
+                if (DUAL) {
+                    const float z = to_f32(cv[u].v[e]);
+                    if (u & 1) t1 = fmaf(x, e >= skip[u] ? z : 0.f, t1); else t0 = fmaf(x, e >= skip[u] ? z : 0.f, t0);
+                }
             }
         }
     }
-    float s = s0 + s1;
+    float s = s0 + s1, r = t0 + t1;
 #pragma unroll
     for (int off2 = 32; off2 > 0; off2 >>= 1) s += __shfl_down(s, off2, 64);
+    if (DUAL) {
+#pragma unroll
+        for (int off2 = 32; off2 > 0; off2 >>= 1) r += __shfl_down(r, off2, 64);
+    }
     if (PER_WAVE) {
-        if ((threadIdx.x & 63) == 0) out[plane] = s;
+        if ((threadIdx.x & 63) == 0) {
+            out[plane] = s;
+            if (DUAL) out2[plane] = r;
+        }
     } else {
-        if ((threadIdx.x & 63) == 0) part[threadIdx.x >> 6] = s;
+        if ((threadIdx.x & 63) == 0) {
+            part[threadIdx.x >> 6] = s;
+            if (DUAL) part2[threadIdx.x >> 6] = r;
+        }
         __syncthreads();
-        if (threadIdx.x == 0) out[plane] = part[0] + part[1] + part[2] + part[3];
+        if (threadIdx.x == 0) {
+            out[plane] = part[0] + part[1] + part[2] + part[3];
+            if (DUAL) out2[plane] = part2[0] + part2[1] + part2[2] + part2[3];
+        }
     }
 }
 
@@ -462,17 +540,19 @@
     return hip_status(hipGetLastError());
 }
 
-extern "C" int afcm_plane_dot(float* out, const void* a, const void* b, int32_t dtype, int64_t planes, int32_t hw, void* stream) {
+static int plane_dot_dense(float* out, float* out2, const void* a, const void* b, const void* c, int32_t dtype, int64_t planes, int32_t hw, void* stream) {
     AFCM_REQUIRE(out != nullptr && a != nullptr && planes > 0 && hw > 0, "plane_dot: empty input");
     AFCM_REQUIRE(planes < (1ll << 31), "plane_dot: too many planes");
-    AFCM_REQUIRE((((uintptr_t)a | (uintptr_t)b) & 15) == 0, "plane_dot: operands must be 16-byte aligned");
+    AFCM_REQUIRE((((uintptr_t)a | (uintptr_t)b | (uintptr_t)c) & 15) == 0, "plane_dot: operands must be 16-byte aligned");
     hipStream_t st = (hipStream_t)stream;
     const int esize = dtype == AFCM_F32 ? 4 : 2;
     const bool per_wave = (long long)hw * esize <= 16384;
+    const bool dual = out2 != nullptr;
     dim3 grid((unsigned)(per_wave ? (planes + 3) / 4 : planes)), block(256);
-#define AFCM_PD(T) do { \
-        if (per_wave) hipLaunchKernelGGL((plane_dot_wave_kernel<T>), grid, block, 0, st, out, (const T*)a, (const T*)b, (long long)planes, hw); \
-        else hipLaunchKernelGGL((plane_dot_kernel<T>), grid, block, 0, st, out, (const T*)a, (const T*)b, (long long)planes, hw); } while (0)
+#define AFCM_PD_(T, D) do { \
+        if (per_wave) hipLaunchKernelGGL((plane_dot_wave_kernel<T, D>), grid, block, 0, st, out, (const T*)a, (const T*)b, (long long)planes, hw, out2, (const T*)c); \
+        else hipLaunchKernelGGL((plane_dot_kernel<T, D>), grid, block, 0, st, out, (const T*)a, (const T*)b, (long long)planes, hw, out2, (const T*)c); } while (0)
+#define AFCM_PD(T) do { if (dual) AFCM_PD_(T, true); else AFCM_PD_(T, false); } while (0)
     switch (dtype) {
         case AFCM_F32: AFCM_PD(float); break;
         case AFCM_F16: AFCM_PD(f16_t); break;
@@ -480,25 +560,39 @@
         default: set_error("plane_dot: bad dtype"); return AFCM_E_INVALID;
     }
 #undef AFCM_PD
-    return hip_status(hipGetLastError());
+#undef AFCM_PD_
+    return hip_status(hipGetLastError());
+}
+
+extern "C" int afcm_plane_dot(float* out, const void* a, const void* b, int32_t dtype, int64_t planes, int32_t hw, void* stream) {
+    return plane_dot_dense(out, nullptr, a, b, nullptr, dtype, planes, hw, stream);
+}
+
+extern "C" int afcm_plane_dot2(float* out_b, float* out_c, const void* a, const void* b, const void* c, int32_t dtype, int64_t planes, int32_t hw,
+                               void* stream) {
+    AFCM_REQUIRE(out_b != nullptr && out_c != nullptr && b != nullptr && c != nullptr, "plane_dot2: null pointer");
+    return plane_dot_dense(out_b, out_c, a, b, c, dtype, planes, hw, stream);
 }
 
 static int plane_dot_rows(float* out, const void* a, const void* b, int32_t dtype, int64_t planes, int32_t h, int32_t w,
-                          int32_t a_pitch, int32_t b_pitch, const PlaneGate& gate, void* stream) {
+                          int32_t a_pitch, int32_t b_pitch, const PlaneGate& gate, void* stream, float* out2 = nullptr, const void* c = nullptr,
+                          int32_t c_pitch = 0) {
     AFCM_REQUIRE(out != nullptr && a != nullptr && planes > 0 && h > 0 && w > 0, "plane_dot: empty input");
     AFCM_REQUIRE(planes < (1ll << 31), "plane_dot: too many planes");
     const int esize = dtype == AFCM_F32 ? 4 : 2;
-    const int lda = a_pitch ? a_pitch : w, ldb = b_pitch ? b_pitch : w;
-    AFCM_REQUIRE(lda >= w && ldb >= w, "plane_dot: row pitches %d / %d are below the width %d", lda, ldb, w);
+    const int lda = a_pitch ? a_pitch : w, ldb = b_pitch ? b_pitch : w, ldc = c_pitch ? c_pitch : w;
+    const bool dual = out2 != nullptr;
+    AFCM_REQUIRE(lda >= w && ldb >= w && ldc >= w, "plane_dot: row pitches %d / %d / %d are below the width %d", lda, ldb, ldc, w);
     AFCM_REQUIRE(w >= 16 / esize, "plane_dot: rows of %d elements are shorter than one 16-byte vector", w);
-    AFCM_REQUIRE((((uintptr_t)a | (uintptr_t)b) & 3) == 0 && (esize == 4 || ((w | lda | ldb) & 1) == 0), "plane_dot: rows must start on 4-byte boundaries");
-    AFCM_REQUIRE((long long)h * (lda > ldb ? lda : ldb) < (1ll << 31) / 16, "plane_dot: plane is out of range");
+    AFCM_REQUIRE((((uintptr_t)a | (uintptr_t)b | (uintptr_t)c) & 3) == 0 && (esize == 4 || ((w | lda | ldb | ldc) & 1) == 0), "plane_dot: rows must start on 4-byte boundaries");
+    AFCM_REQUIRE((long long)h * (lda > ldb ? lda : ldb) < (1ll << 31) / 16 && (long long)h * ldc < (1ll << 31) / 16, "plane_dot: plane is out of range");
     hipStream_t st = (hipStream_t)stream;
     const bool per_wave = (long long)h * w * esize <= 16384;
     dim3 grid((unsigned)(per_wave ? (planes + 3) / 4 : planes)), block(256);
-#define AFCM_PDR(T) do { \
-        if (per_wave) hipLaunchKernelGGL((plane_dot_rows_kernel<T, true>), grid, block, 0, st, out, (const T*)a, (const T*)b, (long long)planes, h, w, lda, ldb, gate); \
-        else hipLaunchKernelGGL((plane_dot_rows_kernel<T, false>), grid, block, 0, st, out, (const T*)a, (const T*)b, (long long)planes, h, w, lda, ldb, gate); } while (0)
+#define AFCM_PDR_(T, D) do { \
+        if (per_wave) hipLaunchKernelGGL((plane_dot_rows_kernel<T, true, D>), grid, block, 0, st, out, (const T*)a, (const T*)b, (long long)planes, h, w, lda, ldb, gate, out2, (const T*)c, ldc); \
+        else hipLaunchKernelGGL((plane_dot_rows_kernel<T, false, D>), grid, block, 0, st, out, (const T*)a, (const T*)b, (long long)planes, h, w, lda, ldb, gate, out2, (const T*)c, ldc); } while (0)
+#define AFCM_PDR(T) do { if (dual) AFCM_PDR_(T, true); else AFCM_PDR_(T, false); } while (0)
     switch (dtype) {
         case AFCM_F32: AFCM_PDR(float); break;
         case AFCM_F16: AFCM_PDR(f16_t); break;
@@ -506,7 +600,15 @@
         default: set_error("plane_dot: bad dtype"); return AFCM_E_INVALID;
     }
 #undef AFCM_PDR
-    return hip_status(hipGetLastError());
+#undef AFCM_PDR_
+    return hip_status(hipGetLastError());
+}
+
+extern "C" int afcm_plane_dot2_ld(float* out_b, float* out_c, const void* a, const void* b, const void* c, int32_t dtype, int64_t planes, int32_t h,
+                                  int32_t w, int32_t a_pitch, int32_t b_pitch, int32_t c_pitch, void* stream) {
+    AFCM_REQUIRE(out_b != nullptr && out_c != nullptr && b != nullptr && c != nullptr, "plane_dot2: null pointer");
+    return plane_dot_rows(out_b, a, b, dtype, planes, h, w, a_pitch, b_pitch, PlaneGate{nullptr, 0, nullptr, nullptr, nullptr, nullptr}, stream, out_c, c,
+                          c_pitch);
 }
 
 extern "C" int afcm_plane_dot_ld(float* out, const void* a, const void* b, int32_t dtype, int64_t planes, int32_t h, int32_t w,
diff --git a/afcm_amd/csrc/conv2d_wgrad.hip b/afcm_amd/csrc/conv2d_wgrad.hip
--- a/afcm_amd/csrc/conv2d_wgrad.hip
+++ b/afcm_amd/csrc/conv2d_wgrad.hip
@@ -861,21 +861,24 @@
 }
 
 struct WgradSlabs { int splits; };
-__global__ __launch_bounds__(256) void wgrad_reduce_kernel(float* __restrict__ dw, const float* __restrict__ part, long long numel, WgradSlabs w) {
-    for (long long idx = (long long)blockIdx.x * blockDim.x + threadIdx.x; idx < numel; idx += (long long)gridDim.x * blockDim.x) {
+__device__ __forceinline__ void wgrad_reduce_body(int bid, int nblocks, float* __restrict__ dw, const float* __restrict__ part, long long numel, WgradSlabs w) {
+    for (long long idx = (long long)bid * blockDim.x + threadIdx.x; idx < numel; idx += (long long)nblocks * blockDim.x) {
         float s = 0.f;
         for (int k = 0; k < w.splits; k++) s += part[(size_t)k * numel + idx];
         dw[idx] = s;
     }
 }
+__global__ __launch_bounds__(256) void wgrad_reduce_kernel(float* __restrict__ dw, const float* __restrict__ part, long long numel, WgradSlabs w) {
+    wgrad_reduce_body((int)blockIdx.x, (int)gridDim.x, dw, part, numel, w);
+}
 
 template <int COLS>
-__global__ __launch_bounds__(256) void wgrad_reduce4_kernel(float* __restrict__ dw, const float* __restrict__ part, long long numel4, WgradSlabs w) {
+__device__ __forceinline__ void wgrad_reduce4_body(int bid, float* __restrict__ dw, const float* __restrict__ part, long long numel4, WgradSlabs w) {
     constexpr int GROUPS = 256 / COLS;
     typedef __attribute__((ext_vector_type(4))) float f32x4v;
     __shared__ f32x4v red[GROUPS][COLS];
     const int col = threadIdx.x % COLS, grp = threadIdx.x / COLS;
-    const long long c4 = (long long)blockIdx.x * COLS + col;
+    const long long c4 = (long long)bid * COLS + col;
     f32x4v s0 = {0.f, 0.f, 0.f, 0.f}, s1 = s0;
     if (c4 < numel4) {
         const f32x4v* src = (const f32x4v*)part + c4;
@@ -901,14 +904,18 @@
         ((f32x4v*)dw)[c4] = s0;
     }
 }
+template <int COLS>
+__global__ __launch_bounds__(256) void wgrad_reduce4_kernel(float* __restrict__ dw, const float* __restrict__ part, long long numel4, WgradSlabs w) {
+    wgrad_reduce4_body<COLS>((int)blockIdx.x, dw, part, numel4, w);
+}
 
 
 template <typename T, int KK>
-__global__ __launch_bounds__(1024) void wgrad_reduce_dots_kernel(float* __restrict__ dw, float* __restrict__ dots, const float* __restrict__ part,
-                                                                 const float* __restrict__ w, int N, int O, int I, int splits_img) {
+__device__ __forceinline__ void wgrad_reduce_dots_body(int i, float* __restrict__ dw, float* __restrict__ dots, const float* __restrict__ part,
+                                                       const float* __restrict__ w, int N, int O, int I, int splits_img) {
     constexpr int NW = 16;
     __shared__ float red[NW - 1][64][KK];
-    const int i = blockIdx.x, lane = threadIdx.x & 63, q = threadIdx.x >> 6;
+    const int lane = threadIdx.x & 63, q = threadIdx.x >> 6;
     const size_t slab = (size_t)O * I * KK;
     float dotp[4];
 #pragma unroll
@@ -962,6 +969,32 @@
         for (int off = 32; off > 0; off >>= 1) d += __shfl_xor(d, off);
         if (lane == 0) dots[(size_t)n * I + i] = d;
     }
+}
+template <typename T, int KK>
+__global__ __launch_bounds__(1024) void wgrad_reduce_dots_kernel(float* __restrict__ dw, float* __restrict__ dots, const float* __restrict__ part,
+                                                                 const float* __restrict__ w, int N, int O, int I, int splits_img) {
+    wgrad_reduce_dots_body<T, KK>((int)blockIdx.x, dw, dots, part, w, N, O, I, splits_img);
+}
+
+__global__ __launch_bounds__(256) void wgrad_tail_reduce_kernel(float* __restrict__ dw, const float* __restrict__ part, long long numel, WgradSlabs w,
+                                                                int cblocks, const afcm_layer_coefs c) {
+    if ((int)blockIdx.x >= cblocks) { wgrad_reduce_body((int)blockIdx.x - cblocks, (int)gridDim.x - cblocks, dw, part, numel, w); return; }
+    const int o = (int)blockIdx.x * 4 + (int)(threadIdx.x >> 6);
+    if (o < c.cout) layer_bwd_coefs_wave(c, o, (int)(threadIdx.x & 63));
+}
+template <int COLS>
+__global__ __launch_bounds__(256) void wgrad_tail_reduce4_kernel(float* __restrict__ dw, const float* __restrict__ part, long long numel4, WgradSlabs w,
+                                                                 int cblocks, const afcm_layer_coefs c) {
+    if ((int)blockIdx.x >= cblocks) { wgrad_reduce4_body<COLS>((int)blockIdx.x - cblocks, dw, part, numel4, w); return; }
+    const int o = (int)blockIdx.x * 4 + (int)(threadIdx.x >> 6);
+    if (o < c.cout) layer_bwd_coefs_wave(c, o, (int)(threadIdx.x & 63));
+}
+template <typename T, int KK>
+__global__ __launch_bounds__(1024) void wgrad_tail_dots_kernel(float* __restrict__ dw, float* __restrict__ dots, const float* __restrict__ part,
+                                                               const float* __restrict__ w, int N, int O, int I, int splits_img, int cblocks, const afcm_layer_coefs c) {
+    if ((int)blockIdx.x >= cblocks) { wgrad_reduce_dots_body<T, KK>((int)blockIdx.x - cblocks, dw, dots, part, w, N, O, I, splits_img); return; }
+    const int o = (int)blockIdx.x * 16 + (int)(threadIdx.x >> 6);
+    if (o < c.cout) layer_bwd_coefs_wave(c, o, (int)(threadIdx.x & 63));
 }
 }
 
@@ -1029,8 +1062,13 @@
 }
 
 static int wgrad_impl(float* dw, float* workspace, const void* dy, const void* x, int32_t dtype, int32_t n, int32_t cin,
-                      int32_t cout, int32_t h, int32_t w, int32_t ks, int32_t pad, int32_t dy_pitch, int32_t x_pitch, float* dots, const float* wref, void* stream) {
+                      int32_t cout, int32_t h, int32_t w, int32_t ks, int32_t pad, int32_t dy_pitch, int32_t x_pitch, float* dots, const float* wref, void* stream,
+                      const afcm_layer_coefs* tail = nullptr) {
     AFCM_REQUIRE(dw != nullptr && workspace != nullptr && dy != nullptr && x != nullptr, "conv2d_wgrad: null pointer");
+    if (tail != nullptr) {
+        const int trc = layer_coefs_check(*tail);
+        if (trc != AFCM_OK) return trc;
+    }
     AFCM_REQUIRE(dtype == AFCM_F32 || dtype == AFCM_F16 || dtype == AFCM_BF16, "x must be float32, float16 or bfloat16");
     AFCM_REQUIRE(ks == 1 || ks == 3, "only 1x1 and 3x3 kernels are supported");
     AFCM_REQUIRE(pad >= 0 && pad <= ks - 1, "padding must be in [0, k-1]");
@@ -1082,7 +1120,13 @@
         const dim3 rgrid((unsigned)cin), rblock(1024);
 #define AFCM_RD(T) do { if (ks == 3) hipLaunchKernelGGL((wgrad_reduce_dots_kernel<T, 9>), rgrid, rblock, 0, st, dw, dots, (const float*)workspace, wref, n, cout, cin, p.splits_img); \
                         else hipLaunchKernelGGL((wgrad_reduce_dots_kernel<T, 1>), rgrid, rblock, 0, st, dw, dots, (const float*)workspace, wref, n, cout, cin, p.splits_img); } while (0)
-        if (dtype == AFCM_F16) AFCM_RD(f16_t); else AFCM_RD(bf16_t);
+#define AFCM_RDT(T) do { const int tb = cdiv(tail->cout, 16); const dim3 tgrid((unsigned)(cin + tb)); \
+                         if (ks == 3) hipLaunchKernelGGL((wgrad_tail_dots_kernel<T, 9>), tgrid, rblock, 0, st, dw, dots, (const float*)workspace, wref, n, cout, cin, p.splits_img, tb, *tail); \
+                         else hipLaunchKernelGGL((wgrad_tail_dots_kernel<T, 1>), tgrid, rblock, 0, st, dw, dots, (const float*)workspace, wref, n, cout, cin, p.splits_img, tb, *tail); } while (0)
+        if (tail != nullptr) { if (dtype == AFCM_F16) AFCM_RDT(f16_t); else AFCM_RDT(bf16_t); }
+        else if (dtype == AFCM_F16) AFCM_RD(f16_t);
+        else AFCM_RD(bf16_t);
+#undef AFCM_RDT
 #undef AFCM_RD
         return hip_status(hipGetLastError());
     }
@@ -1091,9 +1135,18 @@
     if (rb > 2048) rb = 2048;
     if (pl.reduce != kWgReduceScalar && (((uintptr_t)dw | (uintptr_t)workspace) & 15) == 0) {
         const long long n4 = numel / 4;
-        if (pl.reduce == kWgReduce4x16) hipLaunchKernelGGL(wgrad_reduce4_kernel<16>, dim3((unsigned)cdiv(n4, 16)), dim3(256), 0, st, dw, (const float*)workspace, n4, slabs);
+        if (tail != nullptr) {
+            const int tb = cdiv(tail->cout, 4);
+#define AFCM_R4T(COLS) hipLaunchKernelGGL(wgrad_tail_reduce4_kernel<COLS>, dim3((unsigned)(cdiv(n4, COLS) + tb)), dim3(256), 0, st, dw, (const float*)workspace, n4, slabs, tb, *tail)
+            if (pl.reduce == kWgReduce4x16) AFCM_R4T(16);
+            else if (pl.reduce == kWgReduce4x64) AFCM_R4T(64);
+            else AFCM_R4T(256);
+#undef AFCM_R4T
+        } else if (pl.reduce == kWgReduce4x16) hipLaunchKernelGGL(wgrad_reduce4_kernel<16>, dim3((unsigned)cdiv(n4, 16)), dim3(256), 0, st, dw, (const float*)workspace, n4, slabs);
         else if (pl.reduce == kWgReduce4x64) hipLaunchKernelGGL(wgrad_reduce4_kernel<64>, dim3((unsigned)cdiv(n4, 64)), dim3(256), 0, st, dw, (const float*)workspace, n4, slabs);
         else hipLaunchKernelGGL(wgrad_reduce4_kernel<256>, dim3((unsigned)cdiv(n4, 256)), dim3(256), 0, st, dw, (const float*)workspace, n4, slabs);
+    } else if (tail != nullptr) {
+        hipLaunchKernelGGL(wgrad_tail_reduce_kernel, dim3((unsigned)(rb + cdiv(tail->cout, 4))), dim3(256), 0, st, dw, (const float*)workspace, numel, slabs, cdiv(tail->cout, 4), *tail);
     } else {
         hipLaunchKernelGGL(wgrad_reduce_kernel, dim3((unsigned)rb), dim3(256), 0, st, dw, (const float*)workspace, numel, slabs);
     }
@@ -1110,6 +1163,13 @@
                                          int32_t x_pitch, void* stream) {
     AFCM_REQUIRE(dots != nullptr, "conv2d_wgrad_dots: dots must be non-null");
     return wgrad_impl(dw, workspace, dy, x, dtype, n, cin, cout, h, w, ks, pad, dy_pitch, x_pitch, dots, wref, stream);
+}
+
+extern "C" int afcm_conv2d_wgrad_tail_ld(float* dw, float* dots, float* workspace, const void* dy, const void* x, const float* wref, int32_t dtype,
+                                         int32_t n, int32_t cin, int32_t cout, int32_t h, int32_t w, int32_t ks, int32_t pad, int32_t dy_pitch,
+                                         int32_t x_pitch, const afcm_layer_coefs* tail, void* stream) {
+    AFCM_REQUIRE(tail != nullptr, "conv2d_wgrad_tail: the layer's coefficient arguments are missing");
+    return wgrad_impl(dw, workspace, dy, x, dtype, n, cin, cout, h, w, ks, pad, dy_pitch, x_pitch, dots, wref, stream, tail);
 }
 
 extern "C" int afcm_conv2d_wgrad_plan(int32_t dtype, int32_t n, int32_t cin, int32_t cout, int32_t h, int32_t w, int32_t ks, int32_t pad,
diff --git a/afcm_amd/csrc/modulation.hip b/afcm_amd/csrc/modulation.hip
--- a/afcm_amd/csrc/modulation.hip
+++ b/afcm_amd/csrc/modulation.hip
@@ -247,28 +247,8 @@
     style_coefs_bwd2_body((int)blockIdx.x, dt, g_wsq, G, Q, partial, t, r_in, N, I, O, demod, NP);
 }
 
-__global__ __launch_bounds__(64) void layer_bwd_coefs_kernel(float* __restrict__ db, float* __restrict__ d_next, float* __restrict__ d_out,
-                                                             const float* __restrict__ psum, int slots, const float* __restrict__ out_scale,
-                                                             const float* __restrict__ next_scale, const float* __restrict__ bias,
-                                                             const float* __restrict__ gz, const float* __restrict__ dysy, int N, int O) {
-    const int o = blockIdx.x;
-    const float b = bias ? bias[o] : 0.f;
-    float acc = 0.f;
-    for (int n = threadIdx.x; n < N; n += 64) {
-        const size_t idx = (size_t)n * O + o;
-        float ps = 0.f;
-        for (int k = 0; k < slots; k++) ps += psum[idx * slots + k];
-        const float d = out_scale ? out_scale[idx] : 1.f;
-        acc += ps / d;
-        if (d_next) {
-            const float ns = next_scale[idx];
-            d_next[idx] = ns != 0.f ? gz[idx] / ns : 0.f;
-        }
-        if (d_out) d_out[idx] = (dysy[idx] - b * ps) / (d * d);
-    }
-#pragma unroll
-    for (int off = 32; off > 0; off >>= 1) acc += __shfl_xor(acc, off, 64);
-    if (db && threadIdx.x == 0) db[o] = acc;
+__global__ __launch_bounds__(64) void layer_bwd_coefs_kernel(const afcm_layer_coefs c) {
+    layer_bwd_coefs_wave(c, (int)blockIdx.x, (int)threadIdx.x);
 }
 
 struct ModBank {
@@ -348,11 +328,11 @@
 extern "C" int afcm_layer_bwd_coefs(float* db, float* d_next, float* d_out, const float* psum, int32_t slots, const float* out_scale,
                                     const float* next_scale, const float* bias, const float* gz, const float* dysy, int32_t n, int32_t cout,
                                     void* stream) {
-    AFCM_REQUIRE(psum && slots > 0 && n > 0 && cout > 0, "layer_bwd_coefs: bad arguments");
-    AFCM_REQUIRE(!d_next || (next_scale && gz), "layer_bwd_coefs: d_next needs next_scale and <g, z>");
-    AFCM_REQUIRE(!d_out || (out_scale && dysy), "layer_bwd_coefs: d_out needs out_scale and <dys, y>");
-    hipLaunchKernelGGL(layer_bwd_coefs_kernel, dim3(cout), dim3(64), 0, (hipStream_t)stream, db, d_next, d_out, psum, slots, out_scale, next_scale,
-                       bias, gz, dysy, n, cout);
+    const afcm_layer_coefs c{db, d_next, d_out, psum, out_scale, next_scale, bias, gz, dysy, slots, n, cout,
+                             AFCM_F32, AFCM_F32, AFCM_F32, AFCM_F32, AFCM_F32, AFCM_F32};
+    const int rc = layer_coefs_check(c);
+    if (rc != AFCM_OK) return rc;
+    hipLaunchKernelGGL(layer_bwd_coefs_kernel, dim3(cout), dim3(64), 0, (hipStream_t)stream, c);
     return hip_status(hipGetLastError());
 }
 
diff --git a/afcm_amd/torch_utils/ops/conv2d.py b/afcm_amd/torch_utils/ops/conv2d.py
--- a/afcm_amd/torch_utils/ops/conv2d.py
+++ b/afcm_amd/torch_utils/ops/conv2d.py
@@ -112,6 +112,31 @@
     return out
 
 
+def _rows_route(a, b):
+    lda, ldb = _rows.pitch_of(a), _rows.pitch_of(b)
+    return (not (a.is_contiguous() and b.is_contiguous()) and lda is not None and ldb is not None
+            and a.shape[3] * a.element_size() >= 16 and (a.element_size() == 4 or a.shape[3] % 2 == 0)
+            and a.data_ptr() % 4 == 0 and b.data_ptr() % 4 == 0)
+
+
+def plane_dot2(a, b, c):
+    lib = _lib.load()
+    assert b.shape == a.shape and b.dtype == a.dtype and c.shape == a.shape and c.dtype == a.dtype
+    n, ch, h, w = a.shape
+    rows_b, rows_c = _rows_route(a, b), _rows_route(a, c)
+    if rows_b and rows_c:
+        ob, oc = (torch.empty([n, ch], dtype=torch.float32, device=a.device) for _ in range(2))
+        _lib.launched(lib.afcm_plane_dot2_ld(ob.data_ptr(), oc.data_ptr(), a.data_ptr(), b.data_ptr(), c.data_ptr(), _lib.dtype_code(a), n * ch, h, w,
+                                             _rows.pitch_of(a), _rows.pitch_of(b), _rows.pitch_of(c), _lib.stream_ptr(a)), 'plane_dot2')
+        return ob, oc
+    if not rows_b and not rows_c and all(t.is_contiguous() and t.data_ptr() % 16 == 0 for t in (a, b, c)):
+        ob, oc = (torch.empty([n, ch], dtype=torch.float32, device=a.device) for _ in range(2))
+        _lib.launched(lib.afcm_plane_dot2(ob.data_ptr(), oc.data_ptr(), a.data_ptr(), b.data_ptr(), c.data_ptr(), _lib.dtype_code(a), n * ch, h * w,
+                                          _lib.stream_ptr(a)), 'plane_dot2')
+        return ob, oc
+    return plane_dot(a, b), plane_dot(a, c)
+
+
 def plane_dot_gated(a, b, flags, out_scale, gz, next_scale=None, gskip=None):
     lib = _lib.load()
     assert b.shape == a.shape and b.dtype == a.dtype
@@ -328,7 +353,7 @@
     return dy, pad
 
 
-def _wgrad_raw(dy, x, cout, cin, ks, pad, work_share=1.0, dots_with=None):
+def _wgrad_raw(dy, x, cout, cin, ks, pad, work_share=1.0, dots_with=None, tail=None):
     lib = _lib.load()
     n, _, h, w = x.shape
     work = work_share * 2.0 * n * cout * cin * ks * ks * (h + 2 * pad - ks + 1) * (w + 2 * pad - ks + 1)
@@ -346,12 +371,21 @@
     if dots_with is not None and x.dtype in (torch.bfloat16, torch.float16):
         wref = dots_with.detach().to(torch.float32).contiguous()
         dots = torch.empty([n, cin], dtype=torch.float32, device=x.device)
-        rc = _lib.check(lib.afcm_conv2d_wgrad_dots_ld(dw.data_ptr(), dots.data_ptr(), ws.data_ptr(), dy.data_ptr(), x.data_ptr(), wref.data_ptr(),
-                                                      _lib.dtype_code(x), n, cin, cout, h, w, ks, pad, 0 if lddy == dy.shape[3] else lddy,
-                                                      0 if ldx == w else ldx, _lib.stream_ptr(x)), 'conv2d_wgrad_dots')
+        if tail is not None:
+            rc = _lib.check(lib.afcm_conv2d_wgrad_tail_ld(dw.data_ptr(), dots.data_ptr(), ws.data_ptr(), dy.data_ptr(), x.data_ptr(), wref.data_ptr(),
+                                                          _lib.dtype_code(x), n, cin, cout, h, w, ks, pad, 0 if lddy == dy.shape[3] else lddy,
+                                                          0 if ldx == w else ldx, tail, _lib.stream_ptr(x)), 'conv2d_wgrad_tail')
+        else:
+            rc = _lib.check(lib.afcm_conv2d_wgrad_dots_ld(dw.data_ptr(), dots.data_ptr(), ws.data_ptr(), dy.data_ptr(), x.data_ptr(), wref.data_ptr(),
+                                                          _lib.dtype_code(x), n, cin, cout, h, w, ks, pad, 0 if lddy == dy.shape[3] else lddy,
+                                                          0 if ldx == w else ldx, _lib.stream_ptr(x)), 'conv2d_wgrad_dots')
         if rc != 0:
             dots = None
-    if dots is None:
+    if dots is None and tail is not None:
+        _lib.launched(lib.afcm_conv2d_wgrad_tail_ld(dw.data_ptr(), None, ws.data_ptr(), dy.data_ptr(), x.data_ptr(), None, _lib.dtype_code(x), n, cin,
+                                                    cout, h, w, ks, pad, 0 if lddy == dy.shape[3] else lddy, 0 if ldx == w else ldx, tail,
+                                                    _lib.stream_ptr(x)), 'conv2d_wgrad_tail')
+    elif dots is None:
         _lib.launched(lib.afcm_conv2d_wgrad_ld(dw.data_ptr(), ws.data_ptr(), dy.data_ptr(), x.data_ptr(), _lib.dtype_code(x), n, cin, cout,
                                                h, w, ks, pad, 0 if lddy == dy.shape[3] else lddy, 0 if ldx == w else ldx, _lib.stream_ptr(x)), 'conv2d_wgrad')
     if span is not None:
diff --git a/afcm_amd/torch_utils/ops/fused_layer.py b/afcm_amd/torch_utils/ops/fused_layer.py
--- a/afcm_amd/torch_utils/ops/fused_layer.py
+++ b/afcm_amd/torch_utils/ops/fused_layer.py
@@ -56,31 +56,47 @@
         dx = dw = d_in = d_out = db = d_skip = d_next = None
         n, o = int(g.shape[0]), int(g.shape[1])
         want_db, want_next, want_out = ctx.needs_input_grad[4], ctx.needs_input_grad[8], ctx.needs_input_grad[3]
+        tail = keep = None
         if want_db or want_next or want_out:
-            lib = _lib.load()
-            gz = None
-            if want_next or (want_out and flags is not None):
+            gz = gsk = None
+            by_homogeneity = want_out and flags is not None
+            if want_next or by_homogeneity:
                 if ctx.link_out is not None and ctx.link_out.gz is not None and tuple(ctx.link_out.gz.shape) == (n, o):
                     gz, ctx.link_out.gz = ctx.link_out.gz, None
+                elif by_homogeneity and skip is not None:
+                    gz, gsk = _conv.plane_dot2(g, z, skip)
                 else:
                     gz = _conv.plane_dot(g, z)
-            osc = None if out_scale is None else out_scale.to(f32).contiguous()
-            nsc = None if next_scale is None else next_scale.to(f32).contiguous()
-            if want_out and flags is not None:
-                gsk = _conv.plane_dot(g, skip) if skip is not None else None
-                dysy = _conv.plane_dot_gated(dys, y, flags, osc, gz, nsc, gsk)
+            if by_homogeneity:
+                if skip is not None and gsk is None:
+                    gsk = _conv.plane_dot(g, skip)
+                dysy = _conv.plane_dot_gated(dys, y, flags, out_scale.to(f32).contiguous(), gz, None if next_scale is None else next_scale.to(f32).contiguous(), gsk)
             else:
                 dysy = _conv.plane_dot(dys, y) if want_out else None
-            db32 = torch.empty([o], dtype=f32, device=g.device) if want_db else None
-            dn32 = torch.empty([n, o], dtype=f32, device=g.device) if want_next else None
-            do32 = torch.empty([n, o], dtype=f32, device=g.device) if want_out else None
-            b32 = None if bias is None else bias.to(f32).contiguous()
-            _lib.launched(lib.afcm_layer_bwd_coefs(_lib.ptr(db32), _lib.ptr(dn32), _lib.ptr(do32), psum.data_ptr(), int(psum.shape[2]), _lib.ptr(osc),
-                                                   _lib.ptr(nsc), _lib.ptr(b32), _lib.ptr(gz if want_next else None), _lib.ptr(dysy), n, o, _lib.stream_ptr(g)),
-                          'layer_bwd_coefs')
-            db = None if db32 is None else db32.to(bias.dtype)
-            d_next = None if dn32 is None else dn32.to(next_scale.dtype)
-            d_out = None if do32 is None else do32.to(out_scale.dtype)
+            direct = ctx.needs_input_grad[1] and all(t is None or (t.dtype in _lib._DTYPES and t.is_contiguous()) for t in (out_scale, next_scale, bias))
+            if direct:
+                db = torch.empty([o], dtype=bias.dtype, device=g.device) if want_db else None
+                d_next = torch.empty([n, o], dtype=next_scale.dtype, device=g.device) if want_next else None
+                d_out = torch.empty([n, o], dtype=out_scale.dtype, device=g.device) if want_out else None
+                code = lambda t: _lib.F32 if t is None else _lib._DTYPES[t.dtype]
+                keep = (psum, gz, dysy)
+                tail = _lib.LayerCoefs(db=_lib.ptr(db), d_next=_lib.ptr(d_next), d_out=_lib.ptr(d_out), psum=psum.data_ptr(), out_scale=_lib.ptr(out_scale),
+                                       next_scale=_lib.ptr(next_scale), bias=_lib.ptr(bias), gz=_lib.ptr(gz if want_next else None), dysy=_lib.ptr(dysy),
+                                       slots=int(psum.shape[2]), n=n, cout=o, out_scale_dtype=code(out_scale), next_scale_dtype=code(next_scale),
+                                       bias_dtype=code(bias), db_dtype=code(db), d_next_dtype=code(d_next), d_out_dtype=code(d_out))
+            else:
+                osc = None if out_scale is None else out_scale.to(f32).contiguous()
+                nsc = None if next_scale is None else next_scale.to(f32).contiguous()
+                b32 = None if bias is None else bias.to(f32).contiguous()
+                db32 = torch.empty([o], dtype=f32, device=g.device) if want_db else None
+                dn32 = torch.empty([n, o], dtype=f32, device=g.device) if want_next else None
+                do32 = torch.empty([n, o], dtype=f32, device=g.device) if want_out else None
+                _lib.launched(_lib.load().afcm_layer_bwd_coefs(_lib.ptr(db32), _lib.ptr(dn32), _lib.ptr(do32), psum.data_ptr(), int(psum.shape[2]), _lib.ptr(osc),
+                                                               _lib.ptr(nsc), _lib.ptr(b32), _lib.ptr(gz if want_next else None), _lib.ptr(dysy), n, o,
+                                                               _lib.stream_ptr(g)), 'layer_bwd_coefs')
+                db = None if db32 is None else db32.to(bias.dtype)
+                d_next = None if dn32 is None else dn32.to(next_scale.dtype)
+                d_out = None if do32 is None else do32.to(out_scale.dtype)
         if has_skip and ctx.needs_input_grad[7]:
             d_skip = _conv.scale_planes(g, next_scale) if (next_scale is not None and not ctx.skip_by_fork) else g
         if ctx.needs_input_grad[0] or (ctx.needs_input_grad[2] and not prescaled):
@@ -92,10 +108,11 @@
                 d_in = torch.where(s2 > 0, _conv.plane_dot(xs, dx) / s2.clamp_min(1e-30), torch.zeros_like(s2)).to(in_scale.dtype)
         if ctx.needs_input_grad[1]:
             if ctx.link_in is not None and ctx.link_in.want:
-                dw, ctx.link_in.gz = _conv._wgrad_raw(dys, xs, cout, cin, ks, conv_pad, dots_with=w)
+                dw, ctx.link_in.gz = _conv._wgrad_raw(dys, xs, cout, cin, ks, conv_pad, dots_with=w, tail=tail)
                 dw = dw.to(w.dtype)
             else:
-                dw = _conv._wgrad_raw(dys, xs, cout, cin, ks, conv_pad).to(w.dtype)
+                dw = _conv._wgrad_raw(dys, xs, cout, cin, ks, conv_pad, tail=tail).to(w.dtype)
+        del keep
         return dx, dw, d_in, d_out, db, None, None, d_skip, d_next, None, None, None, None, None, None, None
 
 
diff --git a/include/afcm_hip.h b/include/afcm_hip.h
--- a/include/afcm_hip.h
+++ b/include/afcm_hip.h
@@ -107,6 +107,10 @@
 int afcm_plane_dot_gated_ld(float* out, const void* a, const void* b, int32_t dtype, int64_t planes, int32_t h, int32_t w,
                             int32_t a_pitch, int32_t b_pitch, const int32_t* flags, int32_t slots, const float* out_scale,
                             const float* gz, const float* next_scale, const float* gskip, void* stream);
+int afcm_plane_dot2(float* out_b, float* out_c, const void* a, const void* b, const void* c, int32_t dtype, int64_t planes, int32_t hw,
+                    void* stream);
+int afcm_plane_dot2_ld(float* out_b, float* out_c, const void* a, const void* b, const void* c, int32_t dtype, int64_t planes, int32_t h,
+                       int32_t w, int32_t a_pitch, int32_t b_pitch, int32_t c_pitch, void* stream);
 
 int afcm_weight_norm_fwd(float* w_hat, float* wsq, float* scale, const float* w, int32_t cout, int32_t cin, int32_t kk, void* stream);
 int afcm_weight_norm_bwd(float* dw, const float* g_hat, const float* g_wsq, const float* w_hat, const float* scale, int32_t cout,
@@ -120,6 +124,24 @@
 int afcm_layer_bwd_coefs(float* db, float* d_next, float* d_out, const float* psum, int32_t slots, const float* out_scale,
                          const float* next_scale, const float* bias, const float* gz, const float* dysy, int32_t n, int32_t cout,
                          void* stream);
+
+typedef struct afcm_layer_coefs {
+    void*        db;
+    void*        d_next;
+    void*        d_out;
+    const float* psum;
+    const void*  out_scale;
+    const void*  next_scale;
+    const void*  bias;
+    const float* gz;
+    const float* dysy;
+    int32_t slots, n, cout;
+    int32_t out_scale_dtype, next_scale_dtype, bias_dtype;
+    int32_t db_dtype, d_next_dtype, d_out_dtype;
+} afcm_layer_coefs;
+int afcm_conv2d_wgrad_tail_ld(float* dw, float* dots, float* workspace, const void* dy, const void* x, const float* wref, int32_t dtype,
+                              int32_t n, int32_t cin, int32_t cout, int32_t h, int32_t w, int32_t ks, int32_t pad, int32_t dy_pitch,
+                              int32_t x_pitch, const afcm_layer_coefs* tail, void* stream);
 
 typedef struct afcm_adam_entry {
     void*   p;
```

New measurement: 484.6 images/sec (median of 4 runs). Within noise of the previous version (+0.1%).
